# DavidPeicho/cuda-pathtracer

Hardware: AMD Instinct MI355X
Metric: Msamples/sec at 1920x1080, 4 spp, indoor.obj (higher is better)
Workload: dtype f32

## Files before the change

cuda-pathtracer_amd/__init__.py:

```python
from . import native
from .native import (KERNEL_AUTO, KERNEL_BRUTE_FORCE, KERNEL_BVH, KERNEL_BVH_PERSISTENT, KERNEL_BVH_BLOCKWISE, KERNEL_BVH_SPLIT, KERNEL_BVH_RESTART, KERNEL_BVH_RESTART_FMA,
                     PtamdError)
from .scene import (HostScene, cubemap_for_scene, cubemap_from_color, cubemap_from_cross,
                    FACE_DTYPE, MATERIAL_DTYPE, LIGHT_DTYPE, TEXTURE_DTYPE, CAMERA_DTYPE)
from .render import (Context, FrameRenderer, SceneRig, host_pose_faces, host_skin_faces, host_morph_faces, AdaptiveState, host_adaptive_select, host_denoise, DenoiseHistory, HostDenoiseHistory, host_denoise_temporal, orbit_camera, host_bvh_trace, host_skip_trace, host_faces_away, FORM_FLAT_SKIP, FORM_PLAIN_SKIP, host_scene_tables, host_scene_quality, host_bvh_refit_trace, host_bvh4_trace, host_bvh4q_trace, host_bvh8_trace, origin_reach, interleaved_rows, wang_hash, REFERENCE_BOUNCES,
                     POST_NONE, POST_GRAYSCALE, POST_SEPIA, POST_INVERT)
from .tiles import row_bands, band_of_rank, BandGather, interleaved_bands, rank_times_ms, time_gather_ms
from .synthetic import tessellate, deform
from .image import save_ppm, load_ppm, save_png
from .images import pil_image_loader, ldr_to_float, load_image, load_image8, native_image_loader, resize_float

__all__ = [n for n in dir() if not n.startswith("_")]
```

cuda-pathtracer_amd/csrc/ptamd_host.h:

```cpp
#pragma once

#include "../host/ptamd_internal.h"
#include "pt_device.h"
#include "pt_launch.h"
#include "pt_refit.h"
#include "ptamd_owners.h"
#include "ptamd_tuning.h"

#include <string>
#include <type_traits>
#include <vector>

namespace ptamd {

struct DeviceScene {
  DeviceBuffer<float4> nodes;
  DeviceBuffer<float4> nodes4;
  DeviceBuffer<float4> nodes8;
  DeviceBuffer<float4> nodes4q;
  uint32_t n_nodes8 = 0, depth8 = 0;
  DeviceBuffer<float4> tris_bvh;
  DeviceBuffer<float4> tris_brute;
  DeviceBuffer<float4> shade;
  bool flat = false;
  DeviceBuffer<int4> materials;
  DeviceBuffer<float4> lights;
  DeviceBuffer<TexDesc> textures;
  DeviceBuffer<float> texels;
  uint32_t n_faces = 0, n_lights = 0, n_nodes = 0, n_materials = 0, n_textures = 0;
  uint32_t n_bvh_tris = 0;
  uint32_t n_nodes4 = 0, depth4 = 0;
  float extent = 0.0f;
  bool all_finite = true;
  uint32_t n_skipped = 0;
  bool links = false, cull_on = false;
  uint32_t n_culled = 0;
  DeviceBuffer<uint32_t> links_plain;
  Bvh topology;
  std::vector<uint32_t> record_face;
  std::vector<uint8_t> skip_set, cull_bits;
  std::vector<uint32_t> link_words;
  PinnedBuffer<uint32_t> h_links[2];
  float reach = 0.0f;
  float margin_floor = 0.0f;
  ptamd_scene_info info{};
  bool released = false;
  bool refit_ok = false;
  std::vector<uint32_t> material_ids;
  std::vector<ptamd_light> host_lights;
  DeviceBuffer<float> raw;
  DeviceBuffer<uint32_t> refit_groups;
  DeviceBuffer<uint32_t> refit_levels;
  DeviceBuffer<uint32_t> refit_sched;
  DeviceBuffer<uint32_t> wide_child;
  uint32_t n_refit_groups = 0, n_refit_levels = 0, n_refit_sched = 0, refit_top_first = 0, refit_top_levels = 0;
  DeviceBuffer<float> d_faces;
  PinnedBuffer<ptamd_face> h_stage[2];
  Event staged[2];
  bool staged_valid[2] = { false, false };
  uint32_t stage_next = 0;
  Event updated;
  bool updated_valid = false;
  DeviceBuffer<float> d_margin;
  PinnedBuffer<float> h_margin;
  Event margin_ready[2];
  bool margin_ready_valid[2] = { false, false };
  uint32_t margin_next = 0, margin_slot = 0;
  bool margins_pending = false;
  PinnedBuffer<ptamd_light> h_lights[2];
  Event lights_staged[2];
  bool lights_staged_valid[2] = { false, false };
  uint32_t lights_next = 0;
  double quality_built = 0.0;
  DeviceBuffer<double> d_quality;
};

struct DeviceCubemap {
  DeviceBuffer<float4> faces;
  uint32_t size = 0;
  bool uniform = false;
  float color[3] = { 0.f, 0.f, 0.f };
};

}

struct ptamd_context {
  int device = 0;
  ptamd::TuningSettings knobs;
  std::vector<ptamd::DeviceScene> scenes;
  std::vector<ptamd::DeviceCubemap> cubemaps;
  uint32_t frame_counter = 0;
  int32_t last_restart_form = -1;
  ptamd::DeviceBuffer<unsigned long long> d_stats;
  ptamd::DeviceBuffer<float> d_gamma;
  ptamd::DeviceBuffer<uint32_t> d_tickets;
  ptamd::DeviceBuffer<uint32_t> d_heads;
  uint32_t ticket_next = 0;
  std::vector<bool> heads_clean;
  std::vector<bool> slot_pinned;
  int n_cus = 0;
  struct Occupancy { size_t lds = ~(size_t)0; int blocks_per_cu = -1; } occupancy[ptamd::kFormSlots];
  struct SampleScratch {
    void* stream = nullptr;
    ptamd::DeviceBuffer<float> buf[4];
    size_t bytes[4] = { 0, 0, 0, 0 };
    ptamd::Event mega_done[3];
    ptamd::Event resolved[3];
    bool resolved_valid[3] = { false, false, false };
    ptamd::Event last_done;
    uint32_t flip = 0;
    bool no_pipeline = false;
    bool captured = false;
    std::vector<uint32_t> pinned_slots;
  };
  std::vector<SampleScratch> sample_scratch;
  static constexpr uint32_t kMaxLanes = 4;
  ptamd::Stream lane[kMaxLanes];
  uint32_t n_lanes = 0;
  ptamd::Stream internal[2];
  uint32_t lane_next = 0;
  ptamd::DeviceBuffer<uint2> d_trace_spill;
  struct { uint32_t config = ~0u; size_t lds = 0; int resident = 0; } trace_queue_cache;
  size_t trace_spill_bytes = 0;
  ptamd::DeviceBuffer<unsigned long long> d_timeline;
  uint32_t timeline_waves = 0;
  ptamd::DeviceBuffer<float4> d_denoise;
  size_t denoise_pixels = 0;
};

static_assert(!std::is_copy_constructible<ptamd::DeviceScene>::value && !std::is_copy_constructible<ptamd::DeviceCubemap>::value &&
              !std::is_copy_constructible<ptamd_context::SampleScratch>::value && !std::is_copy_constructible<ptamd_context>::value,
              "structs that own device resources move, they are never copied");

namespace ptamd {

constexpr size_t kLdsBudget = 64 * 1024;
constexpr uint32_t kCompactMaxNodes = 896;
constexpr uint32_t kCompactMaxTris = 2047;
constexpr float kBoxMargin = 1e-3f;
constexpr uint32_t kTicketRing = 1024;
constexpr uint32_t kMaxFramesPerSlab = 4;

int hip_fail(const char* what, hipError_t e);

#define PT_HIP(call)                                         \
  do {                                                       \
    hipError_t _e = (call);                                  \
    if (_e != hipSuccess) return hip_fail(#call, _e);        \
  } while (0)

inline bool live_scene(const ptamd_context* ctx, uint32_t scene_id)
{
  return scene_id < ctx->scenes.size() && !ctx->scenes[scene_id].released;
}

int bring_up(ptamd_context* ctx, hipStream_t s);
bool stream_is_capturing(hipStream_t stream);

bool far_origin_camera(const DeviceScene& s, const ptamd_camera& cam);
int settle_margins(DeviceScene& s, hipStream_t stream, const char* who);
void fill_scene(const DeviceScene& s, const DeviceCubemap* cm, KParams& p);
int wait_for_update(const DeviceScene& s, hipStream_t stream, bool capturing);
int update_scene_checks(const char* who, const ptamd_context* ctx, uint32_t scene_id, uint32_t n_faces, const void* faces);
int update_capture_checks(const char* who, const ptamd_context* ctx, hipStream_t stream);
int wait_for_readers(const ptamd_context* ctx, const DeviceScene& s, hipStream_t stream);
int device_array_checks(const char* who, const char* what, const ptamd_context* ctx, const void* p, size_t bytes, bool aligned16);
int prepare_device_refit(const char* who, DeviceScene& s, RefitParams& r);
int enqueue_device_refit(DeviceScene& s, RefitParams& r, const float* faces, hipStream_t stream);

float frame_nb_inverse(float c);
float camera_terms(const ptamd_camera& cam, uint32_t width, KParams& p);
int do_launch(ptamd_context* ctx, const ptamd_launch* l, bool stats, const AdaptiveParams* ad = nullptr);

}
```

cuda-pathtracer_amd/csrc/ptamd_launch.cpp:

```cpp
#include "ptamd_host.h"
#include "pt_adaptive.h"

#include <algorithm>
#include <cmath>
#include <cstdlib>
#include <cstring>

namespace ptamd {

float frame_nb_inverse(float c)
{
  uint32_t bits;
  std::memcpy(&bits, &c, 4);
  const uint32_t exponent = bits >> 23;
  if ((bits & 0x007FFFFFu) != 0u || exponent < 1u || exponent > 253u) return 0.0f;
  return 1.0f / c;
}

namespace {

constexpr float kQuantisedMaxExtent = 1.0e8f;
constexpr size_t kMaxScratchStreams = 16;

void fill_far_table(uint32_t t[16])
// ... 226 lines not shown
  const uint32_t node_bytes = p.wide8 == 2u ? 64u : 128u;
  const uint32_t waves = restart_threads(false) / 64u;
  const uint32_t share = 160u * 1024u / restart_wide_blocks_per_cu() - 256u;
  const uint32_t pools = (ctx->knobs.pool_in_lds && ctx->knobs.pool_in_lds_wide && !ad) ? waves * PT_POOL_LDS_BYTES : 0u;
  const uint32_t region = restart_treelet_region_bytes();
  uint32_t treelet_want = ctx->knobs.treelet_nodes * (128u / node_bytes);
  if (region && treelet_want > region / node_bytes) treelet_want = region / node_bytes;
  uint32_t treelet = treelet_want < p.n_nodes4 ? treelet_want : p.n_nodes4;
  if (!region && treelet * node_bytes + waves * 512u * 4u + pools > share) treelet = (share - pools - waves * 512u * 4u) / node_bytes;
  const uint32_t treelet_bytes = region ? (treelet ? region : 0u) : treelet * node_bytes;
  uint32_t fit = (share - pools - treelet_bytes) / (waves * 512u);
  if (const char* ev = tuning_env("PTAMD_STACK_LDS")) { int v = std::atoi(ev); if (v >= 1 && (uint32_t)v <= fit) fit = (uint32_t)v; }
  p.treelet_nodes = treelet;
  p.stack_lds_entries = need < fit ? need : fit;
  p.stack_spill_entries = need - p.stack_lds_entries;
  pl.launch_lds = (size_t)treelet_bytes + (size_t)p.stack_lds_entries * waves * 512u;
  if (pools) {
    p.pool_lds_offset = (uint32_t)pl.launch_lds;
    if (!p.pool_lds_offset) p.pool_lds_offset = 16u;
    pl.launch_lds = p.pool_lds_offset + pools;
  }
}

KernelForm form_of(const LaunchPlan& pl, bool stats, bool list, const KParams* p)
{
  return megakernel_form(pl.fma ? (uint32_t)PTAMD_KERNEL_BVH_RESTART_FMA : pl.which, pl.resident, stats, list, pl.launch_lds, p);
}

int blocks_per_cu(ptamd_context* ctx, const LaunchPlan& pl, const KernelForm& form, int& bpc)
{
  ptamd_context::Occupancy& occ = ctx->occupancy[form.cache_slot];
  const size_t key = pl.resident ? pl.launch_lds : (pl.which == PTAMD_KERNEL_BVH_RESTART ? pl.launch_lds + 1u : 0);
  if (occ.blocks_per_cu < 0 || occ.lds != key) {
    int q = -1;
    const hipError_t e = form_blocks_per_cu(form, &q);
    if (e != hipSuccess || q < 1) {
      occ.blocks_per_cu = -1;
      return hip_fail((std::string("occupancy query of the ") + form.name + " kernel").c_str(), e);
    }
    occ.blocks_per_cu = q; occ.lds = key;
  }
  bpc = occ.blocks_per_cu;
  return PTAMD_OK;
}

int size_grid(ptamd_context* ctx, const ptamd_launch* l, const AdaptiveParams* ad, LaunchPlan& pl, KParams& p)
{
  const bool restart = pl.which == PTAMD_KERNEL_BVH_RESTART;
  const uint32_t count = l->frame_count > 1 ? l->frame_count : 1u;
  uint32_t rows = l->row_end - l->row_begin;
  if (l->interleave_ranks > 1u) {
    rows = ptamd_interleaved_rows(l->height, l->interleave_ranks, l->interleave_rank, l->interleave_rows);
    p.ilv_ranks = l->interleave_ranks; p.ilv_rank = l->interleave_rank; p.ilv_rows = l->interleave_rows;
    p.row_begin = 0; p.row_end = rows;
    p.tfb_row0 = l->height - rows;
    p.surf_row0 = 0;
  }
  p.y_limit = l->row_end;
  p.tiles_x = (l->width + PT_TILE_W - 1u) / PT_TILE_W;
  p.n_tiles = p.tiles_x * ((rows + PT_TILE_H - 1u) / PT_TILE_H);
  if (p.n_tiles == 0) return PTAMD_OK;
  if ((uint64_t)p.n_tiles * count >= (1ull << 31)) {
    set_error("ptamd_raytrace: rows x width x frame_count too large for one launch (split the batch)");
    return PTAMD_ERR_LIMIT;
  }
  int bpc = 0;
  const KernelForm form = form_of(pl, false, ad != nullptr, nullptr);
  const int rc = blocks_per_cu(ctx, pl, form, bpc);
  if (rc != PTAMD_OK) return rc;
  pl.waves_per_block = form.ticket_waves;
  uint32_t n_blocks = (uint32_t)ctx->n_cus * (uint32_t)bpc;
  p.sample_count = count;
  p.frame_nb0 = l->frame_nb;
  p.refill_min = ctx->knobs.refill_min ? ctx->knobs.refill_min : (l->bounces >= 5 ? 16u : 64u);
  p.tiles_per_ticket = ad ? 1u : ctx->knobs.tiles_per_ticket;
  const uint32_t share = pl.pipelined ? (l->machine_share > 2u ? l->machine_share : 2u) : l->machine_share;
  if (share > 1u) n_blocks = n_blocks / share > 0u ? n_blocks / share : 1u;
  const uint32_t n_tickets = (p.n_tiles * count + p.tiles_per_ticket - 1u) / p.tiles_per_ticket;
  const uint32_t useful = (n_tickets + pl.waves_per_block - 1u) / pl.waves_per_block;
  if (n_blocks > useful) n_blocks = useful;
  if (restart && !ad && p.tiles_per_ticket == 1u && n_blocks >= 8u && (uint64_t)p.n_tiles * count < (1ull << 28) &&
      (ctx->knobs.xcd_regions == 2u || (ctx->knobs.xcd_regions == 1u && !pl.resident))) {
    n_blocks &= ~7u;
    p.xcd_regions = 1u;
  }
  pl.n_blocks = n_blocks;
  if (count > 1) p.frame_nb_f = (float)(int)(l->frame_nb + count - 1u);
  p.frame_nb_inv = frame_nb_inverse(p.frame_nb_f);
  return PTAMD_OK;
}

constexpr int kReplan = -1;

int bind_slab(ptamd_context* ctx, const ptamd_launch* l, LaunchPlan& pl, KParams& p)
{
  ptamd_context::SampleScratch* sc = pl.sc;
  const bool restart = pl.which == PTAMD_KERNEL_BVH_RESTART;
  if (p.sample_count <= 1 && !restart) return PTAMD_OK;
  const size_t sample_bytes = ((size_t)p.sample_count * (p.row_end - p.row_begin) * l->width * 3u * sizeof(float) + 255u) & ~(size_t)255u;
  const size_t pool_bytes = (restart && !p.pool_lds_offset) ? (size_t)pl.n_blocks * pl.waves_per_block * 192u * sizeof(float4) : 0u;
  const size_t spill_bytes = (size_t)pl.n_blocks * pl.waves_per_block * p.stack_spill_entries * 512u;
  const size_t need = sample_bytes + pool_bytes + spill_bytes + 16u;
  auto grow = [&](uint32_t i) -> int {
    PT_HIP(hipStreamSynchronize(pl.stream));
    for (uint32_t k = 0; k < ctx->n_lanes; ++k) PT_HIP(hipStreamSynchronize(ctx->lane[k].get()));
    for (const Stream& is : ctx->internal) if (is) PT_HIP(hipStreamSynchronize(is.get()));
    sc->bytes[i] = 0;
    if (sc->buf[i].alloc(need) != hipSuccess) { (void)hipGetLastError(); return PTAMD_ERR_HIP; }
    sc->bytes[i] = need;
    return PTAMD_OK;
  };
  pl.slab = pl.pipelined ? sc->flip % 3u : 3u;
  if (pl.pipelined) {
    for (int i = 0; i < 3; ++i) {
      PT_HIP(sc->mega_done[i].ensure());
      PT_HIP(sc->resolved[i].ensure());
    }
    bool ok = true;
    for (uint32_t i = 0; i < 3u && ok; ++i) if (need > sc->bytes[i]) ok = grow(i) == PTAMD_OK;
    if (!ok) {
      for (uint32_t i = 0; i < 3u; ++i) { sc->buf[i].reset(); sc->bytes[i] = 0; }
      sc->no_pipeline = true;
      return kReplan;
    }
  } else if (need > sc->bytes[3]) {
    if (pl.capturing) {
      set_error("ptamd_raytrace: a launch cannot size its stream's sample slab inside a graph capture: issue this configuration once eagerly first");
      return PTAMD_ERR_LIMIT;
    }
    if (sc->captured) {
      set_error("ptamd_raytrace: a captured graph pins this stream's sample slab; a larger launch would reallocate it under the graph "
                "(ptamd_release_captured(ctx, stream) once the graph is gone)");
      return PTAMD_ERR_LIMIT;
    }
    if (grow(3u) != PTAMD_OK) return hip_fail("hipMalloc of the sample slab", hipErrorOutOfMemory);
  }
  p.samples_out = sc->buf[pl.slab].get();
  p.pool = reinterpret_cast<float4*>(reinterpret_cast<char*>(p.samples_out) + sample_bytes);
  p.stack_spill = reinterpret_cast<uint2*>(reinterpret_cast<char*>(p.samples_out) + sample_bytes + pool_bytes);
  return PTAMD_OK;
}

int take_slot(ptamd_context* ctx, bool capturing, ptamd_context::SampleScratch* sc, uint32_t& slot)
{
  slot = ctx->ticket_next++ % kTicketRing;
  for (uint32_t tries = 0; ctx->slot_pinned[slot]; ++tries) {
    if (tries >= kTicketRing) { set_error("ptamd_raytrace: every ring slot of ticket heads is pinned by captured graphs (ptamd_release_captured)"); return PTAMD_ERR_LIMIT; }
    slot = ctx->ticket_next++ % kTicketRing;
  }
  if (capturing && sc) { ctx->slot_pinned[slot] = true; sc->pinned_slots.push_back(slot); sc->captured = true; }
  return PTAMD_OK;
}

int issue(ptamd_context* ctx, const DeviceScene& scene, bool stats, const AdaptiveParams* ad, const LaunchPlan& pl, KParams& p)
{
  const bool split = pl.which == PTAMD_KERNEL_BVH_SPLIT, restart = pl.which == PTAMD_KERNEL_BVH_RESTART;
  ptamd_context::SampleScratch* sc = pl.sc;
  int urc = wait_for_update(scene, pl.stream, pl.capturing);
  if (urc != PTAMD_OK) return urc;
  p.round_min = ctx->knobs.round_min;
  p.round_div = ctx->knobs.round_div;
  p.round_div_m16 = (65536u + ctx->knobs.round_div - 1u) / ctx->knobs.round_div;
  p.walk_min = ctx->knobs.walk_min;
  p.walk_min4 = ctx->knobs.walk_min4;
  p.tile_counter = ctx->d_tickets.get() + pl.slot;
  if (ad) p.adaptive = ad->block;
  p.n_static = pl.n_blocks * pl.waves_per_block;
  if (split) PT_HIP(hipMemsetD32Async(reinterpret_cast<hipDeviceptr_t>(p.tile_counter), (int)p.n_static, 1, pl.stream));
  hipStream_t mega_stream = pl.stream;
  if (pl.pipelined) {
    mega_stream = pl.stream != nullptr ? ctx->lane[ctx->lane_next++ % ctx->n_lanes].get() : ctx->internal[ctx->lane_next++ & 1u].get();
    sc->flip++;
    if (sc->resolved_valid[pl.slab]) PT_HIP(hipStreamWaitEvent(mega_stream, sc->resolved[pl.slab].get(), 0));
    if ((urc = wait_for_update(scene, mega_stream, false)) != PTAMD_OK) return urc;
  }
  if (!split) {
    p.tile_heads = ctx->d_heads.get() + (size_t)pl.slot * 8u * PT_HEAD_STRIDE;
    if (!ctx->heads_clean[pl.slot]) PT_HIP(hipMemsetD32Async(reinterpret_cast<hipDeviceptr_t>(p.tile_heads), 0, 8u * PT_HEAD_STRIDE, mega_stream));
    ctx->heads_clean[pl.slot] = false;
  }
  if (restart && !pl.fma && ctx->d_timeline && p.n_static <= ctx->timeline_waves) p.timeline = ctx->d_timeline.get();
  if (split) p.tiles_per_ticket = 1;
  ctx->last_restart_form = restart ? restart_select(pl.resident, stats, ad != nullptr, pl.fma, &p).variant : -1;
  hipError_t e = launch_form(form_of(pl, stats, ad != nullptr, &p), p, pl.n_blocks, restart ? mega_stream : pl.stream);
  if (e == hipSuccess && pl.pipelined) {
    PT_HIP(hipEventRecord(sc->mega_done[pl.slab].get(), mega_stream));
    PT_HIP(hipStreamWaitEvent(pl.stream, sc->mega_done[pl.slab].get(), 0));
  }
  if (e == hipSuccess && (p.sample_count > 1 || restart)) {
    if (ad) {
      AdaptiveParams a = *ad;
      a.samples = p.samples_out;
      a.tile_heads = p.tile_heads;
      e = launch_adaptive_resolve_list(a, pl.stream);
    } else {
      e = launch_resolve(p, pl.stream);
    }
    if (e == hipSuccess && !split) ctx->heads_clean[pl.slot] = true;
    if (e == hipSuccess && pl.pipelined) {
      PT_HIP(hipEventRecord(sc->resolved[pl.slab].get(), pl.stream));
      sc->resolved_valid[pl.slab] = true;
    }
  }
  if (e == hipSuccess && !pl.capturing && ctx->knobs.overlap) {
    PT_HIP(sc->last_done.ensure());
    PT_HIP(hipEventRecord(sc->last_done.get(), pl.stream));
  }
  return e == hipSuccess ? PTAMD_OK : hip_fail("megakernel launch", e);
}

int launch_part(ptamd_context* ctx, const ptamd_launch* l, bool stats, bool later_chunk, const AdaptiveParams* ad, const LaunchPlan& resolved)
{
  LaunchPlan pl = resolved;
  KParams p;
  int rc;
  if (persistent_family(pl.which)) {
    do {
      pl = resolved;
      fill_launch(ctx, l, stats, pl, p);
      if ((rc = plan_stream(ctx, l, stats, later_chunk, ad, pl)) != PTAMD_OK) return rc;
      lay_out_lds(ctx, ctx->scenes[l->scene_id], stats, ad, pl, p);
      if ((rc = size_grid(ctx, l, ad, pl, p)) != PTAMD_OK || p.n_tiles == 0) return rc;
      rc = bind_slab(ctx, l, pl, p);
    } while (rc == kReplan);
    if (rc != PTAMD_OK || (rc = take_slot(ctx, pl.capturing, pl.sc, pl.slot)) != PTAMD_OK) return rc;
    return issue(ctx, ctx->scenes[l->scene_id], stats, ad, pl, p);
  }
  fill_launch(ctx, l, stats, pl, p);
  if (ctx->scenes[l->scene_id].updated_valid &&
      (rc = wait_for_update(ctx->scenes[l->scene_id], pl.stream, stream_is_capturing(pl.stream))) != PTAMD_OK) return rc;
  const KernelForm form = form_of(pl, stats, false, &p);
  uint32_t n_blocks = 0;
  if (pl.which == PTAMD_KERNEL_BVH_BLOCKWISE) {
    const uint32_t rows = l->row_end - l->row_begin;
    const uint32_t st_rows = (form.threads / 64u) * 2u;
    p.tiles_x = (l->width + 31u) / 32u;
    p.n_tiles = p.tiles_x * ((rows + st_rows - 1u) / st_rows);
    if (p.n_tiles == 0) return PTAMD_OK;
    int bpc = 0;
    if ((rc = blocks_per_cu(ctx, pl, form, bpc)) != PTAMD_OK || (rc = take_slot(ctx, false, nullptr, pl.slot)) != PTAMD_OK) return rc;
    n_blocks = std::min((uint32_t)ctx->n_cus * (uint32_t)bpc, p.n_tiles);
    p.tile_counter = ctx->d_tickets.get() + pl.slot;
    PT_HIP(hipMemsetD32Async(reinterpret_cast<hipDeviceptr_t>(p.tile_counter), (int)n_blocks, 1, pl.stream));
  }
  const hipError_t e = launch_form(form, p, n_blocks, pl.stream);
  return e == hipSuccess ? PTAMD_OK : hip_fail("megakernel launch", e);
}

}

int do_launch(ptamd_context* ctx, const ptamd_launch* l, bool stats, const AdaptiveParams* ad)
{
  int rc = validate_launch(ctx, l);
  LaunchPlan resolved;
  if (rc != PTAMD_OK || (rc = settle_margins(ctx->scenes[l->scene_id], static_cast<hipStream_t>(l->stream), "ptamd_raytrace")) != PTAMD_OK ||
      (rc = resolve_kernel(ctx, l, stats, ad, resolved)) != PTAMD_OK) return rc;
  PT_HIP(hipSetDevice(ctx->device));
  const uint32_t part_frames = persistent_family(resolved.which) ? kMaxFramesPerSlab : 1u;
  for (uint32_t k0 = 0; k0 == 0 || k0 < l->frame_count; k0 += part_frames) {
    ptamd_launch part = *l;
    part.frame_nb = l->frame_nb + k0;
    part.frame_count = std::min(l->frame_count - k0, part_frames);
    if (k0 > 0) part.reset_accumulation = 0;
    if ((rc = launch_part(ctx, &part, stats, k0 > 0, ad, resolved)) != PTAMD_OK) return rc;
  }
  return PTAMD_OK;
}

}

using namespace ptamd;

extern "C" {

int ptamd_raytrace(ptamd_context* ctx, void* surface_rgba8, uint32_t scene_id, uint32_t cubemap_id,
                   const ptamd_camera* cam, uint32_t width, uint32_t height, void* stream,
                   float* temporal_framebuffer, int32_t moved, uint32_t post_id)
{
  if (!ctx || !cam) { set_error("ptamd_raytrace: null argument"); return PTAMD_ERR_ARG; }
  uint32_t seed = ctx->frame_counter;
  if (moved) seed = 0;
  seed++;
  ptamd_launch l;
  std::memset(&l, 0, sizeof l);
  l.surface_rgba8 = surface_rgba8; l.temporal_framebuffer = temporal_framebuffer; l.stream = stream;
  l.camera = *cam; l.scene_id = scene_id; l.cubemap_id = cubemap_id;
  l.width = width; l.height = height; l.row_begin = 0; l.row_end = height;
  l.frame_nb = seed; l.bounces = 3;
  l.moved = moved; l.post_id = post_id; l.kernel = PTAMD_KERNEL_AUTO;
  int rc = do_launch(ctx, &l, false);
  if (rc == PTAMD_OK) ctx->frame_counter = seed;
  return rc;
}

int ptamd_raytrace_ex(ptamd_context* ctx, const ptamd_launch* launch) { return do_launch(ctx, launch, false); }

int ptamd_release_captured(ptamd_context* ctx, void* stream)
{
  if (!ctx) { set_error("ptamd_release_captured: null context"); return PTAMD_ERR_ARG; }
  for (auto& c : ctx->sample_scratch) {
    if (c.stream != stream) continue;
    for (uint32_t slot : c.pinned_slots) { ctx->slot_pinned[slot] = false; ctx->heads_clean[slot] = false; }
    c.pinned_slots.clear();
    c.captured = false;
  }
  return PTAMD_OK;
}

int ptamd_raytrace_stats(ptamd_context* ctx, const ptamd_launch* launch, ptamd_trace_stats* out)
{
  if (!ctx || !out) { set_error("ptamd_raytrace_stats: null argument"); return PTAMD_ERR_ARG; }
  PT_HIP(hipSetDevice(ctx->device));
  hipStream_t st = launch ? static_cast<hipStream_t>(launch->stream) : nullptr;
  PT_HIP(hipMemsetAsync(ctx->d_stats.get(), 0, 13 * sizeof(unsigned long long), st));
  PT_HIP(hipMemsetAsync(ctx->d_stats.get() + 16, 0, 12 * sizeof(unsigned long long), st));
  int rc = do_launch(ctx, launch, true);
  if (rc != PTAMD_OK) return rc;
  PT_HIP(hipStreamSynchronize(st));
  unsigned long long h[13];
  PT_HIP(hipMemcpy(h, ctx->d_stats.get(), sizeof h, hipMemcpyDeviceToHost));
  out->rays = h[0]; out->nodes_visited = h[1]; out->tris_tested = h[2];
  out->mesh_hits = h[3]; out->nmap_hits = h[4]; out->samples = h[5];
  out->wave_node_iters = h[6]; out->wave_tri_iters = h[7];
  out->fetch_events = h[8]; out->fetch_rays = h[9];
  out->idle_unstarted = h[10]; out->idle_finished = h[11]; out->idle_parked = h[12];
  return PTAMD_OK;
}

int ptamd_trace_rays(ptamd_context* ctx, uint32_t scene_id, uint32_t kernel, const float* rays_host, uint32_t n,
                     int32_t* out_host)
{
  if (!ctx || !live_scene(ctx, scene_id) || (n && (!rays_host || !out_host)) ||
      (kernel > PTAMD_KERNEL_BVH && kernel != PTAMD_KERNEL_BVH_RESTART)) {
    set_error("ptamd_trace_rays: bad argument");
    return PTAMD_ERR_ARG;
  }
  if (n == 0) return PTAMD_OK;
  PT_HIP(hipSetDevice(ctx->device));
  DeviceScene& s = ctx->scenes[scene_id];
  int src = settle_margins(s, nullptr, "ptamd_trace_rays");
  if (src != PTAMD_OK) return src;
  KParams p;
  std::memset(&p, 0, sizeof p);
  fill_scene(s, nullptr, p);
  fill_far_table(p.far_table);
  p.small_det = 0u;
  p.stack_lds_entries = choose_wide_nodes(ctx, s, true, p);
  DeviceBuffer<float> d_rays;
  DeviceBuffer<int4> d_out;
  PT_HIP(d_rays.alloc((size_t)n * 24));
  hipError_t e = d_out.alloc((size_t)n * 16);
  if (e != hipSuccess) return hip_fail("hipMalloc", e);
  if ((e = hipMemcpy(d_rays.get(), rays_host, (size_t)n * 24, hipMemcpyHostToDevice)) != hipSuccess ||
      (e = launch_trace_rays(p, kernel == PTAMD_KERNEL_BRUTE_FORCE ? 1 : (kernel == PTAMD_KERNEL_BVH_RESTART ? 3 : 2), d_rays.get(), n, d_out.get(), nullptr)) != hipSuccess ||
      (e = hipDeviceSynchronize()) != hipSuccess ||
      (e = hipMemcpy(out_host, d_out.get(), (size_t)n * 16, hipMemcpyDeviceToHost)) != hipSuccess)
    return hip_fail("ptamd_trace_rays", e);
  return PTAMD_OK;
}

int ptamd_trace_rays_queue(ptamd_context* ctx, uint32_t scene_id, const float* rays_dev, uint32_t n, int32_t* out_dev, uint32_t config,
                           uint32_t refill_min, void* stream, uint32_t* out_waves_per_cu)
{
  if (!ctx || !live_scene(ctx, scene_id) || (n && (!rays_dev || !out_dev)) || config > 3u || n >= 0x80000000u) { set_error("ptamd_trace_rays_queue: bad argument"); return PTAMD_ERR_ARG; }
  if (n == 0) return PTAMD_OK;
  PT_HIP(hipSetDevice(ctx->device));
  const DeviceScene& s = ctx->scenes[scene_id];
  if (s.n_nodes4 == 0) { set_error("ptamd_trace_rays_queue: the scene has no wide tree"); return PTAMD_ERR_ARG; }
  hipStream_t st = static_cast<hipStream_t>(stream);
  KParams p;
  std::memset(&p, 0, sizeof p);
  p.nodes4 = s.nodes4.get(); p.n_nodes4 = s.n_nodes4; p.tris_bvh = s.tris_bvh.get(); p.n_bvh_tris = s.n_bvh_tris;
  p.lights = s.lights.get(); p.n_lights = s.n_lights;
  p.refill_min = refill_min < 1u ? 1u : (refill_min > 64u ? 64u : refill_min);
  p.walk_min4 = ctx->knobs.walk_min4;
  uint32_t threads, plane, bpc;
  trace_queue_shape(config, &threads, &plane, &bpc);
  const uint32_t waves = threads / 64u;
  p.treelet_nodes = plane < s.n_nodes4 ? plane : s.n_nodes4;
// ... 33 lines not shown
```

cuda-pathtracer_amd/csrc/ptamd_scene.cpp:

```cpp
#include "ptamd_host.h"
#include "pt_refit.h"
#include "pt_refit_device.h"

#include <cmath>
#include <cstring>

namespace ptamd {

bool far_origin_camera(const DeviceScene& s, const ptamd_camera& cam)
{
  const float cam_far = std::fmax(std::fabs(cam.position.x), std::fmax(std::fabs(cam.position.y), std::fabs(cam.position.z))) +
                        std::fabs(cam.aperture);
  return !(margins_cover(s.extent, s.margin_floor, cam_far) && margins_cover(s.extent, s.margin_floor, s.reach)) && s.n_faces != 0;
}

int settle_margins(DeviceScene& s, hipStream_t stream, const char* who)
{
  if (!s.margins_pending) return PTAMD_OK;
  if (stream_is_capturing(stream)) {
    set_error(std::string(who) + ": the scene's margins are pending behind ptamd_scene_update_device and a capture cannot wait for "
              "them: render the scene once, or call ptamd_scene_quality, outside the capture");
    return PTAMD_ERR_LIMIT;
  }
  PT_HIP(hipEventSynchronize(s.margin_ready[s.margin_slot].get()));
// ... 152 lines not shown
      word |= 0x40000000u;
      std::memcpy(s + 18, &word, 4);
    }
  }
  const bool flat = t.flat = scene_is_flat(sc);
  if (flat) shade.resize(shade.size() + (size_t)sc->n_faces * 16, 0.0f);
  for (uint32_t i = 0; flat && i < sc->n_faces; ++i) {
    const ptamd_face& f = sc->faces[i];
    const float* texel = sc->texels + sc->textures[sc->materials[f.material_id].diffuse_spec_map].offset;
    float* r = &shade[(size_t)sc->n_faces * kShadeFloats + (size_t)i * 16];
    write_flat_normals(f, r);
    for (int k = 0; k < 3; ++k) r[4 * k + 3] = texel[k];
    r[12] = texel[3];
  }
  return PTAMD_OK;
}

int refit_scene_tables(SceneTables& t, const ptamd_face* faces, uint32_t n_faces, const ptamd_light* lights, uint32_t n_lights)
{
  const int rc = refit_bvh(t.bvh, faces, n_faces, lights, n_lights);
  if (rc != PTAMD_OK) return rc;
  for (uint32_t i = 0; i < n_faces; ++i) {
    write_face_geometry(faces[i], i, &t.brute[(size_t)i * 12], &t.shade[(size_t)i * kShadeFloats]);
    if (t.flat) write_flat_normals(faces[i], &t.shade[(size_t)n_faces * kShadeFloats + (size_t)i * 16]);
  }
  return PTAMD_OK;
}

}

int update_scene_checks(const char* who, const ptamd_context* ctx, uint32_t scene_id, uint32_t n_faces, const void* faces)
{
  const std::string w(who);
  if (!live_scene(ctx, scene_id)) { set_error(w + ": scene_id out of range or released"); return PTAMD_ERR_ARG; }
  const DeviceScene& s = ctx->scenes[scene_id];
  if (n_faces != s.n_faces) { set_error(w + ": n_faces differs from the uploaded count"); return PTAMD_ERR_ARG; }
  if (n_faces && !faces) { set_error(w + ": null faces"); return PTAMD_ERR_ARG; }
  if (!s.refit_ok) {
    set_error(w + ": this scene's tree is not refitted (built with PTAMD_WIDE8, PTAMD_WIDE4Q or PTAMD_BVH_SPLIT_ALPHA)");
    return PTAMD_ERR_ARG;
  }
  return PTAMD_OK;
}

int update_capture_checks(const char* who, const ptamd_context* ctx, hipStream_t stream)
{
  for (const auto& c : ctx->sample_scratch)
    if (c.captured) { set_error(std::string(who) + ": a captured launch pins this context's scenes (ptamd_release_captured)"); return PTAMD_ERR_LIMIT; }
  if (stream_is_capturing(stream)) { set_error(std::string(who) + ": an update cannot be captured into a graph"); return PTAMD_ERR_LIMIT; }
  return PTAMD_OK;
}

int device_array_checks(const char* who, const char* what, const ptamd_context* ctx, const void* p, size_t bytes, bool aligned16)
{
  const std::string w = std::string(who) + ": ", name(what);
  if (aligned16 && (reinterpret_cast<uintptr_t>(p) & 15u) != 0u) {
    set_error(w + name + " is not aligned to 16 bytes (the kernels use 16-byte loads)");
    return PTAMD_ERR_ARG;
  }
  PT_HIP(hipSetDevice(ctx->device));
  hipPointerAttribute_t attr;
  std::memset(&attr, 0, sizeof attr);
  if (hipPointerGetAttributes(&attr, p) != hipSuccess || attr.type != hipMemoryTypeDevice || attr.device != ctx->device) {
    (void)hipGetLastError();
    set_error(w + name + " is not device memory of the context's device (host arrays go to the call that takes them)");
    return PTAMD_ERR_ARG;
  }
  hipDeviceptr_t base = nullptr;
  size_t room = 0;
  if (hipMemGetAddressRange(&base, &room, const_cast<void*>(p)) == hipSuccess) {
    const size_t offset = (size_t)(static_cast<const char*>(p) - static_cast<const char*>(base));
    if (offset > room || room - offset < bytes) {
      set_error(w + "the allocation behind " + name + " is smaller than the call reads");
      return PTAMD_ERR_ARG;
    }
  } else {
    (void)hipGetLastError();
  }
  return PTAMD_OK;
}

namespace {

int refit_params(const char* who, const DeviceScene& s, RefitParams& r)
{
  std::memset(&r, 0, sizeof r);
  r.nodes = reinterpret_cast<float*>(s.nodes.get()); r.tris_bvh = reinterpret_cast<float*>(s.tris_bvh.get());
  r.nodes4 = reinterpret_cast<float*>(s.nodes4.get()); r.tris_brute = reinterpret_cast<float*>(s.tris_brute.get());
  r.shade = reinterpret_cast<float*>(s.shade.get()); r.raw = s.raw.get();
  r.groups = s.refit_groups.get(); r.levels = s.refit_levels.get(); r.sched = s.refit_sched.get(); r.wide_child = s.wide_child.get();
  r.n_faces = s.n_faces; r.n_tris = s.n_bvh_tris; r.n_nodes = s.n_nodes; r.n_nodes4 = s.n_nodes4;
  r.n_groups = s.n_refit_groups; r.top_level_first = s.refit_top_first; r.top_levels = s.refit_top_levels;
  r.flat = s.flat ? 1u : 0u;
  r.margin = kBoxMargin;
  if (!r.nodes || !r.tris_bvh || !r.nodes4 || !r.tris_brute || !r.shade || !r.raw || !r.groups || !r.levels || !r.sched || !r.wide_child ||
      r.n_tris != r.n_faces || r.n_nodes == 0 || r.n_groups == 0 || r.top_level_first + r.top_levels > s.n_refit_levels ||
      s.n_refit_sched >= r.n_nodes) {
    set_error(std::string(who) + ": the scene's refit tables are inconsistent");
    return PTAMD_ERR_ARG;
  }
  return PTAMD_OK;
}

}

int wait_for_readers(const ptamd_context* ctx, const DeviceScene& s, hipStream_t stream)
{
  for (const auto& c : ctx->sample_scratch) {
    for (int i = 0; i < 3; ++i) if (c.mega_done[i]) PT_HIP(hipStreamWaitEvent(stream, c.mega_done[i].get(), 0));
    if (c.last_done) PT_HIP(hipStreamWaitEvent(stream, c.last_done.get(), 0));
  }
  if (s.updated_valid) PT_HIP(hipStreamWaitEvent(stream, s.updated.get(), 0));
  return PTAMD_OK;
}

int prepare_device_refit(const char* who, DeviceScene& s, RefitParams& r)
{
  const int rc = refit_params(who, s, r);
  if (rc != PTAMD_OK) return rc;
  if (!s.d_margin) PT_HIP(s.d_margin.alloc((kMarginWords + 2u * kExtentMaxGroups) * sizeof(float)));
  if (!s.h_margin) PT_HIP(s.h_margin.alloc(2u * kMarginWords * sizeof(float)));
  for (int i = 0; i < 2; ++i) PT_HIP(s.margin_ready[i].ensure());
  PT_HIP(s.updated.ensure());
  return PTAMD_OK;
}

int restore_plain_links(DeviceScene& s, hipStream_t stream)
{
  if (!s.n_culled) return PTAMD_OK;
  PT_HIP(hipMemcpyAsync(reinterpret_cast<float*>(s.nodes.get()) + (size_t)s.n_nodes * 16, s.links_plain.get(), ((size_t)s.n_nodes * 8 + 8) * 4,
                        hipMemcpyDeviceToDevice, stream));
  s.n_culled = 0;
  return PTAMD_OK;
}

int enqueue_device_refit(DeviceScene& s, RefitParams& r, const float* faces, hipStream_t stream)
{
  for (int i = 0; i < 2; ++i)
    if (s.margin_ready_valid[i]) PT_HIP(hipStreamWaitEvent(stream, s.margin_ready[i].get(), 0));
  const int rc = restore_plain_links(s, stream);
  if (rc != PTAMD_OK) return rc;
  PT_HIP(launch_extent(faces, s.n_faces, s.d_margin.get() + kMarginWords, s.d_margin.get(), stream));
  r.faces = faces;
  r.device_margin = s.d_margin.get() + 2;
  PT_HIP(launch_refit(r, stream));
  PT_HIP(hipEventRecord(s.updated.get(), stream));
  s.updated_valid = true;
  const uint32_t slot = s.margin_next++ & 1u;
  PT_HIP(hipMemcpyAsync(s.h_margin.get() + (size_t)slot * kMarginWords, s.d_margin.get(), kMarginWords * sizeof(float), hipMemcpyDeviceToHost, stream));
  PT_HIP(hipEventRecord(s.margin_ready[slot].get(), stream));
  s.margin_ready_valid[slot] = true;
  s.margin_slot = slot;
  s.margins_pending = true;
  return PTAMD_OK;
}

}

using namespace ptamd;

extern "C" {

int ptamd_upload_scene(ptamd_context* ctx, const ptamd_scene_desc* sc, uint32_t* out_scene_id)
{
  if (!ctx || !sc || !out_scene_id) { set_error("ptamd_upload_scene: null argument"); return PTAMD_ERR_ARG; }
  int rc = validate_scene_desc(sc);
  if (rc != PTAMD_OK) return rc;
  SceneTables t;
  if ((rc = make_scene_tables(sc, (ctx->knobs.wide8 ? kBvhForm8 : 0u) | (ctx->knobs.wide4q ? kBvhForm4q : 0u), t)) != PTAMD_OK) return rc;
  const Bvh& bvh = t.bvh;
  const std::vector<float>& brute = t.brute;
  const std::vector<float>& shade = t.shade;
  const bool flat = t.flat;
  std::vector<int32_t> mats((size_t)sc->n_materials * 4, 0);
  for (uint32_t i = 0; i < sc->n_materials; ++i) {
    mats[i * 4 + 0] = sc->materials[i].diffuse_spec_map;
    mats[i * 4 + 1] = sc->materials[i].normal_map;
    std::memcpy(&mats[i * 4 + 2], &sc->materials[i].ior, 4);
  }
  std::vector<TexDesc> tex(sc->n_textures);
  for (uint32_t i = 0; i < sc->n_textures; ++i) {
    tex[i].w = sc->textures[i].w; tex[i].h = sc->textures[i].h; tex[i].nb_chan = sc->textures[i].nb_chan;
    tex[i].pad = 0; tex[i].offset = sc->textures[i].offset;
  }

  PT_HIP(hipSetDevice(ctx->device));
  DeviceScene d;
  d.n_faces = sc->n_faces; d.n_lights = sc->n_lights; d.n_nodes = bvh.n_nodes; d.n_bvh_tris = bvh.n_tris;
  d.extent = bvh.extent; d.all_finite = bvh.all_finite; d.reach = bvh.reach; d.margin_floor = bvh.margin_floor;
  d.n_nodes4 = bvh.n_nodes4; d.depth4 = bvh.depth4;
  d.n_nodes8 = bvh.n_nodes8; d.depth8 = bvh.depth8;
  d.n_materials = sc->n_materials; d.n_textures = sc->n_textures;
  d.flat = flat;
  std::vector<ptamd_light> dev_lights(sc->lights, sc->lights + sc->n_lights);
  for (ptamd_light& dl : dev_lights) dl.radius = dl.radius * dl.radius;
  std::vector<float> nodes_and_links(bvh.nodes);
  if (bvh.n_nodes * 64u + bvh.n_tris * 48u <= kLdsBudget && bvh.n_nodes <= kCompactMaxNodes && bvh.n_tris <= kCompactMaxTris && skip_links_fit(bvh)) {
    const uint32_t mode = ctx->knobs.skip_mode;
    SkipTables t;
    build_skip_tables(bvh, mode == PTAMD_SKIP_SET ? mode : (mode | PTAMD_SKIP_CULLED), ctx->knobs.skip_threshold, nullptr, t);
    d.n_skipped = t.n_skipped; d.n_culled = t.n_culled;
    d.links = t.n_skipped != 0u || t.n_culled != 0u;
    if (d.links) {
      nodes_and_links.resize(bvh.nodes.size() + t.words.size());
      std::memcpy(nodes_and_links.data() + bvh.nodes.size(), t.words.data(), t.words.size() * 4);
    }
    if (t.n_culled) {
      std::vector<uint32_t> plain;
      skip_link_table(bvh, t.skip, plain);
      if ((rc = upload(d.links_plain, plain.data(), plain.size() * 4))) return rc;
      d.cull_on = true;
      d.topology.nodes = bvh.nodes;
      d.topology.n_nodes = bvh.n_nodes; d.topology.n_tris = bvh.n_tris;
      d.topology.tris.resize((size_t)bvh.n_tris * 12);
      d.skip_set = t.skip;
      d.record_face.resize(bvh.n_tris);
      for (uint32_t j = 0; j < bvh.n_tris; ++j) std::memcpy(&d.record_face[j], &bvh.tris[(size_t)j * 12 + 9], 4);
    }
  }
  if ((rc = upload(d.nodes, nodes_and_links.data(), nodes_and_links.size() * 4)) ||
      (rc = upload(d.nodes4, bvh.nodes4.data(), bvh.nodes4.size() * 4)) ||
      (bvh.nodes8.empty() ? 0 : (rc = upload(d.nodes8, bvh.nodes8.data(), bvh.nodes8.size() * 4))) ||
      (bvh.nodes4q.empty() ? 0 : (rc = upload(d.nodes4q, bvh.nodes4q.data(), bvh.nodes4q.size() * 4))) ||
      (rc = upload_padded(d.tris_bvh, bvh.tris.data(), bvh.tris.size() * 4, 128)) ||
      (rc = upload(d.tris_brute, brute.data(), brute.size() * 4)) ||
      (rc = upload(d.shade, shade.data(), shade.size() * 4)) ||
      (rc = upload(d.materials, mats.data(), mats.size() * 4)) ||
      (rc = upload(d.lights, dev_lights.data(), dev_lights.size() * sizeof(ptamd_light))) ||
      (rc = upload(d.textures, tex.data(), tex.size() * sizeof(TexDesc))) ||
      (rc = upload(d.texels, sc->texels, (size_t)sc->n_texel_floats * 4)))
    return rc;
  d.refit_ok = !bvh.split && bvh.nodes8.empty() && bvh.nodes4q.empty();
  if (d.refit_ok) {
    if ((rc = upload(d.raw, bvh.raw.data(), bvh.raw.size() * 4)) ||
        (rc = upload(d.refit_groups, bvh.refit_groups.data(), bvh.refit_groups.size() * 4)) ||
        (rc = upload(d.refit_levels, bvh.refit_levels.data(), bvh.refit_levels.size() * 4)) ||
        (rc = upload(d.refit_sched, bvh.refit_sched.data(), bvh.refit_sched.size() * 4)) ||
        (rc = upload(d.wide_child, bvh.wide_child.data(), bvh.wide_child.size() * 4)))
      return rc;
    d.n_refit_groups = (uint32_t)bvh.refit_groups.size() / 4u; d.n_refit_levels = (uint32_t)bvh.refit_levels.size();
    d.n_refit_sched = (uint32_t)bvh.refit_sched.size();
    d.refit_top_first = bvh.refit_top_first; d.refit_top_levels = bvh.refit_top_levels;
    d.material_ids.resize(sc->n_faces);
    for (uint32_t i = 0; i < sc->n_faces; ++i) d.material_ids[i] = sc->faces[i].material_id;
  }
  d.host_lights.assign(sc->lights, sc->lights + sc->n_lights);
  d.quality_built = tree_quality(bvh.nodes.data(), bvh.n_nodes, sc->n_faces);
  d.info.n_faces = sc->n_faces; d.info.n_lights = sc->n_lights; d.info.n_nodes = bvh.n_nodes;
  d.info.n_leaves = bvh.n_leaves; d.info.max_leaf_size = bvh.max_leaf; d.info.depth = bvh.depth;
  d.info.node_bytes = 64; d.info.tri_bytes = 48;
  d.info.n_nodes4 = d.n_nodes4; d.info.depth4 = d.depth4;
  d.info.lds_bytes_bvh = bvh.n_nodes * 64u + bvh.n_tris * 48u;
  d.info.lds_bytes_brute = sc->n_faces * 48u;
  ctx->scenes.push_back(std::move(d));
  *out_scene_id = (uint32_t)ctx->scenes.size() - 1;
  return PTAMD_OK;
}

int ptamd_scene_update(ptamd_context* ctx, const ptamd_scene_update_desc* d)
{
  if (!ctx || !d) { set_error("ptamd_scene_update: null argument"); return PTAMD_ERR_ARG; }
  int rc = update_scene_checks("ptamd_scene_update", ctx, d->scene_id, d->n_faces, d->faces);
  if (rc != PTAMD_OK) return rc;
  DeviceScene& s = ctx->scenes[d->scene_id];
  for (uint32_t i = 0; i < d->n_faces; ++i)
    if (d->faces[i].material_id != s.material_ids[i]) { set_error("ptamd_scene_update: a face's material_id differs from the uploaded one"); return PTAMD_ERR_ARG; }
  hipStream_t stream = static_cast<hipStream_t>(d->stream);
  if ((rc = update_capture_checks("ptamd_scene_update", ctx, stream)) != PTAMD_OK) return rc;
  if (d->n_faces == 0) return PTAMD_OK;
  PT_HIP(hipSetDevice(ctx->device));
  RefitParams r;
  if ((rc = refit_params("ptamd_scene_update", s, r)) != PTAMD_OK) return rc;
  const size_t bytes = (size_t)d->n_faces * sizeof(ptamd_face);
  if (!s.d_faces) PT_HIP(s.d_faces.alloc(bytes));
  const size_t link_words = (size_t)s.n_nodes * 8 + 8;
  for (int i = 0; i < 2; ++i) {
    if (!s.h_stage[i]) PT_HIP(s.h_stage[i].alloc(bytes));
    if (s.cull_on && !s.h_links[i]) PT_HIP(s.h_links[i].alloc(link_words * 4));
    PT_HIP(s.staged[i].ensure());
  }
  PT_HIP(s.updated.ensure());
  Bvh m;
  m.margin = kBoxMargin;
  r.origin_margin = bvh_margins(m, d->faces, d->n_faces, s.host_lights.data(), (uint32_t)s.host_lights.size());
  const uint32_t slot = s.stage_next++ & 1u;
  if (s.staged_valid[slot]) PT_HIP(hipEventSynchronize(s.staged[slot].get()));
  std::memcpy(s.h_stage[slot].get(), d->faces, bytes);
  if ((rc = wait_for_readers(ctx, s, stream)) != PTAMD_OK) return rc;
  PT_HIP(hipMemcpyAsync(s.d_faces.get(), s.h_stage[slot].get(), bytes, hipMemcpyHostToDevice, stream));
  if (s.cull_on) {
    Bvh& topo = s.topology;
    for (uint32_t j = 0; j < s.n_bvh_tris; ++j) rf_tri_record(&d->faces[s.record_face[j]].vertices[0].x, s.record_face[j], &topo.tris[(size_t)j * 12]);
    const uint32_t n_culled = cull_table(topo, s.cull_bits);
    skip_link_table(topo, s.skip_set, s.link_words, n_culled ? &s.cull_bits : nullptr);
    std::memcpy(s.h_links[slot].get(), s.link_words.data(), link_words * 4);
    PT_HIP(hipMemcpyAsync(reinterpret_cast<float*>(s.nodes.get()) + (size_t)s.n_nodes * 16, s.h_links[slot].get(), link_words * 4, hipMemcpyHostToDevice, stream));
    s.n_culled = n_culled;
  }
  PT_HIP(hipEventRecord(s.staged[slot].get(), stream));
  s.staged_valid[slot] = true;
  r.faces = s.d_faces.get();
  PT_HIP(launch_refit(r, stream));
  PT_HIP(hipEventRecord(s.updated.get(), stream));
  s.updated_valid = true;
  s.extent = m.extent; s.all_finite = m.all_finite; s.reach = m.reach; s.margin_floor = m.margin_floor;
  s.margins_pending = false;
  return PTAMD_OK;
}

int ptamd_scene_update_device(ptamd_context* ctx, const ptamd_scene_update_device_desc* d)
{
  const char* who = "ptamd_scene_update_device";
  if (!ctx || !d) { set_error("ptamd_scene_update_device: null argument"); return PTAMD_ERR_ARG; }
  int rc = update_scene_checks(who, ctx, d->scene_id, d->n_faces, d->faces);
  hipStream_t stream = static_cast<hipStream_t>(d->stream);
  if (rc != PTAMD_OK || (rc = update_capture_checks(who, ctx, stream)) != PTAMD_OK) return rc;
  DeviceScene& s = ctx->scenes[d->scene_id];
  if (d->n_faces == 0) return PTAMD_OK;
  if ((rc = device_array_checks(who, "faces", ctx, d->faces, (size_t)d->n_faces * sizeof(ptamd_face), true)) != PTAMD_OK) return rc;
  RefitParams r;
  if ((rc = prepare_device_refit(who, s, r)) != PTAMD_OK || (rc = wait_for_readers(ctx, s, stream)) != PTAMD_OK) return rc;
  return enqueue_device_refit(s, r, reinterpret_cast<const float*>(d->faces), stream);
}

int ptamd_scene_update_lights(ptamd_context* ctx, const ptamd_scene_lights_desc* d)
{
  const char* who = "ptamd_scene_update_lights";
  if (!ctx || !d) { set_error("ptamd_scene_update_lights: null argument"); return PTAMD_ERR_ARG; }
  if (!live_scene(ctx, d->scene_id)) { set_error("ptamd_scene_update_lights: scene_id out of range or released"); return PTAMD_ERR_ARG; }
  DeviceScene& s = ctx->scenes[d->scene_id];
  if (d->n_lights != s.n_lights) { set_error("ptamd_scene_update_lights: n_lights differs from the uploaded count"); return PTAMD_ERR_ARG; }
  if (d->n_lights && !d->lights) { set_error("ptamd_scene_update_lights: null lights"); return PTAMD_ERR_ARG; }
  hipStream_t stream = static_cast<hipStream_t>(d->stream);
  int rc = update_capture_checks(who, ctx, stream);
  if (rc != PTAMD_OK) return rc;
  if (d->n_lights == 0) return PTAMD_OK;
  PT_HIP(hipSetDevice(ctx->device));
  const size_t bytes = (size_t)d->n_lights * sizeof(ptamd_light);
  for (int i = 0; i < 2; ++i) {
    if (!s.h_lights[i]) PT_HIP(s.h_lights[i].alloc(bytes));
    PT_HIP(s.lights_staged[i].ensure());
  }
  PT_HIP(s.updated.ensure());
  const uint32_t slot = s.lights_next++ & 1u;
  if (s.lights_staged_valid[slot]) PT_HIP(hipEventSynchronize(s.lights_staged[slot].get()));
  ptamd_light* staged = s.h_lights[slot].get();
  for (uint32_t i = 0; i < d->n_lights; ++i) {
    staged[i] = d->lights[i];
    staged[i].radius = d->lights[i].radius * d->lights[i].radius;
  }
  if ((rc = wait_for_readers(ctx, s, stream)) != PTAMD_OK) return rc;
  PT_HIP(hipMemcpyAsync(s.lights.get(), staged, bytes, hipMemcpyHostToDevice, stream));
  PT_HIP(hipEventRecord(s.lights_staged[slot].get(), stream));
  s.lights_staged_valid[slot] = true;
  PT_HIP(hipEventRecord(s.updated.get(), stream));
  s.updated_valid = true;
  s.host_lights.assign(d->lights, d->lights + d->n_lights);
  if (!s.margins_pending) {
    Bvh m;
    m.margin = kBoxMargin;
    bvh_margins_of_extent(m, s.extent, s.all_finite, s.host_lights.data(), (uint32_t)s.host_lights.size());
    s.reach = m.reach; s.margin_floor = m.margin_floor;
  }
  return PTAMD_OK;
}

int ptamd_scene_margins(ptamd_context* ctx, uint32_t scene_id, float out[4])
{
  if (!ctx || !out) { set_error("ptamd_scene_margins: null argument"); return PTAMD_ERR_ARG; }
  if (!live_scene(ctx, scene_id)) { set_error("ptamd_scene_margins: scene_id out of range or released"); return PTAMD_ERR_ARG; }
// ... 6 lines not shown

int ptamd_scene_quality(ptamd_context* ctx, uint32_t scene_id, void* stream, ptamd_scene_quality_info* out)
{
  if (!ctx || !out) { set_error("ptamd_scene_quality: null argument"); return PTAMD_ERR_ARG; }
  if (!live_scene(ctx, scene_id)) { set_error("ptamd_scene_quality: scene_id out of range or released"); return PTAMD_ERR_ARG; }
  hipStream_t st = static_cast<hipStream_t>(stream);
  if (stream_is_capturing(st)) { set_error("ptamd_scene_quality: the call waits for its result and cannot be captured into a graph"); return PTAMD_ERR_LIMIT; }
  DeviceScene& s = ctx->scenes[scene_id];
  int rc = settle_margins(s, st, "ptamd_scene_quality");
  if (rc != PTAMD_OK) return rc;
  out->built = s.quality_built;
  out->now = 0.0;
  if (s.n_nodes == 0 || s.n_faces == 0) return PTAMD_OK;
  PT_HIP(hipSetDevice(ctx->device));
  const uint32_t groups = quality_groups(s.n_nodes);
  if (!s.d_quality) PT_HIP(s.d_quality.alloc((size_t)(groups + 1u) * sizeof(double)));
  if ((rc = wait_for_update(s, st, false)) != PTAMD_OK) return rc;
  PT_HIP(launch_quality(reinterpret_cast<const float*>(s.nodes.get()), s.n_nodes, s.d_quality.get(), st));
  std::vector<double> part(groups + 1u);
  PT_HIP(hipMemcpyAsync(part.data(), s.d_quality.get(), part.size() * sizeof(double), hipMemcpyDeviceToHost, st));
  PT_HIP(hipStreamSynchronize(st));
  double sum = 0.0;
  for (uint32_t g = 0; g < groups; ++g) sum += part[g];
  out->now = sum / part[groups];
  return PTAMD_OK;
}

int ptamd_host_scene_quality(const ptamd_scene_desc* sc, const ptamd_face* faces_b, double* out)
{
  if (!sc || !out) { set_error("ptamd_host_scene_quality: null argument"); return PTAMD_ERR_ARG; }
  int rc = validate_scene_desc(sc);
  SceneTables t;
  if (rc != PTAMD_OK || (rc = make_scene_tables(sc, 0u, t)) != PTAMD_OK) return rc;
  if (faces_b && (rc = refit_scene_tables(t, faces_b, sc->n_faces, sc->lights, sc->n_lights)) != PTAMD_OK) return rc;
  *out = tree_quality(t.bvh.nodes.data(), t.bvh.n_nodes, sc->n_faces);
  return PTAMD_OK;
}

int ptamd_scene_release(ptamd_context* ctx, uint32_t scene_id)
{
  if (!ctx) { set_error("ptamd_scene_release: null context"); return PTAMD_ERR_ARG; }
  if (!live_scene(ctx, scene_id)) { set_error("ptamd_scene_release: scene_id out of range or released"); return PTAMD_ERR_ARG; }
  PT_HIP(hipSetDevice(ctx->device));
  PT_HIP(hipDeviceSynchronize());
  ctx->scenes[scene_id] = DeviceScene();
  ctx->scenes[scene_id].released = true;
  return PTAMD_OK;
}

int ptamd_scene_table_read(ptamd_context* ctx, uint32_t scene_id, uint32_t which, void* out, uint64_t* bytes)
{
  if (!ctx || !bytes || which > 4u) { set_error("ptamd_scene_table_read: bad argument"); return PTAMD_ERR_ARG; }
  if (!live_scene(ctx, scene_id)) { set_error("ptamd_scene_table_read: scene_id out of range or released"); return PTAMD_ERR_ARG; }
  const DeviceScene& s = ctx->scenes[scene_id];
  const void* src[5] = { s.nodes.get(), s.tris_bvh.get(), s.nodes4.get(), s.tris_brute.get(), s.shade.get() };
  const uint64_t size[5] = { (uint64_t)s.n_nodes * 64u, (uint64_t)s.n_bvh_tris * 48u, (uint64_t)s.n_nodes4 * 128u, (uint64_t)s.n_faces * 48u,
                             (uint64_t)s.n_faces * (kShadeFloats * 4u + (s.flat ? 64u : 0u)) };
  const uint64_t room = *bytes;
  *bytes = size[which];
  if (!out) return PTAMD_OK;
  if (room < size[which]) { set_error("ptamd_scene_table_read: the buffer is smaller than the table"); return PTAMD_ERR_ARG; }
  PT_HIP(hipSetDevice(ctx->device));
  PT_HIP(hipDeviceSynchronize());
  if (size[which]) PT_HIP(hipMemcpy(out, src[which], size[which], hipMemcpyDeviceToHost));
  return PTAMD_OK;
}

int ptamd_host_scene_refit(const ptamd_scene_desc* sc, const ptamd_face* faces_b, const ptamd_face* faces_c, uint32_t which, void* out,
                           uint64_t* bytes)
{
  if (!sc || !bytes || which > 5u) { set_error("ptamd_host_scene_refit: bad argument"); return PTAMD_ERR_ARG; }
  int rc = validate_scene_desc(sc);
  SceneTables t;
  if (rc != PTAMD_OK || (rc = make_scene_tables(sc, 0u, t)) != PTAMD_OK) return rc;
  for (const ptamd_face* f : { faces_b, faces_c })
    if (f && (rc = refit_scene_tables(t, f, sc->n_faces, sc->lights, sc->n_lights)) != PTAMD_OK) return rc;
  const float scalars[4] = { t.bvh.extent, t.bvh.reach, t.bvh.margin_floor, t.bvh.all_finite ? 1.0f : 0.0f };
  const void* src[6] = { t.bvh.nodes.data(), t.bvh.tris.data(), t.bvh.nodes4.data(), t.brute.data(), t.shade.data(), scalars };
  const uint64_t size[6] = { t.bvh.nodes.size() * 4u, t.bvh.tris.size() * 4u, t.bvh.nodes4.size() * 4u, t.brute.size() * 4u, t.shade.size() * 4u, 16u };
  const uint64_t room = *bytes;
  *bytes = size[which];
  if (!out) return PTAMD_OK;
  if (room < size[which]) { set_error("ptamd_host_scene_refit: the buffer is smaller than the table"); return PTAMD_ERR_ARG; }
  if (size[which]) std::memcpy(out, src[which], size[which]);
  return PTAMD_OK;
}

int ptamd_upload_cubemap(ptamd_context* ctx, const float* faces, uint32_t size, uint32_t* out_cubemap_id)
{
  if (!ctx || !faces || !out_cubemap_id || size == 0 || size > 16384) { set_error("ptamd_upload_cubemap: bad argument"); return PTAMD_ERR_ARG; }
  PT_HIP(hipSetDevice(ctx->device));
  DeviceCubemap c;
  c.size = size;
  if (size == 1) {
    c.uniform = true;
    for (int f = 1; f < 6; ++f) c.uniform = c.uniform && std::memcmp(faces + f * 4, faces, 12) == 0;
    std::memcpy(c.color, faces, 12);
  }
  int rc = upload(c.faces, faces, (size_t)6 * size * size * 16);
  if (rc != PTAMD_OK) return rc;
  ctx->cubemaps.push_back(std::move(c));
  *out_cubemap_id = (uint32_t)ctx->cubemaps.size() - 1;
  return PTAMD_OK;
}

int ptamd_scene_info_get(ptamd_context* ctx, uint32_t scene_id, ptamd_scene_info* out)
{
  if (!ctx || !out || !live_scene(ctx, scene_id)) { set_error("ptamd_scene_info_get: bad argument"); return PTAMD_ERR_ARG; }
  *out = ctx->scenes[scene_id].info;
  return PTAMD_OK;
}

int ptamd_scene_desc_is_flat(const ptamd_scene_desc* sc, int32_t* out_flat)
{
  if (!sc || !out_flat || (sc->n_faces && !sc->faces) || (sc->n_materials && !sc->materials) || (sc->n_textures && !sc->textures)) {
    set_error("ptamd_scene_desc_is_flat: null argument or table");
    return PTAMD_ERR_ARG;
  }
  for (uint32_t i = 0; i < sc->n_faces; ++i) {
    const uint32_t m = sc->faces[i].material_id;
    if (m >= sc->n_materials || sc->materials[m].diffuse_spec_map < 0 || (uint32_t)sc->materials[m].diffuse_spec_map >= sc->n_textures) {
      set_error("ptamd_scene_desc_is_flat: material or texture id out of range");
      return PTAMD_ERR_ARG;
    }
  }
  *out_flat = scene_is_flat(sc) ? 1 : 0;
  return PTAMD_OK;
}

int ptamd_scene_is_flat(ptamd_context* ctx, uint32_t scene_id, uint32_t cubemap_id, int32_t* out_flat)
{
  if (!ctx || !out_flat || !live_scene(ctx, scene_id) || cubemap_id >= ctx->cubemaps.size()) {
    set_error("ptamd_scene_is_flat: bad argument");
    return PTAMD_ERR_ARG;
  }
  *out_flat = ctx->knobs.flat_round && ctx->scenes[scene_id].flat && ctx->cubemaps[cubemap_id].uniform ? 1 : 0;
  return PTAMD_OK;
}

int ptamd_scene_skip_count(ptamd_context* ctx, uint32_t scene_id, uint32_t* out)
{
  if (!ctx || !out || !live_scene(ctx, scene_id)) { set_error("ptamd_scene_skip_count: bad argument"); return PTAMD_ERR_ARG; }
  *out = ctx->scenes[scene_id].n_skipped;
  return PTAMD_OK;
}

int ptamd_last_restart_form(ptamd_context* ctx, int32_t* out)
{
  if (!ctx || !out) { set_error("ptamd_last_restart_form: null argument"); return PTAMD_ERR_ARG; }
  *out = ctx->last_restart_form;
  return PTAMD_OK;
}

int ptamd_scene_cull_count(ptamd_context* ctx, uint32_t scene_id, uint32_t* out)
{
  if (!ctx || !out || !live_scene(ctx, scene_id)) { set_error("ptamd_scene_cull_count: bad argument"); return PTAMD_ERR_ARG; }
  *out = ctx->scenes[scene_id].n_culled;
  return PTAMD_OK;
}

}
```

cuda-pathtracer_amd/csrc/ptamd_tuning.cpp:

```cpp
#include "ptamd_tuning.h"
#include "../host/ptamd_internal.h"

#include <cstdlib>
#include <cstring>

namespace ptamd {

const char* tuning_env(const char* name)
{
  const char* gate = std::getenv("PTAMD_TUNING");
  if (!gate || std::atoi(gate) != 1) return nullptr;
  return std::getenv(name);
}

namespace {

enum KnobKind {
  kSwitch,
  kClamped,
  kKernel,
  kSkipWord,
  kOpenUnit,
};

struct Knob {
  const char* name;
  KnobKind kind;
  bool TuningSettings::* flag;
  uint32_t TuningSettings::* number;
  float TuningSettings::* real;
  int lo, hi;
};

constexpr Knob on_off(const char* name, bool TuningSettings::* f) { return { name, kSwitch, f, nullptr, nullptr, 0, 1 }; }
constexpr Knob number(const char* name, KnobKind kind, uint32_t TuningSettings::* f, int lo, int hi) { return { name, kind, nullptr, f, nullptr, lo, hi }; }

using S = TuningSettings;
constexpr Knob kKnobs[] = {
  on_off("PTAMD_GAMMA_TABLE", &S::gamma_table),
  on_off("PTAMD_OVERLAP", &S::overlap),
  number("PTAMD_REFILL_MIN", kClamped, &S::refill_min, 1, 64),
  number("PTAMD_DEFAULT_KERNEL", kKernel, &S::default_kernel, 1, 6),
  number("PTAMD_ROUND_MIN", kClamped, &S::round_min, 1, 64),
  number("PTAMD_ROUND_DIV", kClamped, &S::round_div, 1, 64),
  number("PTAMD_WALK_MIN", kClamped, &S::walk_min, 1, 64),
  number("PTAMD_WALK_MIN4", kClamped, &S::walk_min4, 1, 64),
  on_off("PTAMD_SHORT_RCP", &S::short_rcp),
  on_off("PTAMD_WIDE8", &S::wide8),
  on_off("PTAMD_WIDE4Q", &S::wide4q),
  on_off("PTAMD_RS_GENERIC", &S::generic_round),
  on_off("PTAMD_RS_FLAT", &S::flat_round),
  number("PTAMD_SKIP", kSkipWord, &S::skip_mode, 0, 0),
  { "PTAMD_SKIP_THRESHOLD", kOpenUnit, nullptr, nullptr, &S::skip_threshold, 0, 1 },
  on_off("PTAMD_POOL_LDS", &S::pool_in_lds),
  on_off("PTAMD_POOL_LDS_WIDE", &S::pool_in_lds_wide),
  number("PTAMD_TREELET", kClamped, &S::treelet_nodes, 0, 1024),
  number("PTAMD_XCD_REGIONS", kClamped, &S::xcd_regions, 0, 2),
  number("PTAMD_TILES_PER_TICKET", kClamped, &S::tiles_per_ticket, 1, 1024),
};

}

void read_tuning_knobs(TuningSettings& s)
{
  s = TuningSettings();
  for (const Knob& k : kKnobs) {
    const char* e = tuning_env(k.name);
    if (!e) continue;
    const int v = std::atoi(e);
    switch (k.kind) {
      case kSwitch: s.*k.flag = v != 0; break;
      case kClamped: s.*k.number = (uint32_t)(v < k.lo ? k.lo : (v > k.hi ? k.hi : v)); break;
      case kKernel:
        if (v >= k.lo && v <= k.hi) { s.*k.number = (uint32_t)v; s.default_kernel_is_builtin = false; }
        break;
      case kSkipWord:
        s.*k.number = !std::strcmp(e, "root") ? PTAMD_SKIP_ROOT : (!std::strcmp(e, "all") ? PTAMD_SKIP_ALL : (!std::strcmp(e, "0") ? PTAMD_SKIP_SET : PTAMD_SKIP_DEFAULT));
        break;
      case kOpenUnit: {
        const float f = (float)std::atof(e);
        if (f > (float)k.lo && f < (float)k.hi) s.*k.real = f;
        break;
      }
    }
  }
}

}
```

cuda-pathtracer_amd/csrc/ptamd_tuning.h:

```cpp
#pragma once

#include "ptamd.h"

namespace ptamd {

struct TuningSettings {
  bool gamma_table = true;
  bool overlap = true;
  uint32_t refill_min = 0;
  uint32_t default_kernel = PTAMD_KERNEL_BVH_RESTART;
  bool default_kernel_is_builtin = true;
  uint32_t round_min = 16, round_div = 4;
  uint32_t walk_min = 7;
  uint32_t walk_min4 = 16;
  bool short_rcp = true;
  bool wide8 = false;
  bool wide4q = false;
  bool generic_round = false;
  bool flat_round = true;
  uint32_t skip_mode = PTAMD_SKIP_DEFAULT;
  float skip_threshold = 0.0f;
  bool pool_in_lds = true;
  bool pool_in_lds_wide = false;
  uint32_t treelet_nodes = 512;
  uint32_t xcd_regions = 0;
  uint32_t tiles_per_ticket = 1;
};

void read_tuning_knobs(TuningSettings& s);

}
```

cuda-pathtracer_amd/host/bvh_walks.cpp:

```cpp
#include "ptamd_internal.h"

#include <algorithm>
#include <cmath>
#include <cstring>
#include <limits>

namespace ptamd {

namespace {

inline uint32_t f2u(float f) { uint32_t u; std::memcpy(&u, &f, 4); return u; }
inline float u2f(uint32_t u) { float f; std::memcpy(&f, &u, 4); return f; }

struct Ray {
  const float* dir;
  const float* origin;
  float inv[3], noi[3];
  Ray(const float d[3], const float o[3]) : dir(d), origin(o)
  {
    for (int a = 0; a < 3; ++a) {
      const float da = std::fabs(dir[a]) < 1e-30f ? std::copysign(1e-30f, dir[a]) : dir[a];
      inv[a] = 1.0f / da;
      noi[a] = -(origin[a] * inv[a]);
    }
  }
  uint32_t octant() const { return (dir[0] < 0.f ? 1u : 0u) | (dir[1] < 0.f ? 2u : 0u) | (dir[2] < 0.f ? 4u : 0u); }
  uint32_t sign_octant() const { return (std::signbit(dir[0]) ? 1u : 0u) | (std::signbit(dir[1]) ? 2u : 0u) | (std::signbit(dir[2]) ? 4u : 0u); }
};

struct Best {
  float t = 100000.0f, u = 0.f, v = 0.f;
  uint32_t idx = 0xFFFFFFFFu;
  void write(HostHit& out) const
  {
    out.kind = idx == 0xFFFFFFFFu ? 0 : 1;
    out.index = idx == 0xFFFFFFFFu ? -1 : (int32_t)idx;
    out.t = t; out.u = u; out.v = v;
  }
};

void test_leaf(const Bvh& bvh, uint32_t first, uint32_t count, const Ray& ray, Best& best, uint64_t* tris_tested)
{
  const float* dir = ray.dir;
  const float* origin = ray.origin;
  for (uint32_t k = 0; k < count; ++k) {
    const float* t = &bvh.tris[(size_t)(first + k) * 12];
    if (tris_tested) ++*tris_tested;
    const float e1[3] = { t[0], t[1], t[2] }, e2[3] = { t[3], t[4], t[5] }, v0[3] = { t[6], t[7], t[8] };
    const float p[3] = { dir[1] * e2[2] - dir[2] * e2[1], dir[2] * e2[0] - dir[0] * e2[2], dir[0] * e2[1] - dir[1] * e2[0] };
    const float det = e1[0] * p[0] + e1[1] * p[1] + e1[2] * p[2];
    if (det < 1e-7f) continue;
    const float inv_det = 1.0f / det;
    const float tv[3] = { origin[0] - v0[0], origin[1] - v0[1], origin[2] - v0[2] };
    const float u = (tv[0] * p[0] + tv[1] * p[1] + tv[2] * p[2]) * inv_det;
    if (u < 0 || u > 1) continue;
    const float q[3] = { tv[1] * e1[2] - tv[2] * e1[1], tv[2] * e1[0] - tv[0] * e1[2], tv[0] * e1[1] - tv[1] * e1[0] };
    const float v = (dir[0] * q[0] + dir[1] * q[1] + dir[2] * q[2]) * inv_det;
    if (v < 0 || u + v > 1) continue;
    const float tt = (e2[0] * q[0] + e2[1] * q[1] + e2[2] * q[2]) * inv_det;
    const uint32_t idx = f2u(t[9]);
    if (tt > 0.0f && (tt < best.t || (tt == best.t && idx < best.idx && best.idx != 0xFFFFFFFFu))) {
      best.t = tt; best.u = u; best.v = v; best.idx = idx;
    }
  }
}

struct Entry { uint32_t ref; float tnear; };

bool next_node(const Bvh& bvh, std::vector<Entry>& stack, const Ray& ray, Best& best, uint64_t* tris_tested, uint32_t& node)
{
  while (!stack.empty()) {
    const Entry e = stack.back();
    stack.pop_back();
    if (!(e.tnear <= best.t)) continue;
    if (!(e.ref & 0x80000000u)) { node = e.ref; return true; }
    test_leaf(bvh, e.ref & 0xFFFFFFu, (e.ref >> 24) & 0x7Fu, ray, best, tris_tested);
  }
  return false;
}

void count_visit(uint64_t* nodes_visited, uint32_t node, uint32_t top, uint32_t upper)
{
  if (!nodes_visited) return;
  ++*nodes_visited;
  if (node < top) ++nodes_visited[3];
  if (node < upper) ++nodes_visited[4];
}

void bvh4_trace_impl(const Bvh& bvh, const float dir[3], const float origin[3], HostHit& out, uint64_t* nodes_visited,
                     uint64_t* tris_tested, bool quantised)
{
  const Ray ray(dir, origin);
  const float* inv = ray.inv;
  const float* noi = ray.noi;
  const uint32_t oct = ray.octant(), soct = ray.sign_octant();
  Best best;
  std::vector<Entry> stack;
  if (bvh.n_nodes4) stack.push_back({ 0u, 0.0f });
  uint32_t node;
  while (next_node(bvh, stack, ray, best, tris_tested, node)) {
    count_visit(nodes_visited, node, 85u, 341u);
    uint32_t hit = 0;
    float tn[4];
    uint32_t order, refs[4];
    int self_counted = 0;
    if (!quantised) {
      const float* q = &bvh.nodes4[(size_t)node * 32];
      for (int c = 0; c < 4; ++c) {
        float tnear = -std::numeric_limits<float>::infinity(), tfar = std::numeric_limits<float>::infinity();
        for (int a = 0; a < 3; ++a) {
          const float tc = std::fma(q[a * 4 + c], inv[a], noi[a]), ai = std::fabs(inv[a]);
          tnear = std::max(tnear, std::fma(-q[12 + a * 4 + c], ai, tc));
          tfar = std::min(tfar, std::fma(q[12 + a * 4 + c], ai, tc));
        }
        tn[c] = std::max(tnear, 0.0f);
        if (tn[c] <= std::min(tfar, best.t)) hit |= 1u << c;
        refs[c] = f2u(q[24 + c]);
      }
      order = (f2u(q[28 + (oct >> 1)]) >> (16 * (oct & 1))) & 0xFFFFu;
    } else {
      const uint32_t* q = &bvh.nodes4q[(size_t)node * 16];
      float A[3], B[3];
      for (int a = 0; a < 3; ++a) {
        A[a] = u2f(((q[3] >> (8 * a)) & 0xFFu) << 23) * inv[a];
        B[a] = std::fma(u2f(q[a]), inv[a], noi[a]);
      }
      for (int c = 0; c < 4; ++c) {
        float tnear = -std::numeric_limits<float>::infinity(), tfar = std::numeric_limits<float>::infinity();
        for (int a = 0; a < 3; ++a) {
          const uint32_t lo = (q[8 + a] >> (8 * c)) & 0xFFu, hi = (q[11 + a] >> (8 * c)) & 0xFFu;
          const bool neg = ((soct >> a) & 1u) != 0u;
          tnear = std::max(tnear, std::fma((float)(neg ? hi : lo), A[a], B[a]));
          tfar = std::min(tfar, std::fma((float)(neg ? lo : hi), A[a], B[a]));
        }
        tn[c] = std::max(tnear, 0.0f);
        if (tn[c] <= std::min(tfar, best.t)) hit |= 1u << c;
        refs[c] = q[4 + c];
      }
      const uint32_t h = (soct & 4u) ? (~soct & 3u) : (soct & 3u);
      order = (q[14 + (h >> 1)] >> (16 * (h & 1u))) & 0xFFFFu;
      if (soct & 4u) { order = ~order & 0xFFFFu; self_counted = 1; }
    }
    Entry pushed[4];
    const int nhit = __builtin_popcount(hit);
    for (int c = 0; c < 4; ++c) {
      if (!((hit >> c) & 1u)) continue;
      const int rank = __builtin_popcount(hit & ((order >> (4 * c)) & 0xFu)) - self_counted;
      pushed[nhit - 1 - rank] = { refs[c], tn[c] };
    }
    for (int i = 0; i < nhit; ++i) stack.push_back(pushed[i]);
  }
  best.write(out);
}

}

void bvh4_trace_host(const Bvh& bvh, const float dir[3], const float origin[3], HostHit& out, uint64_t* nodes_visited,
                     uint64_t* tris_tested)
{
  bvh4_trace_impl(bvh, dir, origin, out, nodes_visited, tris_tested, false);
}
void bvh4q_trace_host(const Bvh& bvh, const float dir[3], const float origin[3], HostHit& out, uint64_t* nodes_visited,
                      uint64_t* tris_tested)
{
  bvh4_trace_impl(bvh, dir, origin, out, nodes_visited, tris_tested, true);
}

void bvh8_trace_host(const Bvh& bvh, const float dir[3], const float origin[3], HostHit& out, uint64_t* nodes_visited,
                     uint64_t* tris_tested)
{
  const Ray ray(dir, origin);
  const uint32_t oct = ray.sign_octant();
  Best best;
  std::vector<Entry> stack;
  if (bvh.n_nodes8) stack.push_back({ 0u, 0.0f });
  uint32_t node;
  while (next_node(bvh, stack, ray, best, tris_tested, node)) {
    const uint32_t* q = &bvh.nodes8[(size_t)node * 32];
    count_visit(nodes_visited, node, 73u, 585u);
    float A[3], B[3];
    for (int a = 0; a < 3; ++a) {
      const float scale = u2f(((q[3] >> (8 * a)) & 0xFFu) << 23);
      A[a] = scale * ray.inv[a];
      B[a] = std::fma(u2f(q[a]), ray.inv[a], ray.noi[a]);
    }
    const uint8_t* planes = reinterpret_cast<const uint8_t*>(q + 12);
    uint32_t hit = 0;
    float tn[8];
    for (int c = 0; c < 8; ++c) {
      float tnear = 0.0f, tfar = best.t;
      for (int a = 0; a < 3; ++a) {
        const float tl = std::fma((float)planes[a * 8 + c], A[a], B[a]), th = std::fma((float)planes[24 + a * 8 + c], A[a], B[a]);
        const bool neg = (oct >> a) & 1u;
        tnear = std::max(tnear, neg ? th : tl);
        tfar = std::min(tfar, neg ? tl : th);
      }
      tn[c] = tnear;
      if (tnear <= tfar) hit |= 1u << c;
    }
    for (int f = 7; f >= 0; --f) {
      const int c = f ^ (int)oct;
      if ((hit >> c) & 1u) stack.push_back({ q[4 + c], tn[c] });
    }
  }
  best.write(out);
}

void bvh_trace_host(const Bvh& bvh, const ptamd_face*, const float dir[3], const float origin[3],
                    HostHit& out, uint64_t* nodes_visited, uint64_t* tris_tested)
{
  const Ray ray(dir, origin);
  const uint32_t oct = ray.octant();
  Best best;
  uint32_t node = bvh.n_nodes ? 0u : 0xFFFFFFFFu;
  while (node != 0xFFFFFFFFu) {
    const float* q = &bvh.nodes[(size_t)node * 16];
    if (nodes_visited) ++*nodes_visited;
    float tnear = -std::numeric_limits<float>::infinity(), tfar = std::numeric_limits<float>::infinity();
    for (int a = 0; a < 3; ++a) {
      float t0 = std::fma(q[a], ray.inv[a], ray.noi[a]);
      float t1 = std::fma(q[4 + a], ray.inv[a], ray.noi[a]);
      tnear = std::fmax(tnear, std::fmin(t0, t1));
      tfar = std::fmin(tfar, std::fmax(t0, t1));
    }
    const bool hit = tnear <= tfar && tfar >= 0.0f && tnear <= best.t;
    const uint32_t info = f2u(q[3]);
    const uint32_t miss = f2u(q[8 + oct]);
    if (!hit) { node = miss; continue; }
    const uint32_t count = info >> 24;
    if (count == 0) {
      const uint32_t child = f2u(q[7]);
      const uint32_t right = child & 0x3FFFFFFFu, axis = child >> 30;
      node = ((oct >> axis) & 1) ? right : node + 1;
      continue;
    }
    test_leaf(bvh, info & 0xFFFFFFu, count, ray, best, tris_tested);
    node = miss;
  }
  best.write(out);
}

namespace {
template <bool MIRROR>
void skip_walk(const Bvh& bvh, const uint32_t* words, const float dir[3], const float origin[3], HostHit& out,
               uint64_t* nodes_visited, uint64_t* tris_tested, uint32_t* node_visits, uint32_t* node_passes)
{
  const Ray ray(dir, origin);
  const uint32_t oct = ray.octant();
  Best best;
  uint32_t node = words[(size_t)bvh.n_nodes * 8 + oct];
  while (node != 0xFFFFu) {
    const float* q = &bvh.nodes[(size_t)node * 16];
    if (nodes_visited) ++*nodes_visited;
    float tnear = -std::numeric_limits<float>::infinity(), tfar = std::numeric_limits<float>::infinity();
    for (int a = 0; a < 3; ++a) {
      if (MIRROR) {
        float t0 = std::fma(q[a], ray.inv[a], ray.noi[a]);
        float t1 = std::fma(q[4 + a], ray.inv[a], ray.noi[a]);
        tnear = std::fmax(tnear, std::fmin(t0, t1));
        tfar = std::fmin(tfar, std::fmax(t0, t1));
      } else {
        const float t0 = q[a] * ray.inv[a] + ray.noi[a], t1 = q[4 + a] * ray.inv[a] + ray.noi[a];
        const float lo = t0 < t1 ? t0 : t1, hi = t0 < t1 ? t1 : t0;
        tnear = lo > tnear ? lo : tnear;
        tfar = hi < tfar ? hi : tfar;
      }
    }
    const bool hit = tnear <= tfar && tfar >= 0.0f && tnear <= best.t;
    if (node_visits) { ++node_visits[node]; node_passes[node] += hit ? 1u : 0u; }
    const uint32_t word = words[(size_t)node * 8 + oct];
    uint32_t code = hit ? (word & 0xFFFFu) : (word >> 16);
    if (code >= 0x8000u && code != 0xFFFFu) {
      test_leaf(bvh, code & 0x7FFu, (code >> 11) & 0xFu, ray, best, tris_tested);
      code = word >> 16;
    }
    node = code;
  }
  best.write(out);
}
}

void skip_trace_host(const Bvh& bvh, const uint32_t* words, const float dir[3], const float origin[3], HostHit& out,
                     uint64_t* nodes_visited, uint64_t* tris_tested, uint32_t* node_visits, uint32_t* node_passes)
{
  skip_walk<true>(bvh, words, dir, origin, out, nodes_visited, tris_tested, node_visits, node_passes);
}

void skip_count_host(const Bvh& bvh, const uint32_t* words, const float dir[3], const float origin[3], uint32_t* node_visits, uint32_t* node_passes)
{
  HostHit h;
  skip_walk<false>(bvh, words, dir, origin, h, nullptr, nullptr, node_visits, node_passes);
}

}

namespace {

typedef void (*Walk)(const ptamd::Bvh&, const float*, const float*, ptamd::HostHit&, uint64_t*, uint64_t*);
void binary_walk(const ptamd::Bvh& bvh, const float* dir, const float* origin, ptamd::HostHit& out, uint64_t* nodes_visited, uint64_t* tris_tested)
{
  ptamd::bvh_trace_host(bvh, nullptr, dir, origin, out, nodes_visited, tris_tested);
}

void trace_rays(const ptamd::Bvh& bvh, Walk walk, const float* rays, uint32_t n, int32_t* out, uint64_t* counters)
{
  for (uint32_t i = 0; i < n; ++i) {
    ptamd::HostHit h;
    walk(bvh, rays + (size_t)i * 6, rays + (size_t)i * 6 + 3, h, counters ? &counters[0] : nullptr, counters ? &counters[1] : nullptr);
    out[i * 4 + 0] = h.kind;
    out[i * 4 + 1] = h.index;
    std::memcpy(&out[i * 4 + 2], &h.t, 4);
    out[i * 4 + 3] = 0;
  }
}

int build_and_trace(const char* entry, uint32_t max_leaf, Walk walk, const ptamd_face* faces, uint32_t n_faces, const float* rays, uint32_t n,
                    int32_t* out, uint64_t* counters, ptamd::Bvh& bvh)
{
  if ((n_faces && !faces) || (n && (!rays || !out))) { ptamd::set_error(std::string(entry) + ": null argument"); return PTAMD_ERR_ARG; }
  const int rc = ptamd::build_bvh(faces, n_faces, 1e-3f, max_leaf, bvh);
  if (rc == PTAMD_OK) trace_rays(bvh, walk, rays, n, out, counters);
  return rc;
}

}

extern "C" int ptamd_host_bvh8_trace(const ptamd_face* faces, uint32_t n_faces, const float* rays, uint32_t n,
                                     int32_t* out, uint64_t* counters)
{
  ptamd::Bvh bvh;
  const int rc = build_and_trace("ptamd_host_bvh8_trace", 2, ptamd::bvh8_trace_host, faces, n_faces, rays, n, out, counters, bvh);
  if (rc == PTAMD_OK && counters) { counters[2] = bvh.depth8; counters[5] = bvh.n_nodes8; }
  return rc;
}

extern "C" int ptamd_host_bvh4_trace(const ptamd_face* faces, uint32_t n_faces, const float* rays, uint32_t n,
                                     int32_t* out, uint64_t* counters)
{
  ptamd::Bvh bvh;
  const int rc = build_and_trace("ptamd_host_bvh4_trace", 4, ptamd::bvh4_trace_host, faces, n_faces, rays, n, out, counters, bvh);
  if (rc == PTAMD_OK && counters) counters[2] = bvh.depth4;
  return rc;
}

extern "C" int ptamd_host_bvh4q_trace(const ptamd_face* faces, uint32_t n_faces, const float* rays, uint32_t n,
                                      int32_t* out, uint64_t* counters)
{
  ptamd::Bvh bvh;
  const int rc = build_and_trace("ptamd_host_bvh4q_trace", 2, ptamd::bvh4q_trace_host, faces, n_faces, rays, n, out, counters, bvh);
  if (rc == PTAMD_OK && counters) counters[2] = bvh.depth4;
  return rc;
}

extern "C" int ptamd_host_bvh_trace(const ptamd_face* faces, uint32_t n_faces, const float* rays, uint32_t n,
                                    int32_t* out, uint64_t* counters)
{
  ptamd::Bvh bvh;
  return build_and_trace("ptamd_host_bvh_trace", 4, binary_walk, faces, n_faces, rays, n, out, counters, bvh);
}

extern "C" int ptamd_host_bvh_refit_trace(const ptamd_face* faces_a, const ptamd_face* faces_b, uint32_t n_faces, const float* rays, uint32_t n,
                                          int32_t* out_binary, int32_t* out_wide)
{
  if ((n_faces && (!faces_a || !faces_b)) || (n && (!rays || !out_binary || !out_wide))) { ptamd::set_error("ptamd_host_bvh_refit_trace: null argument"); return PTAMD_ERR_ARG; }
  ptamd::Bvh bvh;
  int rc = ptamd::build_bvh(faces_a, n_faces, 1e-3f, 4, bvh, 0u);
  if (rc != PTAMD_OK || (rc = ptamd::refit_bvh(bvh, faces_b, n_faces, nullptr, 0)) != PTAMD_OK) return rc;
  trace_rays(bvh, binary_walk, rays, n, out_binary, nullptr);
  trace_rays(bvh, ptamd::bvh4_trace_host, rays, n, out_wide, nullptr);
  return PTAMD_OK;
}

extern "C" int ptamd_host_skip_trace(const ptamd_face* faces, const ptamd_face* faces_refit, uint32_t n_faces, uint32_t mode, float threshold,
                                     const uint8_t* skip_in, const float* rays, uint32_t n, int32_t* out, uint64_t* counters,
                                     uint32_t* n_nodes, uint8_t* skip_out, uint32_t* words_out)
{
  if ((n_faces && !faces) || (n && (!rays || !out)) || !n_nodes || (mode & ~PTAMD_SKIP_CULLED) > PTAMD_SKIP_ALL) { ptamd::set_error("ptamd_host_skip_trace: bad argument"); return PTAMD_ERR_ARG; }
  ptamd::Bvh bvh;
  int rc = ptamd::build_bvh(faces, n_faces, 1e-3f, 2, bvh, 0u);
  if (rc != PTAMD_OK) return rc;
  if (!ptamd::skip_links_fit(bvh)) { ptamd::set_error("ptamd_host_skip_trace: the tree is outside the compact layout's code space"); return PTAMD_ERR_LIMIT; }
  const uint32_t room = *n_nodes;
  *n_nodes = bvh.n_nodes;
  if ((skip_out || words_out) && room < bvh.n_nodes) { ptamd::set_error("ptamd_host_skip_trace: room for fewer nodes than the tree has"); return PTAMD_ERR_ARG; }
  ptamd::SkipTables t;
  ptamd::build_skip_tables(bvh, mode, threshold, skip_in, t);
  if (faces_refit && (rc = ptamd::refit_bvh(bvh, faces_refit, n_faces, nullptr, 0)) != PTAMD_OK) return rc;
  if (faces_refit && (mode & PTAMD_SKIP_CULLED)) {
    const std::vector<uint8_t> kept(t.skip);
    ptamd::build_skip_tables(bvh, PTAMD_SKIP_SET | PTAMD_SKIP_CULLED, 0.0f, kept.data(), t);
  }
  const std::vector<uint8_t>& skip = t.skip;
  const std::vector<uint32_t>& words = t.words;
  for (uint32_t i = 0; i < n; ++i) {
    ptamd::HostHit h;
    uint64_t visits = 0;
    ptamd::skip_trace_host(bvh, words.data(), rays + (size_t)i * 6, rays + (size_t)i * 6 + 3, h, &visits, counters ? &counters[1] : nullptr);
    if (counters) counters[0] += visits;
    out[i * 4 + 0] = h.kind;
    out[i * 4 + 1] = h.index;
    std::memcpy(&out[i * 4 + 2], &h.t, 4);
    out[i * 4 + 3] = (int32_t)visits;
  }
  if (counters) { counters[2] = 0; for (uint8_t s : skip) counters[2] += s; }
  if (skip_out && bvh.n_nodes) std::memcpy(skip_out, skip.data(), bvh.n_nodes);
  if (words_out) std::memcpy(words_out, words.data(), words.size() * 4);
  return PTAMD_OK;
}

extern "C" int ptamd_host_faces_away(const float* edges, uint32_t n, uint8_t* out)
{
  if (n && (!edges || !out)) { ptamd::set_error("ptamd_host_faces_away: null argument"); return PTAMD_ERR_ARG; }
  for (uint32_t i = 0; i < n; ++i) {
    out[i] = 0;
    for (uint32_t o = 0; o < 8; ++o) out[i] |= (uint8_t)((ptamd::record_faces_away(edges + (size_t)i * 6, edges + (size_t)i * 6 + 3, o) ? 1u : 0u) << o);
  }
  return PTAMD_OK;
}
```

cuda-pathtracer_amd/host/ptamd_internal.h:

```cpp
#pragma once

#include "ptamd.h"

#include <string>
#include <vector>

namespace ptamd {

void set_error(const std::string& msg);

const char* tuning_env(const char* name);

struct HostScene {
  std::vector<ptamd_face> faces;
  std::vector<uint32_t> mesh_sizes;
  std::vector<ptamd_material> materials;
  std::vector<ptamd_light> lights;
  std::vector<ptamd_texture_desc> textures;
  std::vector<float> texels;
  std::vector<std::string> unloaded_textures;
  ptamd_camera camera;
  std::string cubemap;
};

struct ImageProvider {
  ptamd_image_load_fn load;
  ptamd_image_free_fn release;
  void* user;
};

int load_host_scene(const char* scene_path, uint32_t flags, const ImageProvider* provider, HostScene*& out);

struct Image8 { int w = 0, h = 0, c = 0; std::vector<uint8_t> px; };
bool decode_jpeg(const uint8_t* bytes, size_t n_bytes, Image8& img, std::string& err);
bool decode_png(const uint8_t* bytes, size_t n_bytes, Image8& img, std::string& err);
bool encode_png(const uint8_t* pixels, int w, int h, int channels, std::vector<uint8_t>& out);
bool load_image8(const char* path, Image8& img, std::string& err);
bool load_image_float(const char* path, int* w, int* h, int* c, float** data, std::string& err);
const float* ldr_to_linear_table();
bool resize_float(const float* in, int in_w, int in_h, float* out, int out_w, int out_h, int channels);
const ImageProvider* builtin_image_provider();

struct Bvh {
  std::vector<float> nodes;
  std::vector<float> tris;
  uint32_t n_nodes = 0, n_leaves = 0, max_leaf = 0, depth = 0;
  uint32_t n_tris = 0;
  std::vector<float> nodes4;
  uint32_t n_nodes4 = 0, depth4 = 0;
  std::vector<uint32_t> nodes4q;
  std::vector<uint32_t> nodes8;
  uint32_t n_nodes8 = 0, depth8 = 0, max_leaf8 = 0;
  float extent = 0.0f;
  bool all_finite = true;
  float reach = 0.0f;
  float margin_floor = 0.0f;
  float margin = 0.0f;
  bool split = false;
  std::vector<float> raw;
  std::vector<uint32_t> wide_child;
  std::vector<uint32_t> refit_groups, refit_levels, refit_sched;
  uint32_t refit_top_first = 0, refit_top_levels = 0;
};


constexpr uint32_t kBvhForm8 = 1u, kBvhForm4q = 2u;
int build_bvh(const ptamd_face* faces, uint32_t n_faces, float margin, uint32_t max_leaf, Bvh& out, uint32_t forms = kBvhForm8 | kBvhForm4q,
              const ptamd_light* lights = nullptr, uint32_t n_lights = 0);

int refit_bvh(Bvh& bvh, const ptamd_face* faces, uint32_t n_faces, const ptamd_light* lights = nullptr, uint32_t n_lights = 0);

float bvh_margins(Bvh& bvh, const ptamd_face* faces, uint32_t n_faces, const ptamd_light* lights, uint32_t n_lights);

float bvh_margins_of_extent(Bvh& bvh, float extent, bool all_finite, const ptamd_light* lights, uint32_t n_lights);

float origin_reach(const ptamd_light* lights, uint32_t n_lights, float extent);

inline bool margins_cover(float extent, float margin_floor, float origin_far)
{
  return (origin_far + extent) * (1.0f / 2097152.0f) <= margin_floor;
}

bool pose_groups_cover(const uint32_t* group_sizes, uint32_t n_groups, uint32_t n_faces);
bool skin_indices_valid(const uint16_t* bone_indices, uint32_t n_faces, uint32_t n_bones);
int morph_targets_check(const char* who, const ptamd_morph_target* targets, uint32_t n_targets, uint32_t n_faces, uint64_t* n_entries);
void morph_table(const ptamd_morph_target* targets, uint32_t n_targets, uint32_t n_faces, std::vector<uint32_t>& begin, std::vector<uint32_t>& entries);

struct HostHit { int32_t kind; int32_t index; float t; float u, v; };
void bvh_trace_host(const Bvh& bvh, const ptamd_face* faces, const float dir[3], const float origin[3],
                    HostHit& out, uint64_t* nodes_visited, uint64_t* tris_tested);
void bvh4_trace_host(const Bvh& bvh, const float dir[3], const float origin[3], HostHit& out, uint64_t* nodes_visited,
                     uint64_t* tris_tested);
void bvh8_trace_host(const Bvh& bvh, const float dir[3], const float origin[3], HostHit& out, uint64_t* nodes_visited,
                     uint64_t* tris_tested);
void bvh4q_trace_host(const Bvh& bvh, const float dir[3], const float origin[3], HostHit& out, uint64_t* nodes_visited,
                      uint64_t* tris_tested);

constexpr float kSkipThreshold = 0.6f;
constexpr uint32_t kSkipRaysPerNode = 2u, kSkipMaxRaysPerNode = 256u, kSkipMinVisits = 16u;
bool skip_links_fit(const Bvh& bvh);

bool record_faces_away(const float e1[3], const float e2[3], uint32_t octant);
uint32_t cull_table(const Bvh& bvh, std::vector<uint8_t>& cull);
void skip_link_table(const Bvh& bvh, const std::vector<uint8_t>& skip, std::vector<uint32_t>& words, const std::vector<uint8_t>* cull = nullptr);
void skip_set_of(const Bvh& bvh, uint32_t mode, float threshold, const uint8_t* given, std::vector<uint8_t>& skip, uint32_t rays_per_node = 0u);
void select_skip_nodes(const Bvh& bvh, float threshold, std::vector<uint8_t>& skip, uint32_t rays_per_node = kSkipRaysPerNode);
struct SkipTables {
  std::vector<uint8_t> skip, cull;
  std::vector<uint32_t> words;
  uint32_t n_skipped = 0, n_culled = 0;
};
void build_skip_tables(const Bvh& bvh, uint32_t mode, float threshold, const uint8_t* given, SkipTables& out);
void skip_trace_host(const Bvh& bvh, const uint32_t* words, const float dir[3], const float origin[3], HostHit& out,
                     uint64_t* nodes_visited, uint64_t* tris_tested, uint32_t* node_visits = nullptr, uint32_t* node_passes = nullptr);
void skip_count_host(const Bvh& bvh, const uint32_t* words, const float dir[3], const float origin[3], uint32_t* node_visits, uint32_t* node_passes);

}
```

cuda-pathtracer_amd/host/skip_links.cpp:

```cpp
#include "ptamd_internal.h"

#include <cmath>
#include <cstdlib>
#include <cstring>

namespace ptamd {

namespace {

inline uint32_t f2u(float f) { uint32_t u; std::memcpy(&u, &f, 4); return u; }

struct Node { uint32_t count, first, right, axis; };
Node node_of(const Bvh& bvh, uint32_t n)
{
  const float* q = &bvh.nodes[(size_t)n * 16];
  const uint32_t info = f2u(q[3]), child = f2u(q[7]);
  return { info >> 24, info & 0xFFFFFFu, child & 0x3FFFFFFFu, child >> 30 };
}

uint32_t down(const Node& nd, uint32_t n, uint32_t o) { return ((o >> nd.axis) & 1u) ? nd.right : n + 1u; }

struct Rng {
  uint64_t s;
  uint32_t next() { s ^= s >> 12; s ^= s << 25; s ^= s >> 27; return (uint32_t)((s * 0x2545F4914F6CDD1Dull) >> 32); }
  float unit() { return (float)(next() >> 8) * (1.0f / 16777216.0f); }
};

}

bool skip_links_fit(const Bvh& bvh) { return bvh.n_nodes <= 896u && bvh.n_tris <= 2047u && bvh.max_leaf <= 15u; }

namespace {

enum Sign { kZero, kNonNeg, kNonPos, kOpen };
Sign product_sign(bool d_negative, float e)
{
  if (e == 0.0f) return kZero;
  return ((e < 0.0f) != d_negative) ? kNonPos : kNonNeg;
}
Sign difference_sign(Sign a, Sign b)
{
  if (a == kZero && b == kZero) return kZero;
  if ((a == kNonPos || a == kZero) && (b == kNonNeg || b == kZero)) return kNonPos;
  if ((a == kNonNeg || a == kZero) && (b == kNonPos || b == kZero)) return kNonNeg;
  return kOpen;
}
bool term_not_positive(float e, Sign p)
{
  if (e == 0.0f || p == kZero) return true;
  if (p == kOpen) return false;
  return (e > 0.0f) == (p == kNonPos);
}

}

bool record_faces_away(const float e1[3], const float e2[3], uint32_t octant)
{
  for (int k = 0; k < 3; ++k)
    if (!(std::fabs(e1[k]) < 1099511627776.0f) || !(std::fabs(e2[k]) < 1099511627776.0f)) return false;
  const bool nx = octant & 1u, ny = (octant >> 1) & 1u, nz = (octant >> 2) & 1u;
  const Sign px = difference_sign(product_sign(ny, e2[2]), product_sign(nz, e2[1]));
  const Sign py = difference_sign(product_sign(nz, e2[0]), product_sign(nx, e2[2]));
  const Sign pz = difference_sign(product_sign(nx, e2[1]), product_sign(ny, e2[0]));
  return term_not_positive(e1[0], px) && term_not_positive(e1[1], py) && term_not_positive(e1[2], pz);
}

uint32_t cull_table(const Bvh& bvh, std::vector<uint8_t>& cull)
{
  const uint32_t N = bvh.n_nodes;
  cull.assign(N, 0);
  for (uint32_t n = N; n-- > 0u;) {
    const Node nd = node_of(bvh, n);
    if (!nd.count) { cull[n] = cull[n + 1u] & cull[nd.right]; continue; }
    uint8_t bits = 0xFFu;
    for (uint32_t k = 0; k < nd.count; ++k) {
      const float* t = &bvh.tris[(size_t)(nd.first + k) * 12];
      for (uint32_t o = 0; o < 8; ++o) if (!record_faces_away(t, t + 3, o)) bits &= (uint8_t)~(1u << o);
    }
    cull[n] = bits;
  }
  uint32_t pairs = 0;
  const uint8_t keep = N ? (uint8_t)~cull[0] : 0xFFu;
  for (uint32_t n = 0; n < N; ++n) {
    cull[n] &= keep;
    if (node_of(bvh, n).count) pairs += (uint32_t)__builtin_popcount(cull[n]);
  }
  return pairs;
}

namespace {

uint32_t leaf_code(const Bvh& bvh, const Node& nd, uint32_t o, bool culling)
{
  uint32_t first = nd.first, count = nd.count;
  if (culling) {
    uint32_t a = 0, b = nd.count;
    const auto away = [&](uint32_t k) { const float* t = &bvh.tris[(size_t)(nd.first + k) * 12]; return record_faces_away(t, t + 3, o); };
    while (a < b && away(a)) ++a;
    while (b > a && away(b - 1u)) --b;
    if (a < b) { first = nd.first + a; count = b - a; }
  }
  return 0x8000u | (count << 11) | (first & 0x7FFu);
}

}

void skip_link_table(const Bvh& bvh, const std::vector<uint8_t>& skip, std::vector<uint32_t>& words, const std::vector<uint8_t>* cull)
{
  const uint32_t N = bvh.n_nodes;
  words.assign((size_t)N * 8 + 8, 0xFFFFu);
  const auto resolve = [&](uint32_t t, uint32_t o, bool culling) {
    while (t != 0xFFFFFFFFu) {
      if (culling && (((*cull)[t] >> o) & 1u)) t = f2u(bvh.nodes[(size_t)t * 16 + 8 + o]);
      else if (skip[t]) t = down(node_of(bvh, t), t, o);
      else break;
    }
    return t == 0xFFFFFFFFu ? 0xFFFFu : t;
  };
  for (uint32_t n = 0; n < N; ++n) {
    const Node nd = node_of(bvh, n);
    for (uint32_t o = 0; o < 8; ++o) {
      const bool culling = cull && !(((*cull)[n] >> o) & 1u);
      const uint32_t hit = nd.count ? leaf_code(bvh, nd, o, culling) : resolve(down(nd, n, o), o, culling);
      words[(size_t)n * 8 + o] = hit | (resolve(f2u(bvh.nodes[(size_t)n * 16 + 8 + o]), o, culling) << 16);
    }
  }
  for (uint32_t o = 0; o < 8 && N; ++o) words[(size_t)N * 8 + o] = resolve(0u, o, cull != nullptr);
}

namespace {

bool training_rays(const Bvh& bvh, uint32_t n_rays, std::vector<float>& rays)
{
  std::vector<double> cdf(bvh.n_tris);
  double total = 0.0;
  for (uint32_t i = 0; i < bvh.n_tris; ++i) {
    const float* t = &bvh.tris[(size_t)i * 12];
    const double nx = (double)t[1] * t[5] - (double)t[2] * t[4], ny = (double)t[2] * t[3] - (double)t[0] * t[5], nz = (double)t[0] * t[4] - (double)t[1] * t[3];
    const double area = std::sqrt(nx * nx + ny * ny + nz * nz);
    bool finite = area > 1.0e-30 && area < 1.0e30;
    for (int k = 0; k < 9; ++k) finite = finite && std::fabs(t[k]) < 1.0e30f;
    if (finite) total += area;
    cdf[i] = total;
  }
  if (!(total > 0.0)) return false;
  rays.resize((size_t)n_rays * 6);
  Rng rng = { 0x9E3779B97F4A7C15ull };
  for (uint32_t r = 0; r < n_rays; ++r) {
    const double pick = (double)rng.unit() * total;
    uint32_t lo = 0, hi = bvh.n_tris - 1u;
    while (lo < hi) { const uint32_t mid = (lo + hi) / 2u; if (cdf[mid] > pick) hi = mid; else lo = mid + 1u; }
    const float* t = &bvh.tris[(size_t)lo * 12];
    const float su = std::sqrt(rng.unit()), b1 = 1.0f - su, b2 = rng.unit() * su;
    float n[3] = { t[1] * t[5] - t[2] * t[4], t[2] * t[3] - t[0] * t[5], t[0] * t[4] - t[1] * t[3] };
    const float len = std::sqrt(n[0] * n[0] + n[1] * n[1] + n[2] * n[2]);
    for (float& c : n) c /= len;
    const int m = std::fabs(n[0]) <= std::fabs(n[1]) && std::fabs(n[0]) <= std::fabs(n[2]) ? 0 : (std::fabs(n[1]) <= std::fabs(n[2]) ? 1 : 2);
    float a[3] = { 0.f, 0.f, 0.f };
    a[m] = 1.0f;
    float tx[3] = { n[1] * a[2] - n[2] * a[1], n[2] * a[0] - n[0] * a[2], n[0] * a[1] - n[1] * a[0] };
    const float tl = std::sqrt(tx[0] * tx[0] + tx[1] * tx[1] + tx[2] * tx[2]);
    for (float& c : tx) c /= tl;
    const float ty[3] = { n[1] * tx[2] - n[2] * tx[1], n[2] * tx[0] - n[0] * tx[2], n[0] * tx[1] - n[1] * tx[0] };
    float dx, dy, rr;
    do { dx = 2.0f * rng.unit() - 1.0f; dy = 2.0f * rng.unit() - 1.0f; rr = dx * dx + dy * dy; } while (rr >= 1.0f);
    const float dz = std::sqrt(1.0f - rr);
    float* ray = &rays[(size_t)r * 6];
    for (int k = 0; k < 3; ++k) {
      ray[k] = dx * tx[k] + dy * ty[k] + dz * n[k];
      ray[3 + k] = (t[6 + k] + b1 * t[k] + b2 * t[3 + k]) + 0.03f * ray[k];
    }
  }
  return true;
}

}

void select_skip_nodes(const Bvh& bvh, float threshold, std::vector<uint8_t>& skip, uint32_t rays_per_node)
{
  const uint32_t N = bvh.n_nodes;
  skip.assign(N, 0);
  const uint32_t n_rays = rays_per_node * N;
  std::vector<float> rays;
  if (N < 3u || !training_rays(bvh, n_rays, rays)) return;
  std::vector<uint32_t> words, visits(N), passes(N);
  for (;;) {
    skip_link_table(bvh, skip, words);
    std::fill(visits.begin(), visits.end(), 0u);
    std::fill(passes.begin(), passes.end(), 0u);
    for (uint32_t r = 0; r < n_rays; ++r) {
      skip_count_host(bvh, words.data(), &rays[(size_t)r * 6], &rays[(size_t)r * 6 + 3], visits.data(), passes.data());
    }
    bool added = false;
    for (uint32_t n = 0; n < N; ++n) {
      if (skip[n] || node_of(bvh, n).count || visits[n] < kSkipMinVisits) continue;
      if ((float)passes[n] > threshold * (float)visits[n]) { skip[n] = 1; added = true; }
    }
    if (!added) return;
  }
}

namespace {

uint32_t rays_knob(uint32_t rule_default)
{
  const char* e = tuning_env("PTAMD_SKIP_RAYS");
  const int v = e ? std::atoi(e) : 0;
  return v < 1 ? rule_default : ((uint32_t)v > kSkipMaxRaysPerNode ? kSkipMaxRaysPerNode : (uint32_t)v);
}

}

void skip_set_of(const Bvh& bvh, uint32_t mode, float threshold, const uint8_t* given, std::vector<uint8_t>& skip, uint32_t rays_per_node)
{
  const uint32_t N = bvh.n_nodes;
  skip.assign(N, 0);
  if (mode == PTAMD_SKIP_DEFAULT) select_skip_nodes(bvh, threshold > 0.0f ? threshold : kSkipThreshold, skip, rays_per_node ? rays_per_node : rays_knob(kSkipRaysPerNode));
  for (uint32_t n = 0; n < N; ++n) {
    if (node_of(bvh, n).count) { skip[n] = 0; continue; }
    if (mode == PTAMD_SKIP_ALL || (mode == PTAMD_SKIP_ROOT && n == 0u) || (mode == PTAMD_SKIP_SET && given && given[n])) skip[n] = 1;
  }
}

void build_skip_tables(const Bvh& bvh, uint32_t mode, float threshold, const uint8_t* given, SkipTables& out)
{
  out = SkipTables();
  const char* knob = tuning_env("PTAMD_SKIP_CULL");
  if ((mode & PTAMD_SKIP_CULLED) && !(knob && std::atoi(knob) == 0)) {
    out.n_culled = cull_table(bvh, out.cull);
    if (!out.n_culled) out.cull.clear();
  }
  skip_set_of(bvh, mode & 0xFFu, threshold, given, out.skip);
  for (uint8_t k : out.skip) out.n_skipped += k;
  skip_link_table(bvh, out.skip, out.words, out.cull.empty() ? nullptr : &out.cull);
}

}
```

cuda-pathtracer_amd/native.py:

```python
from __future__ import annotations

import ctypes as C
import os
import sys

_HERE = os.path.dirname(os.path.abspath(__file__))
LIB_PATH = os.path.join(_HERE, "libptamd.so")


class PtamdError(RuntimeError):

    def __init__(self, status: int, message: str):
        super().__init__(f"ptamd status {status}: {message}")
        self.status = status


PTAMD_OK, PTAMD_ERR_ARG, PTAMD_ERR_HIP, PTAMD_ERR_IO, PTAMD_ERR_LIMIT = 0, 1, 2, 3, 4
KERNEL_AUTO, KERNEL_BRUTE_FORCE, KERNEL_BVH, KERNEL_BVH_PERSISTENT, KERNEL_BVH_BLOCKWISE, KERNEL_BVH_SPLIT, KERNEL_BVH_RESTART = 0, 1, 2, 3, 4, 5, 6
KERNEL_BVH_RESTART_FMA = 7


class Float3(C.Structure):
    _fields_ = [("x", C.c_float), ("y", C.c_float), ("z", C.c_float)]

# ... 122 lines not shown

DENOISE_HISTORY_BYTES = 100


class AdaptiveView(C.Structure):
    _fields_ = [("width", C.c_uint32), ("height", C.c_uint32), ("counts", C.c_void_p), ("moments", C.c_void_p),
                ("list", C.c_void_p), ("active_count", C.c_void_p)]


class AdaptiveDesc(C.Structure):
    _fields_ = [("surface_rgba8", C.c_void_p), ("temporal_framebuffer", C.c_void_p), ("stream", C.c_void_p),
                ("camera", Camera), ("scene_id", C.c_uint32), ("cubemap_id", C.c_uint32), ("width", C.c_uint32),
                ("height", C.c_uint32), ("bounces", C.c_uint32), ("post_id", C.c_uint32), ("kernel", C.c_uint32),
                ("state", C.c_void_p), ("min_spp", C.c_uint32), ("max_spp", C.c_uint32), ("samples_per_round", C.c_uint32),
                ("rounds", C.c_uint32), ("threshold", C.c_float), ("err_floor", C.c_float), ("dilate", C.c_uint32),
                ("active_counts", C.c_void_p)]


ADAPTIVE_ERR_FLOOR = 0.01


TABLE_NODES, TABLE_TRIS_BVH, TABLE_NODES4, TABLE_TRIS_BRUTE, TABLE_SHADE, TABLE_SCALARS = 0, 1, 2, 3, 4, 5
TABLE_NAMES = ("nodes", "tris_bvh", "nodes4", "tris_brute", "shade")

FEATURE_MISS, FEATURE_MESH, FEATURE_LIGHT = 0, 1, 2
FEATURE_BYTES = 32
DENOISE_MAX_LEVELS = 8

assert C.sizeof(Face) == 112 and C.sizeof(Material) == 16 and C.sizeof(Light) == 32 and C.sizeof(Camera) == 64

IMAGE_LOAD_FN = C.CFUNCTYPE(C.c_int, C.c_void_p, C.c_char_p, C.POINTER(C.c_int32), C.POINTER(C.c_int32),
                            C.POINTER(C.c_int32), C.POINTER(C.POINTER(C.c_float)))
IMAGE_FREE_FN = C.CFUNCTYPE(None, C.c_void_p, C.POINTER(C.c_float))
LOAD_FIX_BACKSLASHES, LOAD_NO_IMAGES = 1, 2

SIGNATURES = {
    "ptamd_get_last_error": (C.c_char_p, []),
    "ptamd_version": (C.c_char_p, []),
    "ptamd_build_id": (C.c_char_p, []),
    "ptamd_host_scene_load": (C.c_int, [C.c_char_p, C.c_uint32, C.POINTER(C.c_void_p)]),
    "ptamd_host_scene_load_ex": (C.c_int, [C.c_char_p, C.c_uint32, IMAGE_LOAD_FN, IMAGE_FREE_FN, C.c_void_p,
                                            C.POINTER(C.c_void_p)]),
    "ptamd_image_loadf": (C.c_int, [C.c_char_p, C.POINTER(C.c_int32), C.POINTER(C.c_int32), C.POINTER(C.c_int32),
                                    C.POINTER(C.POINTER(C.c_float))]),
    "ptamd_image_load8": (C.c_int, [C.c_char_p, C.POINTER(C.c_int32), C.POINTER(C.c_int32), C.POINTER(C.c_int32),
                                    C.POINTER(C.POINTER(C.c_uint8))]),
    "ptamd_image_free": (None, [C.c_void_p]),
    "ptamd_image_save_png": (C.c_int, [C.c_char_p, C.POINTER(C.c_uint8), C.c_int32, C.c_int32, C.c_int32]),
    "ptamd_image_resize_float": (C.c_int, [C.POINTER(C.c_float), C.c_int32, C.c_int32, C.POINTER(C.c_float), C.c_int32, C.c_int32,
                                           C.c_int32]),
    "ptamd_host_scene_unloaded_count": (C.c_uint32, [C.c_void_p]),
    "ptamd_host_scene_unloaded_name": (C.c_char_p, [C.c_void_p, C.c_uint32]),
    "ptamd_host_scene_free": (None, [C.c_void_p]),
    "ptamd_host_scene_desc": (C.c_int, [C.c_void_p, C.POINTER(SceneDesc)]),
    "ptamd_host_scene_camera": (C.c_int, [C.c_void_p, C.POINTER(Camera)]),
    "ptamd_host_scene_cubemap": (C.c_char_p, [C.c_void_p]),
    "ptamd_cubemap_from_color": (C.c_int, [C.c_uint32, C.POINTER(C.c_float)]),
    "ptamd_cubemap_from_cross": (C.c_int, [C.POINTER(C.c_float), C.c_uint32, C.c_uint32, C.c_uint32,
                                           C.POINTER(C.c_float), C.POINTER(C.c_uint32)]),
    "ptamd_create": (C.c_int, [C.c_int32, C.POINTER(C.c_void_p)]),
    "ptamd_destroy": (None, [C.c_void_p]),
    "ptamd_upload_scene": (C.c_int, [C.c_void_p, C.POINTER(SceneDesc), C.POINTER(C.c_uint32)]),
    "ptamd_scene_update": (C.c_int, [C.c_void_p, C.POINTER(SceneUpdateDesc)]),
    "ptamd_scene_update_device": (C.c_int, [C.c_void_p, C.POINTER(SceneUpdateDeviceDesc)]),
    "ptamd_scene_rig_create": (C.c_int, [C.c_void_p, C.c_uint32, C.POINTER(Face), C.c_uint32, C.POINTER(C.c_uint32), C.c_uint32,
                                         C.POINTER(C.c_void_p)]),
    "ptamd_scene_rig_pose": (C.c_int, [C.c_void_p, C.POINTER(SceneRigPoseDesc)]),
    "ptamd_scene_rig_faces": (C.c_int, [C.c_void_p, C.POINTER(C.c_void_p)]),
    "ptamd_scene_rig_destroy": (C.c_int, [C.c_void_p, C.c_void_p]),
    "ptamd_host_pose_faces": (C.c_int, [C.POINTER(Face), C.c_uint32, C.POINTER(C.c_uint32), C.c_uint32, C.POINTER(C.c_float),
                                        C.POINTER(C.c_float), C.POINTER(Face)]),
    "ptamd_scene_rig_attach_skin": (C.c_int, [C.c_void_p, C.c_void_p, C.POINTER(C.c_uint16), C.POINTER(C.c_float), C.c_uint32]),
    "ptamd_scene_rig_skin": (C.c_int, [C.c_void_p, C.POINTER(SceneRigSkinDesc)]),
    "ptamd_host_skin_faces": (C.c_int, [C.POINTER(Face), C.c_uint32, C.POINTER(C.c_uint16), C.POINTER(C.c_float), C.c_uint32,
                                        C.POINTER(C.c_float), C.POINTER(C.c_float), C.POINTER(Face)]),
    "ptamd_scene_rig_attach_morphs": (C.c_int, [C.c_void_p, C.c_void_p, C.POINTER(MorphTarget), C.c_uint32]),
    "ptamd_scene_rig_morph": (C.c_int, [C.c_void_p, C.POINTER(SceneRigMorphDesc)]),
    "ptamd_host_morph_faces": (C.c_int, [C.POINTER(Face), C.c_uint32, C.POINTER(MorphTarget), C.c_uint32, C.POINTER(C.c_float),
                                         C.POINTER(Face)]),
    "ptamd_scene_update_lights": (C.c_int, [C.c_void_p, C.POINTER(SceneLightsDesc)]),
    "ptamd_scene_quality": (C.c_int, [C.c_void_p, C.c_uint32, C.c_void_p, C.POINTER(SceneQualityInfo)]),
    "ptamd_host_scene_quality": (C.c_int, [C.POINTER(SceneDesc), C.POINTER(Face), C.POINTER(C.c_double)]),
    "ptamd_scene_margins": (C.c_int, [C.c_void_p, C.c_uint32, C.POINTER(C.c_float)]),
    "ptamd_scene_release": (C.c_int, [C.c_void_p, C.c_uint32]),
    "ptamd_scene_table_read": (C.c_int, [C.c_void_p, C.c_uint32, C.c_uint32, C.c_void_p, C.POINTER(C.c_uint64)]),
    "ptamd_host_scene_refit": (C.c_int, [C.POINTER(SceneDesc), C.POINTER(Face), C.POINTER(Face), C.c_uint32, C.c_void_p,
                                         C.POINTER(C.c_uint64)]),
    "ptamd_host_bvh_refit_trace": (C.c_int, [C.POINTER(Face), C.POINTER(Face), C.c_uint32, C.POINTER(C.c_float), C.c_uint32,
                                             C.POINTER(C.c_int32), C.POINTER(C.c_int32)]),
    "ptamd_upload_cubemap": (C.c_int, [C.c_void_p, C.POINTER(C.c_float), C.c_uint32, C.POINTER(C.c_uint32)]),
    "ptamd_setup_function_tables": (C.c_int, [C.c_void_p]),
    "ptamd_raytrace": (C.c_int, [C.c_void_p, C.c_void_p, C.c_uint32, C.c_uint32, C.POINTER(Camera), C.c_uint32,
                                 C.c_uint32, C.c_void_p, C.c_void_p, C.c_int32, C.c_uint32]),
    "ptamd_raytrace_ex": (C.c_int, [C.c_void_p, C.POINTER(Launch)]),
    "ptamd_reset_frame_counter": (C.c_int, [C.c_void_p]),
    "ptamd_wang_hash": (C.c_uint32, [C.c_uint32]),
    "ptamd_interleaved_rows": (C.c_uint32, [C.c_uint32, C.c_uint32, C.c_uint32, C.c_uint32]),
    "ptamd_release_captured": (C.c_int, [C.c_void_p, C.c_void_p]),
    "ptamd_raytrace_stats": (C.c_int, [C.c_void_p, C.POINTER(Launch), C.POINTER(TraceStats)]),
    "ptamd_scene_info_get": (C.c_int, [C.c_void_p, C.c_uint32, C.POINTER(SceneInfo)]),
    "ptamd_scene_desc_is_flat": (C.c_int, [C.POINTER(SceneDesc), C.POINTER(C.c_int32)]),
    "ptamd_scene_is_flat": (C.c_int, [C.c_void_p, C.c_uint32, C.c_uint32, C.POINTER(C.c_int32)]),
    "ptamd_set_timeline": (C.c_int, [C.c_void_p, C.c_uint32]),
    "ptamd_read_timeline": (C.c_int, [C.c_void_p, C.POINTER(C.c_uint64), C.c_uint32, C.POINTER(C.c_uint32)]),
    "ptamd_device_error_count": (C.c_int, [C.c_void_p, C.POINTER(C.c_uint64)]),
    "ptamd_phase_cycles": (C.c_int, [C.c_void_p, C.POINTER(C.c_uint64)]),
    "ptamd_gamma_table_selftest": (C.c_int, [C.c_void_p, C.POINTER(C.c_uint64), C.POINTER(C.c_uint64)]),
    "ptamd_trace_rays": (C.c_int, [C.c_void_p, C.c_uint32, C.c_uint32, C.POINTER(C.c_float), C.c_uint32,
                                   C.POINTER(C.c_int32)]),
    "ptamd_host_bvh_trace": (C.c_int, [C.POINTER(Face), C.c_uint32, C.POINTER(C.c_float), C.c_uint32,
                                       C.POINTER(C.c_int32), C.POINTER(C.c_uint64)]),
    "ptamd_host_bvh4_trace": (C.c_int, [C.POINTER(Face), C.c_uint32, C.POINTER(C.c_float), C.c_uint32,
                                       C.POINTER(C.c_int32), C.POINTER(C.c_uint64)]),
    "ptamd_host_bvh4q_trace": (C.c_int, [C.POINTER(Face), C.c_uint32, C.POINTER(C.c_float), C.c_uint32,
                                       C.POINTER(C.c_int32), C.POINTER(C.c_uint64)]),
    "ptamd_host_bvh8_trace": (C.c_int, [C.POINTER(Face), C.c_uint32, C.POINTER(C.c_float), C.c_uint32,
                                       C.POINTER(C.c_int32), C.POINTER(C.c_uint64)]),
    "ptamd_host_origin_reach": (C.c_int, [C.POINTER(Face), C.c_uint32, C.POINTER(Light), C.c_uint32, C.POINTER(C.c_float)]),
    "ptamd_trace_rays_queue": (C.c_int, [C.c_void_p, C.c_uint32, C.c_void_p, C.c_uint32, C.c_void_p, C.c_uint32, C.c_uint32, C.c_void_p,
                                        C.POINTER(C.c_uint32)]),
    "ptamd_denoise": (C.c_int, [C.c_void_p, C.POINTER(DenoiseDesc)]),
    "ptamd_render_features": (C.c_int, [C.c_void_p, C.c_uint32, C.c_uint32, C.POINTER(Camera), C.c_uint32, C.c_uint32,
                                        C.c_void_p, C.c_void_p, C.c_void_p]),
    "ptamd_host_denoise": (C.c_int, [C.c_void_p, C.c_void_p, C.POINTER(DenoiseDesc), C.c_void_p, C.c_void_p]),
    "ptamd_get_frame_counter": (C.c_int, [C.c_void_p, C.POINTER(C.c_uint32)]),
    "ptamd_denoise_history_create": (C.c_int, [C.c_void_p, C.c_uint32, C.c_uint32, C.POINTER(C.c_void_p)]),
    "ptamd_denoise_history_destroy": (C.c_int, [C.c_void_p, C.c_void_p]),
    "ptamd_denoise_history_reset": (C.c_int, [C.c_void_p, C.c_void_p, C.c_void_p]),
    "ptamd_denoise_history_view_of": (C.c_int, [C.c_void_p, C.POINTER(DenoiseHistoryView)]),
    "ptamd_denoise_temporal": (C.c_int, [C.c_void_p, C.POINTER(DenoiseTemporalDesc)]),
    "ptamd_host_denoise_temporal": (C.c_int, [C.c_void_p, C.c_void_p, C.POINTER(DenoiseTemporalDesc), C.POINTER(DenoiseHistoryView),
                                              C.c_void_p, C.c_void_p]),
    "ptamd_adaptive_create": (C.c_int, [C.c_void_p, C.c_uint32, C.c_uint32, C.POINTER(C.c_void_p)]),
    "ptamd_adaptive_destroy": (C.c_int, [C.c_void_p, C.c_void_p]),
    "ptamd_adaptive_reset": (C.c_int, [C.c_void_p, C.c_void_p, C.c_void_p]),
    "ptamd_adaptive_view_of": (C.c_int, [C.c_void_p, C.POINTER(AdaptiveView)]),
    "ptamd_render_adaptive": (C.c_int, [C.c_void_p, C.POINTER(AdaptiveDesc)]),
    "ptamd_adaptive_select": (C.c_int, [C.c_void_p, C.POINTER(AdaptiveDesc)]),
    "ptamd_adaptive_resolve": (C.c_int, [C.c_void_p, C.POINTER(AdaptiveDesc), C.c_void_p]),
    "ptamd_host_adaptive_select": (C.c_int, [C.POINTER(AdaptiveDesc), C.c_void_p, C.c_void_p, C.c_void_p, C.c_void_p]),
    "ptamd_device_alloc": (C.c_int, [C.c_void_p, C.c_size_t, C.POINTER(C.c_void_p)]),
    "ptamd_device_free": (C.c_int, [C.c_void_p, C.c_void_p]),
    "ptamd_device_memset": (C.c_int, [C.c_void_p, C.c_void_p, C.c_int, C.c_size_t, C.c_void_p]),
    "ptamd_device_to_host": (C.c_int, [C.c_void_p, C.c_void_p, C.c_void_p, C.c_size_t, C.c_void_p]),
    "ptamd_host_to_device": (C.c_int, [C.c_void_p, C.c_void_p, C.c_void_p, C.c_size_t, C.c_void_p]),
    "ptamd_stream_synchronize": (C.c_int, [C.c_void_p, C.c_void_p]),
    "ptamd_scene_skip_count": (C.c_int, [C.c_void_p, C.c_uint32, C.POINTER(C.c_uint32)]),
    "ptamd_host_skip_trace": (C.c_int, [C.POINTER(Face), C.POINTER(Face), C.c_uint32, C.c_uint32, C.c_float, C.c_void_p,
                                        C.POINTER(C.c_float), C.c_uint32, C.POINTER(C.c_int32), C.POINTER(C.c_uint64),
                                        C.POINTER(C.c_uint32), C.c_void_p, C.c_void_p]),
    "ptamd_scene_cull_count": (C.c_int, [C.c_void_p, C.c_uint32, C.POINTER(C.c_uint32)]),
    "ptamd_last_restart_form": (C.c_int, [C.c_void_p, C.POINTER(C.c_int32)]),
    "ptamd_host_faces_away": (C.c_int, [C.c_void_p, C.c_uint32, C.c_void_p]),
}

_lib = None


def load() -> C.CDLL:
    global _lib
    if _lib is not None:
        return _lib
    if "torch" not in sys.modules and os.environ.get("PTAMD_NO_TORCH_PRELOAD") != "1":
        try:
            import torch
        except Exception:
            pass
    if not os.path.exists(LIB_PATH):
        raise ImportError(
            f"{LIB_PATH} is missing: the HIP library has not been built. "
            "Run `python -c \"import __graft_entry__ as g; g.build()\"` (or `make lib`). "
            "There is no CPU fallback for the render path.")
    lib = C.CDLL(LIB_PATH)
    for name, (res, args) in SIGNATURES.items():
        fn = getattr(lib, name)
        fn.restype = res
        fn.argtypes = args
    _lib = lib
    return lib


def check(status: int) -> None:
    if status != PTAMD_OK:
        raise PtamdError(status, load().ptamd_get_last_error().decode("utf-8", "replace"))
```

cuda-pathtracer_amd/render.py:

```python
from __future__ import annotations

import ctypes as C
from typing import Optional

import numpy as np

from . import native as N
from .scene import FACE_DTYPE, LIGHT_DTYPE, HostScene

POST_NONE, POST_GRAYSCALE, POST_SEPIA, POST_INVERT = 0, 1, 2, 3
REFERENCE_BOUNCES = 3


def _ptr(buf) -> int:
    if isinstance(buf, int):
        return buf
    if hasattr(buf, "data_ptr"):
        if not buf.is_cuda:
            raise ValueError("output buffers must live in device memory (no CPU path exists)")
        if not buf.is_contiguous():
            raise ValueError("output buffers must be contiguous")
        return buf.data_ptr()
    raise TypeError(f"unsupported buffer type {type(buf)!r}")


def _stream_handle(stream) -> int:
    if stream is None:
        return 0
    if isinstance(stream, int):
        return stream
    return int(stream.cuda_stream)


class Context:

    def __init__(self, device: int = 0):
        self._lib = N.load()
        h = C.c_void_p()
        N.check(self._lib.ptamd_create(device, C.byref(h)))
        self._h = h
        self.device = device

    def close(self) -> None:
        if getattr(self, "_h", None):
            self._lib.ptamd_destroy(self._h)
            self._h = None

    def __del__(self):
        try:
            self.close()
        except Exception:
            pass

    def __enter__(self):
        return self

    def __exit__(self, *exc):
        self.close()

    def upload_scene(self, scene: HostScene) -> int:
        d = scene.desc()
        sid = C.c_uint32()
        N.check(self._lib.ptamd_upload_scene(self._h, C.byref(d), C.byref(sid)))
        return sid.value

    def update_scene(self, scene_id: int, faces, stream=None) -> None:
        faces = np.ascontiguousarray(faces.faces if isinstance(faces, HostScene) else faces, dtype=FACE_DTYPE)
        d = N.SceneUpdateDesc()
        d.scene_id = scene_id
        d.faces = faces.ctypes.data_as(C.POINTER(N.Face)); d.n_faces = len(faces)
        d.stream = _stream_handle(stream)
        N.check(self._lib.ptamd_scene_update(self._h, C.byref(d)))

    def update_scene_device(self, scene_id: int, faces, stream=None) -> None:
        import torch
        if not isinstance(faces, torch.Tensor):
            raise ValueError("update_scene_device takes a torch tensor in device memory (host arrays: update_scene)")
        if not faces.is_cuda:
            raise ValueError("update_scene_device takes a tensor in device memory (CPU tensors: update_scene)")
        if faces.device.index != self.device:
            raise ValueError(f"the faces live on {faces.device}, the context on device {self.device}")
        if not ((faces.dtype == torch.float32 and faces.dim() == 2 and faces.shape[1] == 28) or
                (faces.dtype == torch.uint8 and faces.dim() == 2 and faces.shape[1] == 112)):
            raise ValueError("faces must be float32 of shape (n, 28) or uint8 of shape (n, 112)")
        if not faces.is_contiguous():
            raise ValueError("faces must be contiguous")
        d = N.SceneUpdateDeviceDesc()
        d.scene_id = scene_id
        d.faces = faces.data_ptr(); d.n_faces = faces.shape[0]
        d.stream = _stream_handle(stream)
        N.check(self._lib.ptamd_scene_update_device(self._h, C.byref(d)))

    def scene_rig(self, scene_id: int, host_scene, group_sizes=None) -> "SceneRig":
        return SceneRig(self, scene_id, host_scene, group_sizes)

    def update_lights(self, scene_id: int, lights, stream=None) -> None:
        lights = np.ascontiguousarray(lights.lights if isinstance(lights, HostScene) else lights, dtype=LIGHT_DTYPE)
        d = N.SceneLightsDesc()
        d.scene_id = scene_id
        d.lights = lights.ctypes.data_as(C.POINTER(N.Light)); d.n_lights = len(lights)
        d.stream = _stream_handle(stream)
        N.check(self._lib.ptamd_scene_update_lights(self._h, C.byref(d)))

    def scene_quality(self, scene_id: int, stream=None):
        q = N.SceneQualityInfo()
        N.check(self._lib.ptamd_scene_quality(self._h, scene_id, _stream_handle(stream), C.byref(q)))
        return q.built, q.now

    def scene_margins(self, scene_id: int) -> np.ndarray:
        out = (C.c_float * 4)()
        N.check(self._lib.ptamd_scene_margins(self._h, scene_id, out))
        return np.array(out[:], dtype=np.float32)

    def release_scene(self, scene_id: int) -> None:
        N.check(self._lib.ptamd_scene_release(self._h, scene_id))

    def read_scene_tables(self, scene_id: int) -> dict:
        out = {}
        for which, name in enumerate(N.TABLE_NAMES):
            n = C.c_uint64(0)
            N.check(self._lib.ptamd_scene_table_read(self._h, scene_id, which, None, C.byref(n)))
            buf = np.zeros(n.value, np.uint8)
            N.check(self._lib.ptamd_scene_table_read(self._h, scene_id, which, buf.ctypes.data, C.byref(n)))
            out[name] = buf
        return out

    def upload_cubemap(self, faces: np.ndarray) -> int:
        faces = np.ascontiguousarray(faces, dtype=np.float32)
        if faces.ndim != 4 or faces.shape[0] != 6 or faces.shape[1] != faces.shape[2] or faces.shape[3] != 4:
            raise ValueError("cubemap must be float32[6, size, size, 4]")
        cid = C.c_uint32()
        N.check(self._lib.ptamd_upload_cubemap(self._h, faces.ctypes.data_as(C.POINTER(C.c_float)),
                                               faces.shape[1], C.byref(cid)))
        return cid.value

    def setup_function_tables(self) -> None:
        N.check(self._lib.ptamd_setup_function_tables(self._h))

    def scene_info(self, scene_id: int) -> dict:
        info = N.SceneInfo()
        N.check(self._lib.ptamd_scene_info_get(self._h, scene_id, C.byref(info)))
        return {n: getattr(info, n) for n, _ in N.SceneInfo._fields_}

    def scene_skip_count(self, scene_id: int) -> int:
        out = C.c_uint32(0)
        N.check(self._lib.ptamd_scene_skip_count(self._h, scene_id, C.byref(out)))
        return out.value

    def scene_cull_count(self, scene_id: int) -> int:
        out = C.c_uint32(0)
        N.check(self._lib.ptamd_scene_cull_count(self._h, scene_id, C.byref(out)))
        return out.value

    def last_restart_form(self) -> int:
        out = C.c_int32(-1)
        N.check(self._lib.ptamd_last_restart_form(self._h, C.byref(out)))
        return out.value

    def scene_is_flat(self, scene_id: int, cubemap_id: int) -> bool:
        out = C.c_int32()
        N.check(self._lib.ptamd_scene_is_flat(self._h, scene_id, cubemap_id, C.byref(out)))
        return out.value != 0

    def raytrace(self, array, scene_id: int, cubemap_id: int, cam: N.Camera, width: int, height: int,
                 stream, temporal_framebuffer, moved: bool, post_id: int) -> None:
        N.check(self._lib.ptamd_raytrace(self._h, _ptr(array), scene_id, cubemap_id, C.byref(cam), width, height,
                                         _stream_handle(stream), _ptr(temporal_framebuffer),
                                         1 if moved else 0, post_id))

    def reset_frame_counter(self) -> None:
        N.check(self._lib.ptamd_reset_frame_counter(self._h))

    def make_launch(self, array, temporal_framebuffer, scene_id: int, cubemap_id: int, cam: N.Camera,
                    width: int, height: int, frame_nb: int, bounces: int = REFERENCE_BOUNCES,
                    moved: bool = False, post_id: int = POST_NONE, stream=None,
                    rows: Optional[tuple] = None, kernel: int = N.KERNEL_AUTO,
                    band_local_buffers: bool = False, frame_count: int = 1, machine_share: int = 0,
                    interleave: Optional[tuple] = None, reset_accumulation: bool = False, no_pipelining: bool = False) -> N.Launch:
        l = N.Launch()
        l.surface_rgba8 = _ptr(array)
        l.temporal_framebuffer = _ptr(temporal_framebuffer)
        l.stream = _stream_handle(stream)
        l.camera = cam
        l.scene_id, l.cubemap_id = scene_id, cubemap_id
        l.width, l.height = width, height
        l.row_begin, l.row_end = rows if rows is not None else (0, height)
        l.frame_nb, l.bounces = frame_nb, bounces
        l.moved, l.post_id, l.kernel = (1 if moved else 0), post_id, kernel
        l.band_local_buffers = 1 if band_local_buffers else 0
        l.frame_count = frame_count
        l.machine_share = machine_share
        if interleave is not None:
            l.interleave_ranks, l.interleave_rank, l.interleave_rows = interleave
        l.reset_accumulation = 1 if reset_accumulation else 0
        l.no_pipelining = 1 if no_pipelining else 0
        return l

    def raytrace_ex(self, launch: N.Launch) -> None:
        N.check(self._lib.ptamd_raytrace_ex(self._h, C.byref(launch)))

    def frame_counter(self) -> int:
        out = C.c_uint32()
        N.check(self._lib.ptamd_get_frame_counter(self._h, C.byref(out)))
        return out.value

    def denoise(self, surface, temporal_framebuffer, scene_id: int, cubemap_id: int, cam: N.Camera, width: int, height: int,
                frame_nb: int, levels: int = 5, post_id: int = POST_NONE, sigma_n: float = 0.0, sigma_l: float = 0.0,
                sigma_x: float = 0.0, linear=None, stream=None) -> None:
        d = N.DenoiseDesc()
        d.temporal_framebuffer = _ptr(temporal_framebuffer)
        d.frame_nb = frame_nb
        d.camera = cam
        d.scene_id, d.cubemap_id, d.width, d.height = scene_id, cubemap_id, width, height
        d.surface_rgba8 = _ptr(surface)
        d.linear_rgb = _ptr(linear) if linear is not None else None
        d.stream = _stream_handle(stream)
        d.post_id, d.levels = post_id, levels
        d.sigma_n, d.sigma_l, d.sigma_x = sigma_n, sigma_l, sigma_x
        N.check(self._lib.ptamd_denoise(self._h, C.byref(d)))

    def adaptive_state(self, width: int, height: int) -> "AdaptiveState":
        return AdaptiveState(self, width, height)

    def denoise_history(self, width: int, height: int) -> "DenoiseHistory":
        return DenoiseHistory(self, width, height)

    def denoise_temporal(self, surface, temporal_framebuffer, scene_id: int, cubemap_id: int, cam: N.Camera, width: int,
                         height: int, frame_nb: int, history: "DenoiseHistory", levels: int = 5, post_id: int = POST_NONE,
                         sigma_n: float = 0.0, sigma_l: float = 0.0, sigma_x: float = 0.0, alpha_color: float = 0.0,
                         alpha_moments: float = 0.0, reset_history: bool = False, history_length=None, linear=None,
                         stream=None) -> None:
        if history.ctx is not self:
            raise ValueError("the history belongs to another context")
        d = N.DenoiseTemporalDesc()
        b = d.base
        b.temporal_framebuffer = _ptr(temporal_framebuffer)
        b.frame_nb = frame_nb
        b.camera = cam
        b.scene_id, b.cubemap_id, b.width, b.height = scene_id, cubemap_id, width, height
        b.surface_rgba8 = _ptr(surface)
        b.linear_rgb = _ptr(linear) if linear is not None else None
        b.stream = _stream_handle(stream)
        b.post_id, b.levels = post_id, levels
        b.sigma_n, b.sigma_l, b.sigma_x = sigma_n, sigma_l, sigma_x
        d.history = history.handle
        d.alpha_color, d.alpha_moments = alpha_color, alpha_moments
        d.reset_history = 1 if reset_history else 0
        d.history_length = _ptr(history_length) if history_length is not None else None
        N.check(self._lib.ptamd_denoise_temporal(self._h, C.byref(d)))

    def render_features(self, scene_id: int, cubemap_id: int, cam: N.Camera, width: int, height: int, features,
                        rays=None, stream=None) -> None:
        N.check(self._lib.ptamd_render_features(self._h, scene_id, cubemap_id, C.byref(cam), width, height, _ptr(features),
                                                _ptr(rays) if rays is not None else None, _stream_handle(stream)))

    def trace_rays_queue(self, scene_id: int, rays, out, config: int = 0, refill_min: int = 8, stream=None) -> int:
        waves = C.c_uint32(0)
        N.check(self._lib.ptamd_trace_rays_queue(self._h, scene_id, _ptr(rays), int(rays.shape[0]), _ptr(out), config, refill_min,
                                                 _stream_handle(stream), C.byref(waves)))
        return int(waves.value)

    def release_captured(self, stream=None) -> None:
        N.check(self._lib.ptamd_release_captured(self._h, _stream_handle(stream)))

    def raytrace_stats(self, launch: N.Launch) -> dict:
        st = N.TraceStats()
        N.check(self._lib.ptamd_raytrace_stats(self._h, C.byref(launch), C.byref(st)))
        return {n: getattr(st, n) for n, _ in N.TraceStats._fields_}

    def phase_cycles(self) -> dict:
        v = (C.c_uint64 * 12)()
        N.check(self._lib.ptamd_phase_cycles(self._h, v))
        d = dict(zip(("refill", "box_phases", "leaf_phases", "light_loop", "round_loop", "leaf_phases_entered", "node_fetches", "visits", "shading_record_fetch", "path_post_and_parking", "path_post_to_bsdf", "bsdf_sample"), [int(x) for x in v]))
        d["lights_and_shading"] = d["round_loop"] - d["refill"] - d["box_phases"] - d["leaf_phases"]
        return d

    def trace_rays(self, scene_id: int, rays: np.ndarray, kernel: int = N.KERNEL_BVH) -> np.ndarray:
        rays = np.ascontiguousarray(rays, dtype=np.float32)
        out = np.zeros((len(rays), 4), dtype=np.int32)
        N.check(self._lib.ptamd_trace_rays(self._h, scene_id, kernel, rays.ctypes.data_as(C.POINTER(C.c_float)),
                                           len(rays), out.ctypes.data_as(C.POINTER(C.c_int32))))
        return out

    def set_timeline(self, max_waves: int) -> None:
        N.check(self._lib.ptamd_set_timeline(self._h, max_waves))

    def read_timeline(self, n_waves: int):
        out = np.zeros((n_waves, 4), dtype=np.uint64)
        khz = C.c_uint32()
        N.check(self._lib.ptamd_read_timeline(self._h, out.ctypes.data_as(C.POINTER(C.c_uint64)), n_waves, C.byref(khz)))
        return out, khz.value

    def gamma_table_selftest(self):
        n, bad = C.c_uint64(), C.c_uint64()
        N.check(self._lib.ptamd_gamma_table_selftest(self._h, C.byref(n), C.byref(bad)))
        return n.value, bad.value

    def device_error_count(self) -> int:
        v = C.c_uint64()
        N.check(self._lib.ptamd_device_error_count(self._h, C.byref(v)))
        return v.value

    def synchronize(self, stream=None) -> None:
        N.check(self._lib.ptamd_stream_synchronize(self._h, _stream_handle(stream)))

# ... 20 lines not shown
        n = C.c_uint64(0)
        N.check(lib.ptamd_host_scene_refit(C.byref(d), ptrs[0], ptrs[1], which, None, C.byref(n)))
        buf = np.zeros(n.value, np.uint8)
        N.check(lib.ptamd_host_scene_refit(C.byref(d), ptrs[0], ptrs[1], which, buf.ctypes.data, C.byref(n)))
        out[name] = buf.view(np.float32) if name == "scalars" else buf
    return out


def _pose_arrays(n_groups: int, transforms, normal_matrices):
    t = np.ascontiguousarray(transforms, dtype=np.float32).reshape(-1)
    if t.size != n_groups * 12:
        raise ValueError(f"transforms must hold {n_groups} x 12 floats (row-major 3x4 each)")
    m = None
    if normal_matrices is not None:
        m = np.ascontiguousarray(normal_matrices, dtype=np.float32).reshape(-1)
        if m.size != n_groups * 9:
            raise ValueError(f"normal_matrices must hold {n_groups} x 9 floats (row-major 3x3 each)")
    return t, m


def host_pose_faces(hs: HostScene, transforms, normal_matrices=None, group_sizes=None) -> HostScene:
    sizes = np.ascontiguousarray(hs.mesh_sizes if group_sizes is None else group_sizes, dtype=np.uint32)
    t, m = _pose_arrays(len(sizes), transforms, normal_matrices)
    out = np.zeros(len(hs.faces), dtype=FACE_DTYPE)
    fp = C.POINTER(C.c_float)
    N.check(N.load().ptamd_host_pose_faces(hs.faces.ctypes.data_as(C.POINTER(N.Face)), len(hs.faces),
                                           sizes.ctypes.data_as(C.POINTER(C.c_uint32)), len(sizes), t.ctypes.data_as(fp),
                                           m.ctypes.data_as(fp) if m is not None else None, out.ctypes.data_as(C.POINTER(N.Face))))
    return HostScene(out, hs.mesh_sizes, hs.materials, hs.lights, hs.textures, hs.texels, hs.camera, hs.cubemap, hs.unloaded_textures)


def _skin_arrays(n_faces: int, indices, weights):
    idx = np.asarray(indices)
    if idx.size and (idx.min() < 0 or idx.max() > 65535):
        raise ValueError("a bone index does not fit 16 bits")
    idx = np.ascontiguousarray(idx, dtype=np.uint16).reshape(-1)
    w = np.ascontiguousarray(weights, dtype=np.float32).reshape(-1)
    if idx.size != n_faces * 12 or w.size != n_faces * 12:
        raise ValueError(f"indices and weights must hold {n_faces} x 3 x 4 values (four influences per corner)")
    return idx, w


def host_skin_faces(hs: HostScene, indices, weights, transforms, normal_matrices=None) -> HostScene:
    idx, w = _skin_arrays(len(hs.faces), indices, weights)
    n_bones = np.asarray(transforms).size // 12
    t, m = _pose_arrays(n_bones, transforms, normal_matrices)
    out = np.zeros(len(hs.faces), dtype=FACE_DTYPE)
    fp = C.POINTER(C.c_float)
    N.check(N.load().ptamd_host_skin_faces(hs.faces.ctypes.data_as(C.POINTER(N.Face)), len(hs.faces), idx.ctypes.data_as(C.POINTER(C.c_uint16)),
                                           w.ctypes.data_as(fp), n_bones, t.ctypes.data_as(fp), m.ctypes.data_as(fp) if m is not None else None,
                                           out.ctypes.data_as(C.POINTER(N.Face))))
    return HostScene(out, hs.mesh_sizes, hs.materials, hs.lights, hs.textures, hs.texels, hs.camera, hs.cubemap, hs.unloaded_textures)


def _morph_targets(targets):
    keep, arr = [], (N.MorphTarget * max(len(targets), 1))()
    for t, (faces, deltas) in enumerate(targets):
        f = np.asarray(faces)
        if f.dtype != np.uint32 and f.size and (f.min() < 0 or f.max() > 0xffffffff):
            raise ValueError("a face index does not fit 32 bits")
        f = np.ascontiguousarray(f, dtype=np.uint32).reshape(-1)
        d = np.ascontiguousarray(deltas, dtype=np.float32).reshape(-1)
        if d.size != f.size * 18:
            raise ValueError(f"target {t}: deltas must hold 18 floats for each of its {f.size} faces")
        keep.append((f, d))
        arr[t].faces = f.ctypes.data_as(C.POINTER(C.c_uint32)) if f.size else None
        arr[t].deltas = d.ctypes.data_as(C.POINTER(C.c_float)) if f.size else None
        arr[t].n_entries = f.size
    return arr, keep


def host_morph_faces(hs: HostScene, targets, weights) -> HostScene:
    arr, keep = _morph_targets(targets)
    w = np.ascontiguousarray(weights, dtype=np.float32).reshape(-1)
    if w.size != len(targets):
        raise ValueError(f"weights must hold one float for each of the {len(targets)} targets")
    out = np.zeros(len(hs.faces), dtype=FACE_DTYPE)
    N.check(N.load().ptamd_host_morph_faces(hs.faces.ctypes.data_as(C.POINTER(N.Face)), len(hs.faces), arr, len(targets),
                                            w.ctypes.data_as(C.POINTER(C.c_float)), out.ctypes.data_as(C.POINTER(N.Face))))
    return HostScene(out, hs.mesh_sizes, hs.materials, hs.lights, hs.textures, hs.texels, hs.camera, hs.cubemap, hs.unloaded_textures)


def host_scene_quality(scene: HostScene, faces_b=None) -> float:
    ptr = None
    if faces_b is not None:
        fb = np.ascontiguousarray(faces_b.faces if isinstance(faces_b, HostScene) else faces_b, dtype=FACE_DTYPE)
        if len(fb) != len(scene.faces):
            raise ValueError("a refit keeps the face count")
        ptr = fb.ctypes.data_as(C.POINTER(N.Face))
    d = scene.desc()
    out = C.c_double(0.0)
    N.check(N.load().ptamd_host_scene_quality(C.byref(d), ptr, C.byref(out)))
    return out.value


def host_bvh_refit_trace(scene_a: HostScene, scene_b: HostScene, rays: np.ndarray):
    rays = np.ascontiguousarray(rays, dtype=np.float32)
    if len(scene_a.faces) != len(scene_b.faces):
        raise ValueError("a refit keeps the face count")
    out = np.zeros((2, len(rays), 4), dtype=np.int32)
    N.check(N.load().ptamd_host_bvh_refit_trace(scene_a.faces.ctypes.data_as(C.POINTER(N.Face)),
                                                scene_b.faces.ctypes.data_as(C.POINTER(N.Face)), len(scene_a.faces),
                                                rays.ctypes.data_as(C.POINTER(C.c_float)), len(rays),
                                                out[0].ctypes.data_as(C.POINTER(C.c_int32)), out[1].ctypes.data_as(C.POINTER(C.c_int32))))
    return out[0], out[1]


def host_bvh_trace(scene: HostScene, rays: np.ndarray):
    rays = np.ascontiguousarray(rays, dtype=np.float32)
    out = np.zeros((len(rays), 4), dtype=np.int32)
    counters = (C.c_uint64 * 2)(0, 0)
    N.check(N.load().ptamd_host_bvh_trace(scene.faces.ctypes.data_as(C.POINTER(N.Face)), len(scene.faces),
                                          rays.ctypes.data_as(C.POINTER(C.c_float)), len(rays),
                                          out.ctypes.data_as(C.POINTER(C.c_int32)), counters))
    return out, counters[0], counters[1]


SKIP_MODES = {"set": 0, "default": 1, "root": 2, "all": 3}
SKIP_CULLED = 0x100
FORM_FLAT_SKIP, FORM_PLAIN_SKIP = 9, 10


def host_faces_away(edges: np.ndarray) -> np.ndarray:
    edges = np.ascontiguousarray(edges, dtype=np.float32).reshape(-1, 6)
    out = np.zeros(len(edges), dtype=np.uint8)
    N.check(N.load().ptamd_host_faces_away(edges.ctypes.data, len(edges), out.ctypes.data))
    return out


def host_skip_trace(scene: HostScene, rays: np.ndarray, mode="default", skip=None, threshold: float = 0.0, refit_to=None, cull=False) -> dict:
    rays = np.ascontiguousarray(rays, dtype=np.float32).reshape(-1, 6)
    lib = N.load()
    faces = scene.faces.ctypes.data_as(C.POINTER(N.Face))
    fb = None
    if refit_to is not None:
        fb = np.ascontiguousarray(refit_to.faces if isinstance(refit_to, HostScene) else refit_to, dtype=FACE_DTYPE)
        if len(fb) != len(scene.faces):
            raise ValueError("a refit keeps the face count")
    fb_ptr = fb.ctypes.data_as(C.POINTER(N.Face)) if fb is not None else None
    given = None if skip is None else np.ascontiguousarray(skip, dtype=np.uint8)
    n_nodes = C.c_uint32(0)
    N.check(lib.ptamd_host_skip_trace(faces, None, len(scene.faces), 0, 0.0, None, None, 0, None, None, C.byref(n_nodes), None, None))
    if given is not None and len(given) != n_nodes.value:
        raise ValueError("skip holds one byte per node")
    out = np.zeros((len(rays), 4), dtype=np.int32)
    skip_out = np.zeros(n_nodes.value, dtype=np.uint8)
    words = np.zeros((n_nodes.value + 1, 8), dtype=np.uint32)
    counters = (C.c_uint64 * 3)(0, 0, 0)
    N.check(lib.ptamd_host_skip_trace(faces, fb_ptr, len(scene.faces), SKIP_MODES[mode] | (SKIP_CULLED if cull else 0), threshold,
                                      given.ctypes.data if given is not None else None,
                                      rays.ctypes.data_as(C.POINTER(C.c_float)), len(rays), out.ctypes.data_as(C.POINTER(C.c_int32)),
                                      counters, C.byref(n_nodes), skip_out.ctypes.data, words.ctypes.data))
    return {"records": out, "nodes": counters[0], "tris": counters[1], "skip": skip_out, "words": words}


def host_bvh4_trace(scene: HostScene, rays: np.ndarray):
    rays = np.ascontiguousarray(rays, dtype=np.float32)
    out = np.zeros((len(rays), 4), dtype=np.int32)
    counters = (C.c_uint64 * 5)(0, 0, 0, 0, 0)
    N.check(N.load().ptamd_host_bvh4_trace(scene.faces.ctypes.data_as(C.POINTER(N.Face)), len(scene.faces),
                                           rays.ctypes.data_as(C.POINTER(C.c_float)), len(rays),
                                           out.ctypes.data_as(C.POINTER(C.c_int32)), counters))
    host_bvh4_trace.top_visits = (counters[3], counters[4])
    return out, counters[0], counters[1], counters[2]


def host_bvh4q_trace(scene: HostScene, rays: np.ndarray):
    rays = np.ascontiguousarray(rays, dtype=np.float32)
    out = np.zeros((len(rays), 4), dtype=np.int32)
    counters = (C.c_uint64 * 5)(0, 0, 0, 0, 0)
    N.check(N.load().ptamd_host_bvh4q_trace(scene.faces.ctypes.data_as(C.POINTER(N.Face)), len(scene.faces),
                                            rays.ctypes.data_as(C.POINTER(C.c_float)), len(rays),
                                            out.ctypes.data_as(C.POINTER(C.c_int32)), counters))
    host_bvh4q_trace.top_visits = (counters[3], counters[4])
    return out, counters[0], counters[1], counters[2]


def host_bvh8_trace(scene: HostScene, rays: np.ndarray):
    rays = np.ascontiguousarray(rays, dtype=np.float32)
    out = np.zeros((len(rays), 4), dtype=np.int32)
    counters = (C.c_uint64 * 6)(0, 0, 0, 0, 0, 0)
    N.check(N.load().ptamd_host_bvh8_trace(scene.faces.ctypes.data_as(C.POINTER(N.Face)), len(scene.faces),
                                           rays.ctypes.data_as(C.POINTER(C.c_float)), len(rays),
                                           out.ctypes.data_as(C.POINTER(C.c_int32)), counters))
    host_bvh8_trace.top_visits = (counters[3], counters[4])
    return out, counters[0], counters[1], counters[2], counters[5]


def host_denoise(features: np.ndarray, accum: np.ndarray, cam: N.Camera, frame_nb: int, levels: int = 5,
                 post_id: int = POST_NONE, sigma_n: float = 0.0, sigma_l: float = 0.0, sigma_x: float = 0.0):
    features = np.ascontiguousarray(features, dtype=np.float32)
    accum = np.ascontiguousarray(accum, dtype=np.float32)
    h, w = accum.shape[:2]
    if features.shape != (h, w, 8):
        raise ValueError(f"features must be float32[{h}, {w}, 8]")
    d = N.DenoiseDesc()
    d.frame_nb, d.camera, d.width, d.height = frame_nb, cam, w, h
    d.post_id, d.levels = post_id, levels
    d.sigma_n, d.sigma_l, d.sigma_x = sigma_n, sigma_l, sigma_x
    linear = np.zeros((h, w, 3), np.float32)
    rgba = np.zeros((h, w, 4), np.uint8)
    N.check(N.load().ptamd_host_denoise(features.ctypes.data, accum.ctypes.data, C.byref(d), linear.ctypes.data, rgba.ctypes.data))
    return linear, rgba


def _is_tensor(x) -> bool:
    return type(x).__module__.startswith("torch")


def _device_tensor(ctx, name: str, x, per: int, what: str) -> None:
    if not x.is_cuda:
        raise ValueError(f"{name} must live in device memory (CPU tensors: pass numpy arrays)")
    if x.device.index != ctx.device:
        raise ValueError(f"{name} lives on {x.device}, the context on device {ctx.device}")
    if str(x.dtype) != "torch.float32" or not x.is_contiguous() or x.numel() % per:
        raise ValueError(f"{name} must be contiguous float32 of {per} values a {what}")


def _device_transforms(ctx, transforms, normal_matrices) -> int:
    for name, x, per_bone in (("transforms", transforms, 12), ("normal_matrices", normal_matrices, 9)):
        if x is None and per_bone == 9:
            continue
        if not _is_tensor(x):
            raise ValueError("transforms and normal_matrices are both tensors or both host arrays")
        _device_tensor(ctx, name, x, per_bone, "bone")
    n = transforms.numel() // 12
    if normal_matrices is not None and normal_matrices.numel() != n * 9:
        raise ValueError("normal_matrices must hold n_bones x 9 floats")
    return n


def _rig_transforms(ctx, transforms, normal_matrices, device_route=True):
    if device_route and (_is_tensor(transforms) or _is_tensor(normal_matrices)):
        n = _device_transforms(ctx, transforms, normal_matrices)
        return transforms.data_ptr(), normal_matrices.data_ptr() if normal_matrices is not None else None, n, True, None
    n = np.asarray(transforms).size // 12
    keep = _pose_arrays(n, transforms, normal_matrices)
    return keep[0].ctypes.data, keep[1].ctypes.data if keep[1] is not None else None, n, False, keep


class SceneRig:

    def __init__(self, ctx: Context, scene_id: int, host_scene, group_sizes=None):
        faces = np.ascontiguousarray(host_scene.faces if isinstance(host_scene, HostScene) else host_scene, dtype=FACE_DTYPE)
        if group_sizes is None:
            if not isinstance(host_scene, HostScene):
                raise ValueError("group_sizes is needed with a bare face array")
            group_sizes = host_scene.mesh_sizes
        sizes = np.ascontiguousarray(group_sizes, dtype=np.uint32)
        self.ctx, self.scene_id, self.n_faces, self.n_groups = ctx, scene_id, len(faces), len(sizes)
        h = C.c_void_p()
        N.check(ctx._lib.ptamd_scene_rig_create(ctx._h, scene_id, faces.ctypes.data_as(C.POINTER(N.Face)), len(faces),
                                                sizes.ctypes.data_as(C.POINTER(C.c_uint32)), len(sizes), C.byref(h)))
        self.handle = h.value

    def pose(self, transforms, normal_matrices=None, stream=None) -> None:
        t, m, n, _, keep = _rig_transforms(self.ctx, transforms, normal_matrices, device_route=False)
        d = N.SceneRigPoseDesc()
        d.rig, d.n_groups, d.stream = self.handle, n, _stream_handle(stream)
        d.transforms, d.normal_matrices = C.cast(t, C.POINTER(C.c_float)), C.cast(m, C.POINTER(C.c_float))
        N.check(self.ctx._lib.ptamd_scene_rig_pose(self.ctx._h, C.byref(d)))

    def attach_skin(self, indices, weights, n_bones: int) -> None:
        idx, w = _skin_arrays(self.n_faces, indices, weights)
        N.check(self.ctx._lib.ptamd_scene_rig_attach_skin(self.ctx._h, self.handle, idx.ctypes.data_as(C.POINTER(C.c_uint16)),
                                                          w.ctypes.data_as(C.POINTER(C.c_float)), n_bones))

    def skin(self, transforms, normal_matrices=None, stream=None) -> None:
        d = N.SceneRigSkinDesc()
        d.rig = self.handle
        d.stream = _stream_handle(stream)
        d.transforms, d.normal_matrices, d.n_bones, on_device, keep = _rig_transforms(self.ctx, transforms, normal_matrices)
        d.flags = N.SKIN_DEVICE_TRANSFORMS if on_device else 0
        N.check(self.ctx._lib.ptamd_scene_rig_skin(self.ctx._h, C.byref(d)))

    def attach_morphs(self, targets) -> None:
        arr, keep = _morph_targets(targets)
        N.check(self.ctx._lib.ptamd_scene_rig_attach_morphs(self.ctx._h, self.handle, arr, len(targets)))

    def morph(self, weights, then=None, transforms=None, normal_matrices=None, stream=None) -> None:
        thens = {None: N.MORPH_THEN_NOTHING, "pose": N.MORPH_THEN_POSE, "skin": N.MORPH_THEN_SKIN}
        if then not in thens:
            raise ValueError('then is None, "pose" or "skin"')
        if (then is None) != (transforms is None):
            raise ValueError("transforms go with then=\"pose\" or then=\"skin\", and only with them")
        d = N.SceneRigMorphDesc()
        d.rig, d.then, d.flags, d.stream = self.handle, thens[then], 0, _stream_handle(stream)
        if _is_tensor(weights):
            _device_tensor(self.ctx, "weights", weights, 1, "target")
            d.weights, d.n_targets = weights.data_ptr(), weights.numel()
            d.flags |= N.MORPH_DEVICE_WEIGHTS
        else:
            w = np.ascontiguousarray(weights, dtype=np.float32).reshape(-1)
            d.weights, d.n_targets = w.ctypes.data, w.size
        if then != "skin" and (_is_tensor(transforms) or _is_tensor(normal_matrices)):
            raise ValueError("device transforms go with then=\"skin\" only")
        if transforms is not None:
            d.transforms, d.normal_matrices, d.n_transforms, on_device, keep = _rig_transforms(self.ctx, transforms, normal_matrices)
            d.flags |= N.MORPH_DEVICE_TRANSFORMS if on_device else 0
        N.check(self.ctx._lib.ptamd_scene_rig_morph(self.ctx._h, C.byref(d)))

    def faces(self) -> np.ndarray:
        p = C.c_void_p()
        N.check(self.ctx._lib.ptamd_scene_rig_faces(self.handle, C.byref(p)))
        out = np.zeros(self.n_faces, dtype=FACE_DTYPE)
        import torch
# ... 329 lines not shown
```

include/ptamd.h:

```cpp
#ifndef PTAMD_H
#define PTAMD_H

#include <stddef.h>
#include <stdint.h>

#ifdef __cplusplus
extern "C" {
#endif

typedef enum {
  PTAMD_OK = 0,
  PTAMD_ERR_ARG = 1,
  PTAMD_ERR_HIP = 2,
  PTAMD_ERR_IO = 3,
  PTAMD_ERR_LIMIT = 4
} ptamd_status;


typedef struct { float x, y, z; } ptamd_float3;
typedef struct { float x, y; } ptamd_float2;

typedef struct {
  ptamd_float3 vertices[3];
  ptamd_float3 normals[3];
// ... 262 lines not shown
                           uint32_t refill_min, void* stream, uint32_t* out_waves_per_cu);

int ptamd_host_bvh_trace(const ptamd_face* faces, uint32_t n_faces, const float* rays, uint32_t n,
                         int32_t* out, uint64_t* counters);

int ptamd_host_bvh4_trace(const ptamd_face* faces, uint32_t n_faces, const float* rays, uint32_t n,
                          int32_t* out, uint64_t* counters);
int ptamd_host_bvh4q_trace(const ptamd_face* faces, uint32_t n_faces, const float* rays, uint32_t n,
                           int32_t* out, uint64_t* counters);

int ptamd_host_bvh8_trace(const ptamd_face* faces, uint32_t n_faces, const float* rays, uint32_t n,
                          int32_t* out, uint64_t* counters);

int ptamd_host_origin_reach(const ptamd_face* faces, uint32_t n_faces, const ptamd_light* lights, uint32_t n_lights,
                            float* out);

int ptamd_scene_table_read(ptamd_context* ctx, uint32_t scene_id, uint32_t which, void* out, uint64_t* bytes);
int ptamd_scene_margins(ptamd_context* ctx, uint32_t scene_id, float out[4]);
int ptamd_host_scene_refit(const ptamd_scene_desc* scene, const ptamd_face* faces_b, const ptamd_face* faces_c, uint32_t which,
                           void* out, uint64_t* bytes);
int ptamd_host_bvh_refit_trace(const ptamd_face* faces_a, const ptamd_face* faces_b, uint32_t n_faces, const float* rays, uint32_t n,
                               int32_t* out_binary, int32_t* out_wide);

#define PTAMD_FEATURE_MISS 0u
#define PTAMD_FEATURE_MESH 1u
#define PTAMD_FEATURE_LIGHT 2u
#define PTAMD_DENOISE_MAX_LEVELS 8u

typedef struct {
  const float* temporal_framebuffer;
  uint32_t frame_nb;
  ptamd_camera camera;
  uint32_t scene_id, cubemap_id;
  uint32_t width, height;
  void* surface_rgba8;
  float* linear_rgb;
  void* stream;
  uint32_t post_id;
  uint32_t levels;
  float sigma_n;
  float sigma_l;
  float sigma_x;
} ptamd_denoise_desc;

int ptamd_denoise(ptamd_context* ctx, const ptamd_denoise_desc* desc);

int ptamd_render_features(ptamd_context* ctx, uint32_t scene_id, uint32_t cubemap_id, const ptamd_camera* camera,
                          uint32_t width, uint32_t height, void* features_dev, float* rays_dev, void* stream);

int ptamd_host_denoise(const float* features, const float* temporal_framebuffer, const ptamd_denoise_desc* desc,
                       float* linear_rgb, uint8_t* rgba8);

typedef struct ptamd_denoise_history ptamd_denoise_history;

int ptamd_denoise_history_create(ptamd_context* ctx, uint32_t width, uint32_t height, ptamd_denoise_history** out);
int ptamd_denoise_history_destroy(ptamd_context* ctx, ptamd_denoise_history* history);
int ptamd_denoise_history_reset(ptamd_context* ctx, ptamd_denoise_history* history, void* stream);

typedef struct {
  ptamd_denoise_desc base;
  ptamd_denoise_history* history;
  float alpha_color;
  float alpha_moments;
  uint32_t reset_history;
  float* history_length;
} ptamd_denoise_temporal_desc;

int ptamd_denoise_temporal(ptamd_context* ctx, const ptamd_denoise_temporal_desc* desc);

typedef struct {
  uint32_t width, height;
  uint32_t valid;
  uint32_t frame_nb;
  ptamd_camera camera;
  float* color;
  float* moments;
  float* normal;
  float* position;
} ptamd_denoise_history_view;

int ptamd_denoise_history_view_of(const ptamd_denoise_history* history, ptamd_denoise_history_view* out);

int ptamd_host_denoise_temporal(const float* features, const float* temporal_framebuffer, const ptamd_denoise_temporal_desc* desc,
                                ptamd_denoise_history_view* history, float* linear_rgb, uint8_t* rgba8);

typedef struct ptamd_adaptive_state ptamd_adaptive_state;

int ptamd_adaptive_create(ptamd_context* ctx, uint32_t width, uint32_t height, ptamd_adaptive_state** out);
int ptamd_adaptive_destroy(ptamd_context* ctx, ptamd_adaptive_state* state);
int ptamd_adaptive_reset(ptamd_context* ctx, ptamd_adaptive_state* state, void* stream);

typedef struct {
  uint32_t width, height;
  uint32_t* counts;
  float* moments;
  uint32_t* list;
  uint32_t* active_count;
} ptamd_adaptive_view;

int ptamd_adaptive_view_of(const ptamd_adaptive_state* state, ptamd_adaptive_view* out);

typedef struct {
  void* surface_rgba8;
  float* temporal_framebuffer;
  void* stream;
  ptamd_camera camera;
  uint32_t scene_id, cubemap_id;
  uint32_t width, height;
  uint32_t bounces;
  uint32_t post_id;
  uint32_t kernel;
  ptamd_adaptive_state* state;
  uint32_t min_spp, max_spp;
  uint32_t samples_per_round;
  uint32_t rounds;
  float threshold;
  float err_floor;
  uint32_t dilate;
  uint32_t* active_counts;
} ptamd_adaptive_desc;

int ptamd_render_adaptive(ptamd_context* ctx, const ptamd_adaptive_desc* desc);

int ptamd_adaptive_select(ptamd_context* ctx, const ptamd_adaptive_desc* desc);

int ptamd_adaptive_resolve(ptamd_context* ctx, const ptamd_adaptive_desc* desc, float* linear_rgb);

int ptamd_host_adaptive_select(const ptamd_adaptive_desc* desc, const uint32_t* counts, const float* moments, uint32_t* list,
                               uint32_t* active_count);

int ptamd_get_frame_counter(ptamd_context* ctx, uint32_t* out);

int ptamd_device_alloc(ptamd_context* ctx, size_t bytes, void** out);
int ptamd_device_free(ptamd_context* ctx, void* p);
int ptamd_device_memset(ptamd_context* ctx, void* p, int value, size_t bytes, void* stream);
int ptamd_device_to_host(ptamd_context* ctx, void* dst_host, const void* src_dev, size_t bytes, void* stream);
int ptamd_host_to_device(ptamd_context* ctx, void* dst_dev, const void* src_host, size_t bytes, void* stream);
int ptamd_stream_synchronize(ptamd_context* ctx, void* stream);

#define PTAMD_SKIP_SET 0u
#define PTAMD_SKIP_DEFAULT 1u
#define PTAMD_SKIP_ROOT 2u
#define PTAMD_SKIP_ALL 3u
#define PTAMD_SKIP_CULLED 0x100u
#define PTAMD_FORM_FLAT_SKIP 9
#define PTAMD_FORM_PLAIN_SKIP 10
int ptamd_scene_skip_count(ptamd_context* ctx, uint32_t scene_id, uint32_t* out);
int ptamd_scene_cull_count(ptamd_context* ctx, uint32_t scene_id, uint32_t* out);
int ptamd_last_restart_form(ptamd_context* ctx, int32_t* out);
int ptamd_host_skip_trace(const ptamd_face* faces, const ptamd_face* faces_refit, uint32_t n_faces, uint32_t mode, float threshold,
                          const uint8_t* skip_in, const float* rays, uint32_t n, int32_t* out, uint64_t* counters,
                          uint32_t* n_nodes, uint8_t* skip_out, uint32_t* words_out);
int ptamd_host_faces_away(const float* edges, uint32_t n, uint8_t* out);

#ifdef __cplusplus
}
#endif
#endif
```

Before: 14170.

## Choose BVH skip-link nodes per camera view from host-traced sample paths

Adds a view-dependent selection of BVH skip nodes. On the host it traces sample paths from the actual camera, then greedily picks nodes to skip when doing so lowers the expected number of box tests. The rebuilt link tables are uploaded before skip-form restart launches, and the selection is only recomputed when the camera or bounce count changes. A guard turns the feature off if the camera keeps changing. This adds host tracing work and an upload on the first frame, or whenever the view changes, in exchange for shorter GPU traversals.

Result: no change. 14310, median of 6 (+1.0%).

```diff
diff --git a/cuda-pathtracer_amd/__init__.py b/cuda-pathtracer_amd/__init__.py
--- a/cuda-pathtracer_amd/__init__.py
+++ b/cuda-pathtracer_amd/__init__.py
@@ -3,7 +3,7 @@
                      PtamdError)
 from .scene import (HostScene, cubemap_for_scene, cubemap_from_color, cubemap_from_cross,
                     FACE_DTYPE, MATERIAL_DTYPE, LIGHT_DTYPE, TEXTURE_DTYPE, CAMERA_DTYPE)
-from .render import (Context, FrameRenderer, SceneRig, host_pose_faces, host_skin_faces, host_morph_faces, AdaptiveState, host_adaptive_select, host_denoise, DenoiseHistory, HostDenoiseHistory, host_denoise_temporal, orbit_camera, host_bvh_trace, host_skip_trace, host_faces_away, FORM_FLAT_SKIP, FORM_PLAIN_SKIP, host_scene_tables, host_scene_quality, host_bvh_refit_trace, host_bvh4_trace, host_bvh4q_trace, host_bvh8_trace, origin_reach, interleaved_rows, wang_hash, REFERENCE_BOUNCES,
+from .render import (Context, FrameRenderer, SceneRig, host_pose_faces, host_skin_faces, host_morph_faces, AdaptiveState, host_adaptive_select, host_denoise, DenoiseHistory, HostDenoiseHistory, host_denoise_temporal, orbit_camera, host_bvh_trace, host_skip_trace, host_skip_view_trace, host_skip_view_guard, host_faces_away, FORM_FLAT_SKIP, FORM_PLAIN_SKIP, host_scene_tables, host_scene_quality, host_bvh_refit_trace, host_bvh4_trace, host_bvh4q_trace, host_bvh8_trace, origin_reach, interleaved_rows, wang_hash, REFERENCE_BOUNCES,
                      POST_NONE, POST_GRAYSCALE, POST_SEPIA, POST_INVERT)
 from .tiles import row_bands, band_of_rank, BandGather, interleaved_bands, rank_times_ms, time_gather_ms
 from .synthetic import tessellate, deform
diff --git a/cuda-pathtracer_amd/csrc/ptamd_host.h b/cuda-pathtracer_amd/csrc/ptamd_host.h
--- a/cuda-pathtracer_amd/csrc/ptamd_host.h
+++ b/cuda-pathtracer_amd/csrc/ptamd_host.h
@@ -41,6 +41,12 @@
   std::vector<uint8_t> skip_set, cull_bits;
   std::vector<uint32_t> link_words;
   PinnedBuffer<uint32_t> h_links[2];
+  bool view_ok = false;
+  SkipViewState view;
+  std::vector<uint8_t> skip_default;
+  PinnedBuffer<uint32_t> h_view;
+  Event view_staged;
+  bool view_staged_valid = false;
   float reach = 0.0f;
   float margin_floor = 0.0f;
   ptamd_scene_info info{};
@@ -161,6 +167,7 @@
 int settle_margins(DeviceScene& s, hipStream_t stream, const char* who);
 void fill_scene(const DeviceScene& s, const DeviceCubemap* cm, KParams& p);
 int wait_for_update(const DeviceScene& s, hipStream_t stream, bool capturing);
+int choose_view_links(ptamd_context* ctx, DeviceScene& s, const ptamd_launch* l, hipStream_t stream);
 int update_scene_checks(const char* who, const ptamd_context* ctx, uint32_t scene_id, uint32_t n_faces, const void* faces);
 int update_capture_checks(const char* who, const ptamd_context* ctx, hipStream_t stream);
 int wait_for_readers(const ptamd_context* ctx, const DeviceScene& s, hipStream_t stream);
diff --git a/cuda-pathtracer_amd/csrc/ptamd_launch.cpp b/cuda-pathtracer_amd/csrc/ptamd_launch.cpp
--- a/cuda-pathtracer_amd/csrc/ptamd_launch.cpp
+++ b/cuda-pathtracer_amd/csrc/ptamd_launch.cpp
@@ -402,12 +402,17 @@
   return PTAMD_OK;
 }
 
-int issue(ptamd_context* ctx, const DeviceScene& scene, bool stats, const AdaptiveParams* ad, const LaunchPlan& pl, KParams& p)
+int issue(ptamd_context* ctx, const ptamd_launch* l, bool stats, const AdaptiveParams* ad, const LaunchPlan& pl, KParams& p)
 {
   const bool split = pl.which == PTAMD_KERNEL_BVH_SPLIT, restart = pl.which == PTAMD_KERNEL_BVH_RESTART;
   ptamd_context::SampleScratch* sc = pl.sc;
-  int urc = wait_for_update(scene, pl.stream, pl.capturing);
-  if (urc != PTAMD_OK) return urc;
+  DeviceScene& scene = ctx->scenes[l->scene_id];
+  p.n_static = pl.n_blocks * pl.waves_per_block;
+  if (restart && !pl.fma && ctx->d_timeline && p.n_static <= ctx->timeline_waves) p.timeline = ctx->d_timeline.get();
+  const int restart_form = restart ? restart_select(pl.resident, stats, ad != nullptr, pl.fma, &p).variant : -1;
+  int urc = PTAMD_OK;
+  if ((restart_form == PT_RS_FLAT_SKIP || restart_form == PT_RS_PLAIN_SKIP) && !pl.capturing && (urc = choose_view_links(ctx, scene, l, pl.stream)) != PTAMD_OK) return urc;
+  if ((urc = wait_for_update(scene, pl.stream, pl.capturing)) != PTAMD_OK) return urc;
   p.round_min = ctx->knobs.round_min;
   p.round_div = ctx->knobs.round_div;
   p.round_div_m16 = (65536u + ctx->knobs.round_div - 1u) / ctx->knobs.round_div;
@@ -415,7 +420,6 @@
   p.walk_min4 = ctx->knobs.walk_min4;
   p.tile_counter = ctx->d_tickets.get() + pl.slot;
   if (ad) p.adaptive = ad->block;
-  p.n_static = pl.n_blocks * pl.waves_per_block;
   if (split) PT_HIP(hipMemsetD32Async(reinterpret_cast<hipDeviceptr_t>(p.tile_counter), (int)p.n_static, 1, pl.stream));
   hipStream_t mega_stream = pl.stream;
   if (pl.pipelined) {
@@ -429,9 +433,8 @@
     if (!ctx->heads_clean[pl.slot]) PT_HIP(hipMemsetD32Async(reinterpret_cast<hipDeviceptr_t>(p.tile_heads), 0, 8u * PT_HEAD_STRIDE, mega_stream));
     ctx->heads_clean[pl.slot] = false;
   }
-  if (restart && !pl.fma && ctx->d_timeline && p.n_static <= ctx->timeline_waves) p.timeline = ctx->d_timeline.get();
   if (split) p.tiles_per_ticket = 1;
-  ctx->last_restart_form = restart ? restart_select(pl.resident, stats, ad != nullptr, pl.fma, &p).variant : -1;
+  ctx->last_restart_form = restart_form;
   hipError_t e = launch_form(form_of(pl, stats, ad != nullptr, &p), p, pl.n_blocks, restart ? mega_stream : pl.stream);
   if (e == hipSuccess && pl.pipelined) {
     PT_HIP(hipEventRecord(sc->mega_done[pl.slab].get(), mega_stream));
@@ -474,7 +477,7 @@
       rc = bind_slab(ctx, l, pl, p);
     } while (rc == kReplan);
     if (rc != PTAMD_OK || (rc = take_slot(ctx, pl.capturing, pl.sc, pl.slot)) != PTAMD_OK) return rc;
-    return issue(ctx, ctx->scenes[l->scene_id], stats, ad, pl, p);
+    return issue(ctx, l, stats, ad, pl, p);
   }
   fill_launch(ctx, l, stats, pl, p);
   if (ctx->scenes[l->scene_id].updated_valid &&
diff --git a/cuda-pathtracer_amd/csrc/ptamd_scene.cpp b/cuda-pathtracer_amd/csrc/ptamd_scene.cpp
--- a/cuda-pathtracer_amd/csrc/ptamd_scene.cpp
+++ b/cuda-pathtracer_amd/csrc/ptamd_scene.cpp
@@ -328,6 +328,42 @@
   s.margin_ready_valid[slot] = true;
   s.margin_slot = slot;
   s.margins_pending = true;
+  return PTAMD_OK;
+}
+
+int choose_view_links(ptamd_context* ctx, DeviceScene& s, const ptamd_launch* l, hipStream_t stream)
+{
+  if (!s.view_ok || !ctx->knobs.skip_view) return PTAMD_OK;
+  for (const auto& c : ctx->sample_scratch) if (c.captured) return PTAMD_OK;
+  const int what = skip_view_decide(s.view, l->camera, l->bounces);
+  if (what == kSkipViewKeep) return PTAMD_OK;
+  std::vector<uint8_t> set(s.skip_default);
+  const std::vector<uint8_t>* cull = s.n_culled ? &s.cull_bits : nullptr;
+  if (what == kSkipViewSelect) {
+    const SkipView view = { l->camera, l->width, l->height, l->bounces };
+    (void)select_skip_nodes_view(s.topology, cull, view, set);
+  }
+  if (set == s.skip_set) return PTAMD_OK;
+  const size_t words = (size_t)s.n_nodes * 8 + 8;
+  if (!s.h_view) PT_HIP(s.h_view.alloc(2u * words * 4));
+  PT_HIP(s.view_staged.ensure());
+  PT_HIP(s.updated.ensure());
+  if (s.view_staged_valid) PT_HIP(hipEventSynchronize(s.view_staged.get()));
+  skip_link_table(s.topology, set, s.link_words);
+  std::memcpy(s.h_view.get() + words, s.link_words.data(), words * 4);
+  skip_link_table(s.topology, set, s.link_words, cull);
+  std::memcpy(s.h_view.get(), s.link_words.data(), words * 4);
+  const int rc = wait_for_readers(ctx, s, stream);
+  if (rc != PTAMD_OK) return rc;
+  if (s.links_plain) PT_HIP(hipMemcpyAsync(s.links_plain.get(), s.h_view.get() + words, words * 4, hipMemcpyHostToDevice, stream));
+  PT_HIP(hipMemcpyAsync(reinterpret_cast<float*>(s.nodes.get()) + (size_t)s.n_nodes * 16, s.h_view.get(), words * 4, hipMemcpyHostToDevice, stream));
+  PT_HIP(hipEventRecord(s.view_staged.get(), stream));
+  s.view_staged_valid = true;
+  PT_HIP(hipEventRecord(s.updated.get(), stream));
+  s.updated_valid = true;
+  s.skip_set.swap(set);
+  s.n_skipped = 0;
+  for (uint8_t k : s.skip_set) s.n_skipped += k;
   return PTAMD_OK;
 }
 
@@ -381,17 +417,22 @@
       nodes_and_links.resize(bvh.nodes.size() + t.words.size());
       std::memcpy(nodes_and_links.data() + bvh.nodes.size(), t.words.data(), t.words.size() * 4);
     }
+    if (d.links) {
+      d.topology.nodes = bvh.nodes;
+      d.topology.n_nodes = bvh.n_nodes; d.topology.n_tris = bvh.n_tris;
+      d.topology.tris = bvh.tris;
+      d.skip_set = t.skip;
+      d.skip_default = t.skip;
+      d.cull_bits = t.cull;
+      d.record_face.resize(bvh.n_tris);
+      for (uint32_t j = 0; j < bvh.n_tris; ++j) std::memcpy(&d.record_face[j], &bvh.tris[(size_t)j * 12 + 9], 4);
+      d.view_ok = mode == PTAMD_SKIP_DEFAULT;
+    }
     if (t.n_culled) {
       std::vector<uint32_t> plain;
       skip_link_table(bvh, t.skip, plain);
       if ((rc = upload(d.links_plain, plain.data(), plain.size() * 4))) return rc;
       d.cull_on = true;
-      d.topology.nodes = bvh.nodes;
-      d.topology.n_nodes = bvh.n_nodes; d.topology.n_tris = bvh.n_tris;
-      d.topology.tris.resize((size_t)bvh.n_tris * 12);
-      d.skip_set = t.skip;
-      d.record_face.resize(bvh.n_tris);
-      for (uint32_t j = 0; j < bvh.n_tris; ++j) std::memcpy(&d.record_face[j], &bvh.tris[(size_t)j * 12 + 9], 4);
     }
   }
   if ((rc = upload(d.nodes, nodes_and_links.data(), nodes_and_links.size() * 4)) ||
@@ -704,6 +745,14 @@
   return PTAMD_OK;
 }
 
+int ptamd_scene_skip_view_count(ptamd_context* ctx, uint32_t scene_id, uint32_t selections[2])
+{
+  if (!ctx || !selections || !live_scene(ctx, scene_id)) { set_error("ptamd_scene_skip_view_count: bad argument"); return PTAMD_ERR_ARG; }
+  selections[0] = ctx->scenes[scene_id].view.selections;
+  selections[1] = ctx->scenes[scene_id].view.off ? 1u : 0u;
+  return PTAMD_OK;
+}
+
 int ptamd_scene_cull_count(ptamd_context* ctx, uint32_t scene_id, uint32_t* out)
 {
   if (!ctx || !out || !live_scene(ctx, scene_id)) { set_error("ptamd_scene_cull_count: bad argument"); return PTAMD_ERR_ARG; }
diff --git a/cuda-pathtracer_amd/csrc/ptamd_tuning.cpp b/cuda-pathtracer_amd/csrc/ptamd_tuning.cpp
--- a/cuda-pathtracer_amd/csrc/ptamd_tuning.cpp
+++ b/cuda-pathtracer_amd/csrc/ptamd_tuning.cpp
@@ -52,6 +52,7 @@
   on_off("PTAMD_RS_FLAT", &S::flat_round),
   number("PTAMD_SKIP", kSkipWord, &S::skip_mode, 0, 0),
   { "PTAMD_SKIP_THRESHOLD", kOpenUnit, nullptr, nullptr, &S::skip_threshold, 0, 1 },
+  on_off("PTAMD_SKIP_VIEW", &S::skip_view),
   on_off("PTAMD_POOL_LDS", &S::pool_in_lds),
   on_off("PTAMD_POOL_LDS_WIDE", &S::pool_in_lds_wide),
   number("PTAMD_TREELET", kClamped, &S::treelet_nodes, 0, 1024),
diff --git a/cuda-pathtracer_amd/csrc/ptamd_tuning.h b/cuda-pathtracer_amd/csrc/ptamd_tuning.h
--- a/cuda-pathtracer_amd/csrc/ptamd_tuning.h
+++ b/cuda-pathtracer_amd/csrc/ptamd_tuning.h
@@ -20,6 +20,7 @@
   bool flat_round = true;
   uint32_t skip_mode = PTAMD_SKIP_DEFAULT;
   float skip_threshold = 0.0f;
+  bool skip_view = true;
   bool pool_in_lds = true;
   bool pool_in_lds_wide = false;
   uint32_t treelet_nodes = 512;
diff --git a/cuda-pathtracer_amd/host/bvh_walks.cpp b/cuda-pathtracer_amd/host/bvh_walks.cpp
--- a/cuda-pathtracer_amd/host/bvh_walks.cpp
+++ b/cuda-pathtracer_amd/host/bvh_walks.cpp
@@ -2,6 +2,7 @@
 
 #include <algorithm>
 #include <cmath>
+#include <cstdlib>
 #include <cstring>
 #include <limits>
 
@@ -243,7 +244,7 @@
 namespace {
 template <bool MIRROR>
 void skip_walk(const Bvh& bvh, const uint32_t* words, const float dir[3], const float origin[3], HostHit& out,
-               uint64_t* nodes_visited, uint64_t* tris_tested, uint32_t* node_visits, uint32_t* node_passes)
+               uint64_t* nodes_visited, uint64_t* tris_tested, uint32_t* node_visits, uint32_t* node_passes, std::vector<uint32_t>* trail = nullptr)
 {
   const Ray ray(dir, origin);
   const uint32_t oct = ray.octant();
@@ -268,6 +269,7 @@
     }
     const bool hit = tnear <= tfar && tfar >= 0.0f && tnear <= best.t;
     if (node_visits) { ++node_visits[node]; node_passes[node] += hit ? 1u : 0u; }
+    if (trail) trail->push_back(node | (hit ? 0x80000000u : 0u));
     const uint32_t word = words[(size_t)node * 8 + oct];
     uint32_t code = hit ? (word & 0xFFFFu) : (word >> 16);
     if (code >= 0x8000u && code != 0xFFFFu) {
@@ -290,6 +292,11 @@
 {
   HostHit h;
   skip_walk<false>(bvh, words, dir, origin, h, nullptr, nullptr, node_visits, node_passes);
+}
+
+void skip_trail_host(const Bvh& bvh, const uint32_t* words, const float dir[3], const float origin[3], HostHit& out, std::vector<uint32_t>& trail)
+{
+  skip_walk<false>(bvh, words, dir, origin, out, nullptr, nullptr, nullptr, nullptr, &trail);
 }
 
 }
@@ -408,6 +415,50 @@
   return PTAMD_OK;
 }
 
+extern "C" int ptamd_host_skip_view_trace(const ptamd_face* faces, uint32_t n_faces, const ptamd_camera* camera, uint32_t width, uint32_t height,
+                                          uint32_t bounces, const float* rays, uint32_t n, int32_t* out, uint64_t* counters,
+                                          uint32_t* n_nodes, uint8_t* skip_out, uint32_t* words_out)
+{
+  if ((n_faces && !faces) || !camera || (n && (!rays || !out)) || !n_nodes) { ptamd::set_error("ptamd_host_skip_view_trace: bad argument"); return PTAMD_ERR_ARG; }
+  ptamd::Bvh bvh;
+  const int rc = ptamd::build_bvh(faces, n_faces, 1e-3f, 2, bvh, 0u);
+  if (rc != PTAMD_OK) return rc;
+  if (!ptamd::skip_links_fit(bvh)) { ptamd::set_error("ptamd_host_skip_view_trace: the tree is outside the compact layout's code space"); return PTAMD_ERR_LIMIT; }
+  const uint32_t room = *n_nodes;
+  *n_nodes = bvh.n_nodes;
+  if ((skip_out || words_out) && room < bvh.n_nodes) { ptamd::set_error("ptamd_host_skip_view_trace: room for fewer nodes than the tree has"); return PTAMD_ERR_ARG; }
+  ptamd::SkipTables t;
+  ptamd::build_skip_tables(bvh, PTAMD_SKIP_DEFAULT | PTAMD_SKIP_CULLED, 0.0f, nullptr, t);
+  const char* knob = ptamd::tuning_env("PTAMD_SKIP_VIEW");
+  const ptamd::SkipView view = { *camera, width, height, bounces };
+  const std::vector<uint8_t>* cull = t.cull.empty() ? nullptr : &t.cull;
+  const bool chosen = !(knob && std::atoi(knob) == 0) && ptamd::select_skip_nodes_view(bvh, cull, view, t.skip);
+  if (chosen) ptamd::skip_link_table(bvh, t.skip, t.words, cull);
+  for (uint32_t i = 0; i < n; ++i) {
+    ptamd::HostHit h;
+    uint64_t visits = 0;
+    ptamd::skip_trace_host(bvh, t.words.data(), rays + (size_t)i * 6, rays + (size_t)i * 6 + 3, h, &visits, counters ? &counters[1] : nullptr);
+    if (counters) counters[0] += visits;
+    out[i * 4 + 0] = h.kind;
+    out[i * 4 + 1] = h.index;
+    std::memcpy(&out[i * 4 + 2], &h.t, 4);
+    out[i * 4 + 3] = (int32_t)visits;
+  }
+  if (counters) { counters[2] = 0; for (uint8_t k : t.skip) counters[2] += k; counters[3] = chosen ? 1u : 0u; }
+  if (skip_out && bvh.n_nodes) std::memcpy(skip_out, t.skip.data(), bvh.n_nodes);
+  if (words_out) std::memcpy(words_out, t.words.data(), t.words.size() * 4);
+  return PTAMD_OK;
+}
+
+extern "C" int ptamd_host_skip_view_guard(const ptamd_camera* cameras, const uint32_t* bounces, uint32_t n, uint8_t* decisions, uint32_t* selections)
+{
+  if (n && (!cameras || !bounces || !decisions)) { ptamd::set_error("ptamd_host_skip_view_guard: null argument"); return PTAMD_ERR_ARG; }
+  ptamd::SkipViewState st;
+  for (uint32_t i = 0; i < n; ++i) decisions[i] = (uint8_t)ptamd::skip_view_decide(st, cameras[i], bounces[i]);
+  if (selections) *selections = st.selections;
+  return PTAMD_OK;
+}
+
 extern "C" int ptamd_host_faces_away(const float* edges, uint32_t n, uint8_t* out)
 {
   if (n && (!edges || !out)) { ptamd::set_error("ptamd_host_faces_away: null argument"); return PTAMD_ERR_ARG; }
diff --git a/cuda-pathtracer_amd/host/ptamd_internal.h b/cuda-pathtracer_amd/host/ptamd_internal.h
--- a/cuda-pathtracer_amd/host/ptamd_internal.h
+++ b/cuda-pathtracer_amd/host/ptamd_internal.h
@@ -105,6 +105,18 @@
 void skip_link_table(const Bvh& bvh, const std::vector<uint8_t>& skip, std::vector<uint32_t>& words, const std::vector<uint8_t>* cull = nullptr);
 void skip_set_of(const Bvh& bvh, uint32_t mode, float threshold, const uint8_t* given, std::vector<uint8_t>& skip, uint32_t rays_per_node = 0u);
 void select_skip_nodes(const Bvh& bvh, float threshold, std::vector<uint8_t>& skip, uint32_t rays_per_node = kSkipRaysPerNode);
+struct SkipView { ptamd_camera camera; uint32_t width, height, bounces, paths_per_node = 0, min_visits = 0; };
+constexpr uint32_t kSkipViewPathsPerNode = 2u, kSkipViewMaxBounces = 8u, kSkipViewMinVisits = 4u, kSkipViewMinRays = 64u, kSkipViewTestsPerNode = 320u;
+constexpr float kSkipViewTailWeight = 1.0f;
+bool select_skip_nodes_view(const Bvh& bvh, const std::vector<uint8_t>* cull, const SkipView& view, std::vector<uint8_t>& skip, float tail_weight = kSkipViewTailWeight);
+struct SkipViewState {
+  bool have = false, off = false;
+  ptamd_camera camera{};
+  uint32_t bounces = 0, selections = 0, changes = 0;
+};
+constexpr uint32_t kSkipViewMaxChanges = 2u;
+enum { kSkipViewKeep = 0, kSkipViewSelect = 1, kSkipViewRevert = 2 };
+int skip_view_decide(SkipViewState& st, const ptamd_camera& camera, uint32_t bounces);
 struct SkipTables {
   std::vector<uint8_t> skip, cull;
   std::vector<uint32_t> words;
@@ -114,5 +126,6 @@
 void skip_trace_host(const Bvh& bvh, const uint32_t* words, const float dir[3], const float origin[3], HostHit& out,
                      uint64_t* nodes_visited, uint64_t* tris_tested, uint32_t* node_visits = nullptr, uint32_t* node_passes = nullptr);
 void skip_count_host(const Bvh& bvh, const uint32_t* words, const float dir[3], const float origin[3], uint32_t* node_visits, uint32_t* node_passes);
+void skip_trail_host(const Bvh& bvh, const uint32_t* words, const float dir[3], const float origin[3], HostHit& out, std::vector<uint32_t>& trail);
 
 }
diff --git a/cuda-pathtracer_amd/host/skip_links.cpp b/cuda-pathtracer_amd/host/skip_links.cpp
--- a/cuda-pathtracer_amd/host/skip_links.cpp
+++ b/cuda-pathtracer_amd/host/skip_links.cpp
@@ -1,5 +1,6 @@
 #include "ptamd_internal.h"
 
+#include <algorithm>
 #include <cmath>
 #include <cstdlib>
 #include <cstring>
@@ -129,6 +130,24 @@
 }
 
 namespace {
+
+void cosine_about_front(const float* t, Rng& rng, float out[3])
+{
+  float n[3] = { t[1] * t[5] - t[2] * t[4], t[2] * t[3] - t[0] * t[5], t[0] * t[4] - t[1] * t[3] };
+  const float len = std::sqrt(n[0] * n[0] + n[1] * n[1] + n[2] * n[2]);
+  for (float& c : n) c /= len;
+  const int m = std::fabs(n[0]) <= std::fabs(n[1]) && std::fabs(n[0]) <= std::fabs(n[2]) ? 0 : (std::fabs(n[1]) <= std::fabs(n[2]) ? 1 : 2);
+  float a[3] = { 0.f, 0.f, 0.f };
+  a[m] = 1.0f;
+  float tx[3] = { n[1] * a[2] - n[2] * a[1], n[2] * a[0] - n[0] * a[2], n[0] * a[1] - n[1] * a[0] };
+  const float tl = std::sqrt(tx[0] * tx[0] + tx[1] * tx[1] + tx[2] * tx[2]);
+  for (float& c : tx) c /= tl;
+  const float ty[3] = { n[1] * tx[2] - n[2] * tx[1], n[2] * tx[0] - n[0] * tx[2], n[0] * tx[1] - n[1] * tx[0] };
+  float dx, dy, rr;
+  do { dx = 2.0f * rng.unit() - 1.0f; dy = 2.0f * rng.unit() - 1.0f; rr = dx * dx + dy * dy; } while (rr >= 1.0f);
+  const float dz = std::sqrt(1.0f - rr);
+  for (int k = 0; k < 3; ++k) out[k] = dx * tx[k] + dy * ty[k] + dz * n[k];
+}
 
 bool training_rays(const Bvh& bvh, uint32_t n_rays, std::vector<float>& rays)
 {
@@ -152,22 +171,11 @@
     while (lo < hi) { const uint32_t mid = (lo + hi) / 2u; if (cdf[mid] > pick) hi = mid; else lo = mid + 1u; }
     const float* t = &bvh.tris[(size_t)lo * 12];
     const float su = std::sqrt(rng.unit()), b1 = 1.0f - su, b2 = rng.unit() * su;
-    float n[3] = { t[1] * t[5] - t[2] * t[4], t[2] * t[3] - t[0] * t[5], t[0] * t[4] - t[1] * t[3] };
-    const float len = std::sqrt(n[0] * n[0] + n[1] * n[1] + n[2] * n[2]);
-    for (float& c : n) c /= len;
-    const int m = std::fabs(n[0]) <= std::fabs(n[1]) && std::fabs(n[0]) <= std::fabs(n[2]) ? 0 : (std::fabs(n[1]) <= std::fabs(n[2]) ? 1 : 2);
-    float a[3] = { 0.f, 0.f, 0.f };
-    a[m] = 1.0f;
-    float tx[3] = { n[1] * a[2] - n[2] * a[1], n[2] * a[0] - n[0] * a[2], n[0] * a[1] - n[1] * a[0] };
-    const float tl = std::sqrt(tx[0] * tx[0] + tx[1] * tx[1] + tx[2] * tx[2]);
-    for (float& c : tx) c /= tl;
-    const float ty[3] = { n[1] * tx[2] - n[2] * tx[1], n[2] * tx[0] - n[0] * tx[2], n[0] * tx[1] - n[1] * tx[0] };
-    float dx, dy, rr;
-    do { dx = 2.0f * rng.unit() - 1.0f; dy = 2.0f * rng.unit() - 1.0f; rr = dx * dx + dy * dy; } while (rr >= 1.0f);
-    const float dz = std::sqrt(1.0f - rr);
+    float d[3];
+    cosine_about_front(t, rng, d);
     float* ray = &rays[(size_t)r * 6];
     for (int k = 0; k < 3; ++k) {
-      ray[k] = dx * tx[k] + dy * ty[k] + dz * n[k];
+      ray[k] = d[k];
       ray[3 + k] = (t[6 + k] + b1 * t[k] + b2 * t[3 + k]) + 0.03f * ray[k];
     }
   }
@@ -202,6 +210,204 @@
 
 namespace {
 
+double tan_by_series(double x)
+{
+  double sn = x, cs = 1.0, term_s = x, term_c = 1.0;
+  for (int k = 1; k <= 24; ++k) {
+    term_c = -term_c * x * x / (double)((2 * k - 1) * (2 * k));
+    term_s = -term_s * x * x / (double)((2 * k) * (2 * k + 1));
+    cs += term_c;
+    sn += term_s;
+  }
+  return sn / cs;
+}
+
+bool finite3(const ptamd_float3& v) { return std::fabs(v.x) < 1.0e30f && std::fabs(v.y) < 1.0e30f && std::fabs(v.z) < 1.0e30f; }
+
+struct ViewRays {
+  std::vector<uint32_t> trail, begin;
+  std::vector<uint8_t> half, octant;
+};
+bool view_rays(const Bvh& bvh, const uint32_t* words, const SkipView& view, ViewRays& out)
+{
+  const ptamd_camera& cam = view.camera;
+  if (!finite3(cam.position) || !finite3(cam.dir) || !(cam.fov_x >= 0.0f && cam.fov_x < 3.1f) || !view.width || !view.height || !view.bounces) return false;
+  const float dir[3] = { cam.dir.x, cam.dir.y, cam.dir.z };
+  float u[3] = { dir[2], 0.0f, -dir[0] };
+  const float ul = std::sqrt(u[0] * u[0] + u[2] * u[2]);
+  if (!(ul > 1.0e-30f)) return false;
+  for (float& c : u) c /= ul;
+  float v[3] = { u[1] * dir[2] - u[2] * dir[1], u[2] * dir[0] - u[0] * dir[2], u[0] * dir[1] - u[1] * dir[0] };
+  const float vl = std::sqrt(v[0] * v[0] + v[1] * v[1] + v[2] * v[2]);
+  if (!(vl > 1.0e-30f)) return false;
+  for (float& c : v) c /= vl;
+  const float half_w = (float)(view.width / 2u), half_h = (float)(view.height / 2u);
+  const float spread = (float)tan_by_series((double)cam.fov_x * 0.5);
+  const uint32_t want = bvh.n_nodes * (view.paths_per_node ? view.paths_per_node : kSkipViewPathsPerNode);
+  uint32_t gx = 1u;
+  while ((uint64_t)gx * gx * view.height < (uint64_t)want * view.width) ++gx;
+  const uint32_t gy = (want + gx - 1u) / gx;
+  const uint32_t depth = view.bounces < kSkipViewMaxBounces ? view.bounces : kSkipViewMaxBounces;
+  std::vector<uint32_t> record_of;
+  for (uint32_t i = 0; i < bvh.n_tris; ++i) {
+    const uint32_t f = f2u(bvh.tris[(size_t)i * 12 + 9]);
+    if (f >= record_of.size()) record_of.resize((size_t)f + 1u, 0xFFFFFFFFu);
+    if (record_of[f] == 0xFFFFFFFFu) record_of[f] = i;
+  }
+  out.trail.clear(); out.begin.assign(1, 0u); out.half.clear(); out.octant.clear();
+  out.trail.reserve((size_t)gx * gy * depth * 24u);
+  Rng rng = { 0xD1B54A32D192ED03ull };
+  const uint32_t cells = gx * gy;
+  uint32_t stride = (uint32_t)((uint64_t)cells * 618u / 1000u) | 1u;
+  const auto gcd = [](uint32_t a, uint32_t b) { while (b) { const uint32_t t = a % b; a = b; b = t; } return a; };
+  while (gcd(stride, cells) != 1u) stride += 2u;
+  const size_t limit = (size_t)bvh.n_nodes * kSkipViewTestsPerNode;
+  {
+    for (uint32_t cell = 0, at = 0; cell < cells && out.trail.size() < limit; ++cell, at = (uint32_t)(((uint64_t)at + stride) % cells)) {
+      const uint32_t i = at % gx, j = at / gx;
+      const float px = ((float)i + 0.5f) * (float)view.width / (float)gx - half_w, py = ((float)j + 0.5f) * (float)view.height / (float)gy - half_h;
+      float d[3], o[3] = { cam.position.x, cam.position.y, cam.position.z };
+      for (int k = 0; k < 3; ++k) d[k] = dir[k] * half_w + spread * (u[k] * px + v[k] * py);
+      const float dl = std::sqrt(d[0] * d[0] + d[1] * d[1] + d[2] * d[2]);
+      if (!(dl > 1.0e-30f) || !(dl < 1.0e30f)) return false;
+      for (float& c : d) c /= dl;
+      for (uint32_t b = 0; b < depth; ++b) {
+        HostHit h;
+        skip_trail_host(bvh, words, d, o, h, out.trail);
+        out.begin.push_back((uint32_t)out.trail.size());
+        out.half.push_back((uint8_t)((i + j) & 1u));
+        out.octant.push_back((uint8_t)((d[0] < 0.f ? 1u : 0u) | (d[1] < 0.f ? 2u : 0u) | (d[2] < 0.f ? 4u : 0u)));
+        if (h.kind != 1 || (uint32_t)h.index >= record_of.size() || record_of[(uint32_t)h.index] == 0xFFFFFFFFu) break;
+        const float* t = &bvh.tris[(size_t)record_of[(uint32_t)h.index] * 12];
+        float nd[3];
+        cosine_about_front(t, rng, nd);
+        bool ok = true;
+        for (int k = 0; k < 3; ++k) {
+          o[k] = (o[k] + h.t * d[k]) + 0.03f * nd[k];
+          ok = ok && nd[k] == nd[k];
+        }
+        if (!ok) break;
+        for (int k = 0; k < 3; ++k) d[k] = nd[k];
+      }
+    }
+  }
+  return true;
+}
+
+}
+
+bool select_skip_nodes_view(const Bvh& bvh, const std::vector<uint8_t>* cull, const SkipView& view, std::vector<uint8_t>& skip, float tail_weight)
+{
+  const std::vector<uint8_t> current(skip);
+  const uint32_t N = bvh.n_nodes;
+  if (N < 3u) return false;
+  std::vector<uint8_t> none(N, 0);
+  std::vector<uint32_t> words;
+  skip_link_table(bvh, none, words, cull);
+  ViewRays rays;
+  if (!view_rays(bvh, words.data(), view, rays)) return false;
+  const uint32_t R = (uint32_t)rays.half.size();
+  std::vector<uint32_t> visits(N, 0), passes(N, 0), cost(R, 0);
+  std::vector<std::vector<uint32_t>> testers(N);
+  uint32_t n_val = 0;
+  for (uint32_t r = 0; r < R; ++r)
+    if (rays.half[r]) for (uint32_t k = rays.begin[r]; k < rays.begin[r + 1u]; ++k) ++visits[rays.trail[k] & 0x7FFFFFFFu];
+  for (uint32_t n = 0; n < N; ++n) { testers[n].reserve((size_t)visits[n] + visits[n] / 4u + 8u); visits[n] = 0; }
+  for (uint32_t r = 0; r < R; ++r) {
+    if (rays.half[r]) ++n_val;
+    for (uint32_t k = rays.begin[r]; k < rays.begin[r + 1u]; ++k) {
+      const uint32_t n = rays.trail[k] & 0x7FFFFFFFu, pass = rays.trail[k] >> 31;
+      if (!rays.half[r]) { ++visits[n]; passes[n] += pass; }
+      else { testers[n].push_back(r | (pass << 31)); ++cost[r]; }
+    }
+  }
+  if (n_val < kSkipViewMinRays) return false;
+  std::vector<uint32_t> order;
+  const uint32_t floor_visits = view.min_visits ? view.min_visits : kSkipViewMinVisits;
+  for (uint32_t n = 0; n < N; ++n)
+    if (!node_of(bvh, n).count && visits[n] >= floor_visits && 2u * passes[n] > visits[n]) order.push_back(n);
+  std::sort(order.begin(), order.end(), [&](uint32_t a, uint32_t b) {
+    const uint64_t l = (uint64_t)passes[a] * visits[b], r = (uint64_t)passes[b] * visits[a];
+    return l != r ? l > r : a < b;
+  });
+  skip.assign(N, 0);
+  const auto culled = [&](uint32_t n, uint32_t o) { return cull && (((*cull)[n] >> o) & 1u); };
+  std::vector<uint32_t> ends;
+  const auto ends_below = [&](uint32_t n, uint32_t o) {
+    ends.clear();
+    uint32_t stack[64], top = 0;
+    const Node nd = node_of(bvh, n);
+    stack[top++] = nd.right; stack[top++] = n + 1u;
+    while (top) {
+      const uint32_t c = stack[--top];
+      if (culled(c, o)) continue;
+      if (!skip[c]) { ends.push_back(c); continue; }
+      if (top + 2u > 64u) { ends.push_back(c); continue; }
+      stack[top++] = node_of(bvh, c).right; stack[top++] = c + 1u;
+    }
+  };
+  std::vector<uint32_t> hist(2u * (size_t)N + 2u, 0u);
+  const auto bin = [&](uint32_t c) -> uint32_t& { return hist[c < hist.size() ? c : hist.size() - 1u]; };
+  for (uint32_t r = 0; r < R; ++r) if (rays.half[r]) ++bin(cost[r]);
+  for (uint32_t n : order) {
+    if (testers[n].empty()) continue;
+    uint32_t q = 0;
+    for (uint64_t seen = 0; q < hist.size(); ++q) { seen += hist[q]; if (seen * 5u >= (uint64_t)n_val * 4u) break; }
+    uint32_t n_ends[8];
+    for (uint32_t o = 0; o < 8; ++o) { ends_below(n, o); n_ends[o] = (uint32_t)ends.size(); }
+    double delta = 0.0;
+    for (uint32_t e : testers[n]) {
+      const uint32_t r = e & 0x7FFFFFFFu, before = cost[r];
+      const uint32_t after = (e >> 31) ? before - 1u : before - 1u + n_ends[rays.octant[r]];
+      delta += (double)after - (double)before;
+      delta += (double)tail_weight * ((double)(after > q ? after - q : 0u) - (double)(before > q ? before - q : 0u));
+    }
+    if (!(delta < 0.0)) continue;
+    skip[n] = 1;
+    for (uint32_t e : testers[n]) {
+      const uint32_t r = e & 0x7FFFFFFFu;
+      --bin(cost[r]);
+      --cost[r];
+      if (!(e >> 31)) {
+        ends_below(n, rays.octant[r]);
+        for (uint32_t c : ends) { testers[c].push_back(r); ++cost[r]; }
+      }
+      ++bin(cost[r]);
+    }
+  }
+  const auto tests_under = [&](const std::vector<uint8_t>& set) {
+    std::vector<uint32_t> n_ends((size_t)N * 8u, 0u);
+    const std::vector<uint8_t> chosen(skip);
+    skip = set;
+    for (uint32_t n = 0; n < N; ++n)
+      if (set[n]) for (uint32_t o = 0; o < 8; ++o) { ends_below(n, o); n_ends[(size_t)n * 8u + o] = (uint32_t)ends.size(); }
+    skip = chosen;
+    uint64_t total = 0;
+    for (uint32_t r = 0; r < R; ++r) {
+      if (!rays.half[r]) continue;
+      for (uint32_t k = rays.begin[r]; k < rays.begin[r + 1u]; ++k) {
+        const uint32_t n = rays.trail[k] & 0x7FFFFFFFu;
+        total += !set[n] ? 1u : ((rays.trail[k] >> 31) ? 0u : n_ends[(size_t)n * 8u + rays.octant[r]]);
+      }
+    }
+    return total;
+  };
+  if (current.size() == N && tests_under(current) <= tests_under(skip)) { skip = current; return false; }
+  return true;
+}
+
+int skip_view_decide(SkipViewState& st, const ptamd_camera& camera, uint32_t bounces)
+{
+  if (st.off) return kSkipViewKeep;
+  if (st.have && st.bounces == bounces && !std::memcmp(&st.camera, &camera, sizeof camera)) { st.changes = 0; return kSkipViewKeep; }
+  if (st.have && ++st.changes > kSkipViewMaxChanges) { st.off = true; st.have = false; return kSkipViewRevert; }
+  st.have = true; st.camera = camera; st.bounces = bounces;
+  ++st.selections;
+  return kSkipViewSelect;
+}
+
+namespace {
+
 uint32_t rays_knob(uint32_t rule_default)
 {
   const char* e = tuning_env("PTAMD_SKIP_RAYS");
diff --git a/cuda-pathtracer_amd/native.py b/cuda-pathtracer_amd/native.py
--- a/cuda-pathtracer_amd/native.py
+++ b/cuda-pathtracer_amd/native.py
@@ -298,6 +298,11 @@
     "ptamd_scene_cull_count": (C.c_int, [C.c_void_p, C.c_uint32, C.POINTER(C.c_uint32)]),
     "ptamd_last_restart_form": (C.c_int, [C.c_void_p, C.POINTER(C.c_int32)]),
     "ptamd_host_faces_away": (C.c_int, [C.c_void_p, C.c_uint32, C.c_void_p]),
+    "ptamd_scene_skip_view_count": (C.c_int, [C.c_void_p, C.c_uint32, C.POINTER(C.c_uint32)]),
+    "ptamd_host_skip_view_trace": (C.c_int, [C.POINTER(Face), C.c_uint32, C.POINTER(Camera), C.c_uint32, C.c_uint32, C.c_uint32,
+                                             C.POINTER(C.c_float), C.c_uint32, C.POINTER(C.c_int32), C.POINTER(C.c_uint64),
+                                             C.POINTER(C.c_uint32), C.c_void_p, C.c_void_p]),
+    "ptamd_host_skip_view_guard": (C.c_int, [C.POINTER(Camera), C.POINTER(C.c_uint32), C.c_uint32, C.c_void_p, C.POINTER(C.c_uint32)]),
 }
 
 _lib = None
diff --git a/cuda-pathtracer_amd/render.py b/cuda-pathtracer_amd/render.py
--- a/cuda-pathtracer_amd/render.py
+++ b/cuda-pathtracer_amd/render.py
@@ -151,6 +151,11 @@
         out = C.c_uint32(0)
         N.check(self._lib.ptamd_scene_cull_count(self._h, scene_id, C.byref(out)))
         return out.value
+
+    def scene_skip_view_count(self, scene_id: int) -> tuple:
+        out = (C.c_uint32 * 2)(0, 0)
+        N.check(self._lib.ptamd_scene_skip_view_count(self._h, scene_id, out))
+        return out[0], bool(out[1])
 
     def last_restart_form(self) -> int:
         out = C.c_int32(-1)
@@ -477,6 +482,33 @@
                                       rays.ctypes.data_as(C.POINTER(C.c_float)), len(rays), out.ctypes.data_as(C.POINTER(C.c_int32)),
                                       counters, C.byref(n_nodes), skip_out.ctypes.data, words.ctypes.data))
     return {"records": out, "nodes": counters[0], "tris": counters[1], "skip": skip_out, "words": words}
+
+
+def host_skip_view_trace(scene: HostScene, rays: np.ndarray, camera=None, width: int = 1920, height: int = 1080, bounces: int = 4) -> dict:
+    rays = np.ascontiguousarray(rays, dtype=np.float32).reshape(-1, 6)
+    lib = N.load()
+    faces = scene.faces.ctypes.data_as(C.POINTER(N.Face))
+    cam = scene.camera_struct() if camera is None else camera
+    n_nodes = C.c_uint32(0)
+    N.check(lib.ptamd_host_skip_trace(faces, None, len(scene.faces), 0, 0.0, None, None, 0, None, None, C.byref(n_nodes), None, None))
+    out = np.zeros((len(rays), 4), dtype=np.int32)
+    skip_out = np.zeros(n_nodes.value, dtype=np.uint8)
+    words = np.zeros((n_nodes.value + 1, 8), dtype=np.uint32)
+    counters = (C.c_uint64 * 4)(0, 0, 0, 0)
+    N.check(lib.ptamd_host_skip_view_trace(faces, len(scene.faces), C.byref(cam), width, height, bounces,
+                                           rays.ctypes.data_as(C.POINTER(C.c_float)), len(rays), out.ctypes.data_as(C.POINTER(C.c_int32)),
+                                           counters, C.byref(n_nodes), skip_out.ctypes.data, words.ctypes.data))
+    return {"records": out, "nodes": counters[0], "tris": counters[1], "skip": skip_out, "words": words, "chosen": bool(counters[3])}
+
+
+def host_skip_view_guard(cameras, bounces) -> tuple:
+    n = len(cameras)
+    cams = (N.Camera * n)(*cameras)
+    b = (C.c_uint32 * n)(*bounces)
+    out = np.zeros(n, dtype=np.uint8)
+    made = C.c_uint32(0)
+    N.check(N.load().ptamd_host_skip_view_guard(cams, b, n, out.ctypes.data, C.byref(made)))
+    return out, made.value
 
 
 def host_bvh4_trace(scene: HostScene, rays: np.ndarray):
diff --git a/include/ptamd.h b/include/ptamd.h
--- a/include/ptamd.h
+++ b/include/ptamd.h
@@ -438,6 +438,11 @@
                           const uint8_t* skip_in, const float* rays, uint32_t n, int32_t* out, uint64_t* counters,
                           uint32_t* n_nodes, uint8_t* skip_out, uint32_t* words_out);
 int ptamd_host_faces_away(const float* edges, uint32_t n, uint8_t* out);
+int ptamd_scene_skip_view_count(ptamd_context* ctx, uint32_t scene_id, uint32_t selections[2]);
+int ptamd_host_skip_view_trace(const ptamd_face* faces, uint32_t n_faces, const ptamd_camera* camera, uint32_t width, uint32_t height,
+                               uint32_t bounces, const float* rays, uint32_t n, int32_t* out, uint64_t* counters,
+                               uint32_t* n_nodes, uint8_t* skip_out, uint32_t* words_out);
+int ptamd_host_skip_view_guard(const ptamd_camera* cameras, const uint32_t* bounces, uint32_t n, uint8_t* decisions, uint32_t* selections);
 
 #ifdef __cplusplus
 }
```
